# LSaldyt/JAX_llama

Measured on AMD Instinct MI355X. Metric: output_tokens_per_sec, higher is better.
Workload: dtype bf16; 1 GPU; model=llama3-8b, global_batch=2048, seq_len=384, prompt_len=128, gen_len=256, parallelism=dp1, mp=1

## Files before the change

### jax_llama_amd/csrc/bindings.cpp

```cpp
#include <torch/extension.h>
#include <c10/hip/HIPStream.h>

#include "kernels/launchers.h"

namespace {

using torch::Tensor;

hipStream_t stream() { return c10::hip::getCurrentHIPStream().stream(); }

void check(bool cond, const char* msg) { TORCH_CHECK(cond, "jax_llama_amd._C: ", msg); }

void check_gpu(const Tensor& t, const char* name) {
  TORCH_CHECK(t.is_cuda(), "jax_llama_amd._C: ", name, " must be a GPU tensor");
  TORCH_CHECK(t.is_contiguous(), "jax_llama_amd._C: ", name, " must be contiguous");
}

void rc(int r, const char* what) {
  TORCH_CHECK(r == 0, "jax_llama_amd._C: ", what, " failed (code ", r, ")");
}

void gemm_rc(int r, const char* what) {
  const char* why = r == -1   ? "no legal plan for this shape / tile id / epilogue / fused norm / K split"
                    : r == -3 ? "the slab workspace is missing or too small"
// ... 368 lines not shown
                     int64_t splits, c10::optional<Tensor> x_packed, int64_t spl, c10::optional<Tensor> sk_ws,
                     c10::optional<Tensor> sk_tk, c10::optional<Tensor> o_w, int64_t o_n, int64_t o_k,
                     c10::optional<Tensor> o_h, c10::optional<Tensor> o_hb, c10::optional<Tensor> o_hb_pack,
                     int64_t tp_state) {
  check_gpu(x, "x");
  check_packed(w, n, k);
  check(x.dim() == 2 && x.size(1) == k && x.scalar_type() == torch::kBFloat16, "linear_qkv_attn: x bf16 [M, K]");
  const int64_t m = x.size(0);
  check(m <= 32, "linear_qkv_attn: M <= 32");
  jla::QKVArgs qa = qkv_args(m, n, table, positions, kc, vc, slot, 1, h, hkv, dh, q);
  for (auto* t : {&kv_start, &out, &ws, &tickets, &sync}) check_gpu(*t, "linear_qkv_attn arg");
  check(kv_start.scalar_type() == torch::kInt32 && kv_start.numel() == m, "kv_start int32 [B]");
  check(out.scalar_type() == torch::kBFloat16 && out.numel() == m * h * dh, "out bf16 [B, H * Dh]");
  check(ws.scalar_type() == torch::kFloat32 && ws.numel() >= m * hkv * splits * (h / hkv) * (dh + 4), "ws too small");
  check(tickets.scalar_type() == torch::kInt32 && tickets.numel() >= m * hkv, "tickets int32 [pairs]");
  check(sync.scalar_type() == torch::kInt32 && (size_t)sync.numel() >= jla::qkv_attn_sync_ints(),
        "sync int32 [qkv_attn_sync_ints()]");
  check(t_cap <= kc.size(2), "t_cap <= cache length");
  const jla::bf16_t* xp = packed_ptr(x_packed, m, k, "x_packed");
  check(spl == 1 || spl == 2, "linear_qkv_attn: spl 1 or 2");
  if (spl > 1) {
    check(sk_ws.has_value() && sk_tk.has_value(), "linear_qkv_attn spl 2: sk_ws and sk_tk (skinny_workspace)");
    check_gpu(*sk_ws, "sk_ws");
    check_gpu(*sk_tk, "sk_tk");
    check(sk_ws->scalar_type() == torch::kFloat32 && sk_tk->scalar_type() == torch::kInt32 &&
              sk_tk->numel() >= n / 16,
          "linear_qkv_attn: sk_ws fp32, sk_tk int32 [N / 16]");
    qa.sk_ws = ptr<float>(*sk_ws);
    qa.sk_tk = ptr<int32_t>(*sk_tk);
    qa.sk_ws_floats = (int)sk_ws->numel();
  }
  jla::QKVArgs qo{};
  float* oh = nullptr;
  int o_mode = 0;
  if (o_w.has_value()) {
    check_packed(*o_w, o_n, o_k);
    check(o_k == h * dh, "linear_qkv_attn: Wo has H * Dh input columns");
    check(o_h.has_value() && o_hb.has_value(), "linear_qkv_attn: the fused o projection needs h and hb");
    check_gpu(*o_h, "h");
    check_gpu(*o_hb, "hb");
    check(o_h->scalar_type() == torch::kFloat32 && o_h->numel() == m * o_n && o_hb->scalar_type() == torch::kBFloat16 &&
              o_hb->numel() == m * o_n, "linear_qkv_attn: h fp32 / hb bf16 [M, N_o]");
    const int og = jla::qkv_attn_o_groups((int)m, (int)(h / hkv), (int)o_n, (int)o_k);
    check(og > 0, "linear_qkv_attn: the o projection cannot be fused at this shape (qkv_attn_o_groups)");
    oh = ptr<float>(*o_h);
    qo.res_bf16 = bf(*o_hb);
    qo.pack = packed_ptr(o_hb_pack, m, o_n, "o_hb_pack");
    o_mode = MODE_RESIDUAL;
    if (tp_state) {
      void* st = reinterpret_cast<void*>(tp_state);
      check(og <= jla::CAR_WG_COUNTERS && og * jla::TPRES_REGION <= jla::car_max_bytes(st),
            "linear_qkv_attn: too many o workgroups for the TP buffer");
      qo.tp = jla::car_device(st);
      o_mode = MODE_TPRESID;
    }
  }
  rc(jla::linear_qkv_attn(xp ? xp : cbf(x), w.data_ptr(), m, n, k, (float)rms_eps, qa, xp != nullptr, bf(out),
                          packed_ptr(out_pack, m, h * dh, "out_pack"), ptr<int32_t>(kv_start), ptr<float>(ws),
                          ptr<int32_t>(tickets), ptr<int32_t>(sync), (int)t_cap, (int)splits, (int)spl, stream(),
                          o_w.has_value() ? o_w->data_ptr() : nullptr, oh, (int)o_n, (int)o_k, o_mode,
                          o_w.has_value() ? &qo : nullptr),
     "linear_qkv_attn");
}

bool check_gemm_ws(const c10::optional<Tensor>& ws, int64_t k, int64_t ksplit, int64_t m, int64_t n, bool rms,
                   int64_t tile) {
  if (!is_g5(tile) && ksplit <= 1) return false;
  check(ws.has_value(), "gemm: a K split (gemm5: any plan) needs the slab workspace");
  check_gpu(*ws, "gemm ws");
  const int64_t ks = is_g5(tile) ? jla::gemm5_ksplit((int)k, (int)ksplit) : ksplit;
  check(ws->scalar_type() == torch::kFloat32 && ws->numel() >= ks * m * (n + (rms ? 1 : 0)), "gemm ws too small");
  return true;
}

static float* rms_ws_ptr(const c10::optional<Tensor>& rws, int64_t m, size_t* floats) {
  *floats = 0;
  if (!rws.has_value()) return nullptr;
  check_gpu(*rws, "rms_ws");
  check(rws->scalar_type() == torch::kFloat32 && rws->numel() >= m, "rms_ws: fp32, >= M floats");
  *floats = rws->numel();
  return ptr<float>(*rws);
}

void gemm(Tensor x, Tensor w, int64_t n, int64_t k, Tensor out, int64_t mode, bool accumulate,
          c10::optional<Tensor> mirror, int64_t ksplit, c10::optional<Tensor> ws, double rms_eps, int64_t tile,
          c10::optional<Tensor> pack_out, c10::optional<Tensor> rms_ws, int64_t n_body) {
  check_gpu(x, "x");
  check_packed(w, n, k);
  check(n_body >= 0 && (n_body == 0 || jla::gemm_tail_width((int)tile) > 0), "gemm n_body: tail-balanced tiles only");
  check(x.dim() == 2 && x.size(1) == k && x.scalar_type() == torch::kBFloat16, "x must be bf16 [M, K]");
  check(mode >= 0 && mode <= 2, "gemm mode");
  const int64_t m = x.size(0);
  check_linear_out(out, m, n, mode);
  jla::bf16_t* mir = mode == 1 ? mirror_ptr(mirror, out.numel()) : nullptr;
  jla::QKVArgs pqa{};
  if (pack_out.has_value()) {
    check(m <= SKINNY_MAX_M && (mode == 1 || mode == 2) && (mode != 1 || mir), "gemm pack_out: decode M, residual "
          "(with its mirror) or SwiGLU");
    check(ksplit > 1 || is_g5(tile), "gemm pack_out: the split-K reduce-kernel path only");
    pqa.pack = packed_ptr(pack_out, m, mode == 2 ? n / 2 : n, "pack_out");
  }
  const bool slabs = check_gemm_ws(ws, k, ksplit, m, n, rms_eps >= 0, tile);
  size_t rfl = 0;
  float* rws = rms_ws_ptr(rms_ws, m, &rfl);
  gemm_rc(jla::gemm(cbf(x), w.data_ptr(), out.data_ptr(), m, n, k, mode, accumulate,
                    out.scalar_type() == torch::kFloat32, mir, pqa.pack ? &pqa : nullptr,
                    slabs ? ptr<float>(*ws) : nullptr, slabs ? ws->numel() : 0, ksplit, stream(), (float)rms_eps,
                    (int)tile, rws, rfl, (int)n_body),
          "gemm");
}

void gemm_qkv(Tensor x, Tensor w, int64_t n, int64_t k, Tensor table, Tensor positions, Tensor kc, Tensor vc,
              Tensor slot, int64_t seq_len, int64_t h, int64_t hkv, int64_t dh, Tensor q, int64_t ksplit,
              c10::optional<Tensor> ws, double rms_eps, int64_t tile, c10::optional<Tensor> rms_ws) {
  check_gpu(x, "x");
  check_packed(w, n, k);
  check(x.dim() == 2 && x.size(1) == k && x.scalar_type() == torch::kBFloat16, "x must be bf16 [M, K]");
  const int64_t m = x.size(0);
  jla::QKVArgs qa = qkv_args(m, n, table, positions, kc, vc, slot, seq_len, h, hkv, dh, q);
  const bool slabs = check_gemm_ws(ws, k, ksplit, m, n, rms_eps >= 0, tile);
  size_t rfl = 0;
  float* rws = rms_ws_ptr(rms_ws, m, &rfl);
  gemm_rc(jla::gemm(cbf(x), w.data_ptr(), nullptr, m, n, k, MODE_QKV, 0, 0, nullptr, &qa,
                    slabs ? ptr<float>(*ws) : nullptr, slabs ? ws->numel() : 0, ksplit, stream(), (float)rms_eps,
                    (int)tile, rws, rfl),
          "gemm_qkv");
}

void rope_kv_write(Tensor qkv, Tensor table, Tensor positions, Tensor kc, Tensor vc, Tensor slot, int64_t seq_len,
                   int64_t h, int64_t hkv, int64_t dh, Tensor q) {
  for (auto* t : {&qkv, &table, &positions, &kc, &vc, &slot, &q}) check_gpu(*t, "rope_kv_write arg");
  check(qkv.scalar_type() == torch::kBFloat16 && kc.scalar_type() == torch::kBFloat16 &&
            vc.scalar_type() == torch::kBFloat16 && q.scalar_type() == torch::kBFloat16,
        "rope_kv_write bf16 tensors");
  check(table.scalar_type() == torch::kFloat32 && table.dim() == 3 && table.size(1) == dh / 2 && table.size(2) == 2,
        "rope table must be fp32 [L, Dh/2, 2]");
  check(positions.scalar_type() == torch::kInt32 && slot.scalar_type() == torch::kInt32, "int32 positions/slot");
  const int64_t m = qkv.size(0);
  check(qkv.dim() == 2 && qkv.size(1) == (h + 2 * hkv) * dh, "qkv shape");
  check(positions.numel() == m && m % seq_len == 0, "positions shape");
  const int64_t b = m / seq_len;
  check(kc.dim() == 4 && kc.size(0) == b && kc.size(1) == hkv && kc.size(3) == dh && vc.sizes() == kc.sizes(),
        "cache shape [B, Hkv, T, Dh]");
  check(q.numel() == m * h * dh, "q out shape");
  rc(jla::rope_kv_write(cbf(qkv), ptr<float>(table), table.size(0), ptr<int32_t>(positions), bf(kc), bf(vc),
                        ptr<int32_t>(slot), m, seq_len, h, hkv, dh, kc.size(2), bf(q), stream()),
     "rope_kv_write");
}

void check_attn(const Tensor& q, const Tensor& kc, const Tensor& vc, const Tensor& slot, const Tensor& kv_start,
                const c10::optional<Tensor>& key_mask, const Tensor& out) {
  for (auto* t : {&q, &kc, &vc, &slot, &kv_start, &out}) check_gpu(*t, "attention arg");
  check(q.scalar_type() == torch::kBFloat16 && kc.scalar_type() == torch::kBFloat16 &&
            vc.scalar_type() == torch::kBFloat16 && out.scalar_type() == torch::kBFloat16,
        "attention bf16 tensors");
  check(q.dim() == 4 && kc.dim() == 4 && kc.sizes() == vc.sizes(), "attention shapes");
  check(kc.size(0) == q.size(0) && kc.size(3) == q.size(3), "cache/q shape mismatch");
  check(q.size(2) % kc.size(1) == 0, "H must be a multiple of Hkv");
  check(slot.scalar_type() == torch::kInt32 && kv_start.scalar_type() == torch::kInt32 &&
            kv_start.numel() == q.size(0),
        "slot/kv_start");
  check(out.numel() == q.numel(), "attention out shape");
  if (key_mask.has_value()) {
    check_gpu(*key_mask, "key_mask");
    check(key_mask->scalar_type() == torch::kUInt8 && key_mask->dim() == 2 && key_mask->size(0) == q.size(0),
          "key_mask must be uint8 [B, L]");
  }
}

void attn_decode(Tensor q, Tensor kc, Tensor vc, Tensor slot, Tensor kv_start, c10::optional<Tensor> key_mask,
                 Tensor out, Tensor ws, Tensor tickets, int64_t t_cap, int64_t nsplit, c10::optional<Tensor> out_pack) {
  check_attn(q, kc, vc, slot, kv_start, key_mask, out);
  check(q.size(1) == 1, "attn_decode: one query per row");
  const int64_t b = q.size(0), h = q.size(2), dh = q.size(3), hkv = kc.size(1), T = kc.size(2);
  check(t_cap <= T, "t_cap exceeds the cache length");
  check_gpu(ws, "ws");
  check_gpu(tickets, "tickets");
  const jla::AttnPlanResult r = jla::attn_decode_plan(jla::attn_knobs(), b, h, hkv, dh, t_cap, key_mask.has_value());
  TORCH_CHECK(r.rc == 0, "jax_llama_amd._C: attn_decode: no plan (", r.why, "; see attn_plan.h)");
  TORCH_CHECK(nsplit == r.plan.nsplit, "jax_llama_amd._C: attn_decode: nsplit ", nsplit, " is not the plan's ",
              r.plan.nsplit, " (attn_decode_plan_check)");
  check(!out_pack.has_value() || r.plan.packs,
        "attn_decode: this launch does not write the packed copy (attn_decode_plan_check's packs)");
  check(ws.scalar_type() == torch::kFloat32 && (size_t)ws.numel() >= r.plan.ws_floats, "workspace too small");
  check(tickets.scalar_type() == torch::kInt32 && tickets.numel() >= r.plan.tickets, "tickets too small");
  const uint8_t* km = key_mask.has_value() ? ptr<uint8_t>(*key_mask) : nullptr;
  const int ml = key_mask.has_value() ? key_mask->size(1) : 0;
  rc(jla::attn_decode(cbf(q), cbf(kc), cbf(vc), ptr<int32_t>(slot), ptr<int32_t>(kv_start), km, ml, bf(out),
                      ptr<float>(ws), ptr<int32_t>(tickets), b, h, hkv, dh, T, t_cap, nsplit, stream(),
                      packed_ptr(out_pack, b, h * dh, "out_pack")),
     "attn_decode");
}

void attn_prefill(Tensor q, Tensor kc, Tensor vc, Tensor slot, Tensor kv_start, c10::optional<Tensor> key_mask,
                  Tensor out) {
  check_attn(q, kc, vc, slot, kv_start, key_mask, out);
  const uint8_t* km = key_mask.has_value() ? ptr<uint8_t>(*key_mask) : nullptr;
  const int ml = key_mask.has_value() ? key_mask->size(1) : 0;
  rc(jla::attn_prefill(cbf(q), cbf(kc), cbf(vc), ptr<int32_t>(slot), ptr<int32_t>(kv_start), km, ml, bf(out),
                       q.size(0), q.size(1), q.size(2), kc.size(1), q.size(3), kc.size(2), stream()),
     "attn_prefill");
}

static void check_kv8(const Tensor& kq, const Tensor& ks, const Tensor& vq, const Tensor& vs, int64_t b, int64_t hkv,
                      const char* who) {
  for (auto* t : {&kq, &ks, &vq, &vs}) check_gpu(*t, who);
  check(kq.scalar_type() == torch::kUInt8 && vq.scalar_type() == torch::kUInt8 && kq.dim() == 4 && kq.size(0) == b &&
            kq.size(1) == hkv && kq.size(2) > 0 && kq.size(3) == jla::ATTN_DH && vq.sizes() == kq.sizes(),
// ... 24 lines not shown
                           kq.size(2), bf(q), stream()),
     "rope_kv_write_q8");
}

void kv8_dequant(Tensor kq, Tensor ks, Tensor vq, Tensor vs, int64_t n, Tensor kout, Tensor vout) {
  check(kq.dim() == 4, "kv8_dequant: q bytes must be uint8 [B, Hkv, T, 128]");
  const int64_t b = kq.size(0), hkv = kq.size(1);
  check_kv8(kq, ks, vq, vs, b, hkv, "kv8_dequant cache");
  check_gpu(kout, "kout");
  check_gpu(vout, "vout");
  check(kout.scalar_type() == torch::kBFloat16 && vout.scalar_type() == torch::kBFloat16 && kout.dim() == 4 &&
            kout.size(0) == b && kout.size(1) == hkv && kout.size(3) == jla::ATTN_DH && vout.sizes() == kout.sizes(),
        "kv8_dequant: outputs must be bf16 [B, Hkv, n_out, 128]");
  check(n >= 0 && n <= kq.size(2) && n <= kout.size(2), "kv8_dequant: n within the cache and the outputs");
  check(b * hkv <= INT32_MAX && kq.size(2) <= INT32_MAX, "kv8_dequant: sizes");
  rc(jla::kv8_dequant(ptr<uint8_t>(kq), ptr<float>(ks), ptr<uint8_t>(vq), ptr<float>(vs), bf(kout), bf(vout), b * hkv,
                      kq.size(2), n, kout.size(2), stream()),
     "kv8_dequant");
}

void attn_decode_q8(Tensor q, Tensor kq, Tensor ks, Tensor vq, Tensor vs, Tensor slot, Tensor kv_start,
                    c10::optional<Tensor> key_mask, Tensor out, int64_t t_cap, c10::optional<Tensor> ws,
                    c10::optional<Tensor> tickets) {
  for (auto* t : {&q, &slot, &kv_start, &out}) check_gpu(*t, "attn_decode_q8 arg");
  check(q.scalar_type() == torch::kBFloat16 && out.scalar_type() == torch::kBFloat16 && q.dim() == 4 && q.size(1) == 1,
        "attn_decode_q8: q bf16 [B, 1, H, Dh]");
  const int64_t b = q.size(0), h = q.size(2), dh = q.size(3);
  check(kq.dim() == 4, "attn_decode_q8: q bytes must be uint8 [B, Hkv, T, 128]");
  const int64_t hkv = kq.size(1), T = kq.size(2);
  check_kv8(kq, ks, vq, vs, b, hkv, "attn_decode_q8 cache");
  check(slot.scalar_type() == torch::kInt32 && slot.numel() >= 1 && kv_start.scalar_type() == torch::kInt32 &&
            kv_start.numel() == b,
        "slot/kv_start");
  check(out.numel() == q.numel(), "attention out shape");
  check(t_cap >= 0 && t_cap <= T, "t_cap exceeds the cache length");
  check(b <= 65535, "attn_decode_q8: at most 65535 rows");
  if (key_mask.has_value()) {
    check_gpu(*key_mask, "key_mask");
    check(key_mask->scalar_type() == torch::kUInt8 && key_mask->dim() == 2 && key_mask->size(0) == b,
          "key_mask must be uint8 [B, L]");
  }
  const jla::AttnQ8PlanResult r =
      jla::attn_decode_q8_plan(jla::attn_knobs(), b, h, hkv, dh, t_cap, key_mask.has_value());
  TORCH_CHECK(r.rc == 0, "jax_llama_amd._C: attn_decode_q8: no plan (", r.why, "; see attn_plan.h)");
  float* wsp = nullptr;
  int32_t* tkp = nullptr;
  if (r.plan.nsplit > 1) {
    TORCH_CHECK(ws.has_value() && tickets.has_value(), "jax_llama_amd._C: attn_decode_q8: the plan splits the keys (nsplit ",
                r.plan.nsplit, "): ws and tickets are required (attn_decode_q8_split_check)");
    check_gpu(*ws, "ws");
    check_gpu(*tickets, "tickets");
    TORCH_CHECK(ws->scalar_type() == torch::kFloat32 && ws->device() == q.device() &&
                    (size_t)ws->numel() >= r.plan.ws_floats,
                "jax_llama_amd._C: attn_decode_q8: ws must be fp32 on q's device with at least B * H * nsplit * (128 + 4) = ",
                r.plan.ws_floats, " floats (attn_decode_q8_split_check)");
    TORCH_CHECK(tickets->scalar_type() == torch::kInt32 && tickets->device() == q.device() &&
                    tickets->numel() >= r.plan.tickets,
                "jax_llama_amd._C: attn_decode_q8: tickets must be int32 on q's device, one per (row, kv head) pair = ",
                r.plan.tickets, " (attn_decode_q8_split_check)");
    wsp = ptr<float>(*ws);
    tkp = ptr<int32_t>(*tickets);
  }
  const uint8_t* km = key_mask.has_value() ? ptr<uint8_t>(*key_mask) : nullptr;
  const int ml = key_mask.has_value() ? key_mask->size(1) : 0;
  rc(jla::attn_decode_q8(cbf(q), ptr<uint8_t>(kq), ptr<float>(ks), ptr<uint8_t>(vq), ptr<float>(vs),
                         ptr<int32_t>(slot), ptr<int32_t>(kv_start), km, ml, bf(out), b, h, hkv, dh, T, t_cap,
                         stream(), wsp, r.plan.ws_floats, tkp, r.plan.tickets),
     "attn_decode_q8");
}

void argmax(Tensor logits, Tensor idx, Tensor val) {
  check_gpu(logits, "logits");
  check_gpu(idx, "idx");
  check_gpu(val, "val");
  check(logits.scalar_type() == torch::kFloat32 && logits.dim() == 2, "logits must be fp32 [B, V]");
  check(idx.scalar_type() == torch::kInt32 && val.scalar_type() == torch::kFloat32 &&
            idx.numel() == logits.size(0) && val.numel() == logits.size(0),
        "argmax outputs");
  rc(jla::argmax(ptr<float>(logits), logits.size(0), logits.size(1), ptr<int32_t>(idx), ptr<float>(val), stream()),
     "argmax");
}

void gemm_argmax(Tensor x, Tensor w, int64_t n, int64_t k, Tensor ws, double rms_eps, Tensor idx, Tensor val,
                 c10::optional<Tensor> rms_ws) {
  check_gpu(x, "x");
  check_packed(w, n, k);
  check(x.dim() == 2 && x.size(1) == k && x.scalar_type() == torch::kBFloat16, "x must be bf16 [M, K]");
  const int64_t m = x.size(0);
  check_gpu(ws, "ws");
  check(ws.scalar_type() == torch::kFloat32 && (size_t)ws.numel() >= jla::gemm_argmax_workspace_floats(m, n),
        "gemm_argmax ws too small");
  check_gpu(idx, "idx");
  check_gpu(val, "val");
  check(idx.scalar_type() == torch::kInt32 && val.scalar_type() == torch::kFloat32 && idx.numel() == m &&
            val.numel() == m,
        "gemm_argmax outputs");
  size_t rfl = 0;
  float* rws = rms_ws_ptr(rms_ws, m, &rfl);
  rc(jla::gemm_argmax(cbf(x), w.data_ptr(), ptr<float>(ws), ws.numel(), m, n, k, (float)rms_eps, ptr<int32_t>(idx),
                      ptr<float>(val), stream(), rws, rfl),
     "gemm_argmax");
}

static void check_logprob_io(const Tensor& targets, const Tensor& tgt, const Tensor& mx, const Tensor& se, int64_t m,
                             int64_t col_offset) {
  for (auto* t : {&targets, &tgt, &mx, &se}) check_gpu(*t, "logprob arg");
  check(targets.scalar_type() == torch::kInt32 && targets.numel() == m, "targets must be int32 [M]");
  for (auto* t : {&tgt, &mx, &se})
    check(t->scalar_type() == torch::kFloat32 && t->numel() == m, "logprob outputs must be fp32 [M]");
  check(col_offset >= 0 && col_offset <= INT32_MAX, "col_offset");
}

void gemm_logprob(Tensor x, Tensor w, int64_t n, int64_t k, Tensor ws, double rms_eps, Tensor targets,
                  int64_t col_offset, Tensor tgt, Tensor mx, Tensor se, c10::optional<Tensor> rms_ws) {
  check_gpu(x, "x");
  check_packed(w, n, k);
  check(x.dim() == 2 && x.size(1) == k && x.scalar_type() == torch::kBFloat16, "x must be bf16 [M, K]");
  const int64_t m = x.size(0);
  check_gpu(ws, "ws");
  check(ws.scalar_type() == torch::kFloat32 && (size_t)ws.numel() >= jla::gemm_logprob_workspace_floats(m, n),
        "gemm_logprob ws too small");
  check_logprob_io(targets, tgt, mx, se, m, col_offset);
  size_t rfl = 0;
  float* rws = rms_ws_ptr(rms_ws, m, &rfl);
  gemm_rc(jla::gemm_logprob(cbf(x), w.data_ptr(), ptr<float>(ws), ws.numel(), m, n, k, (float)rms_eps,
                            ptr<int32_t>(targets), (int)col_offset, ptr<float>(tgt), ptr<float>(mx), ptr<float>(se),
                            stream(), rws, rfl),
          "gemm_logprob");
}

void logprob_rows(Tensor logits, Tensor targets, int64_t col_offset, Tensor tgt, Tensor mx, Tensor se) {
  check_gpu(logits, "logits");
  check(logits.scalar_type() == torch::kFloat32 && logits.dim() == 2 && logits.size(1) > 0,
        "logits must be fp32 [B, V]");
  check(logits.size(1) <= INT32_MAX, "logprob_rows: V too large");
  check_logprob_io(targets, tgt, mx, se, logits.size(0), col_offset);
  rc(jla::logprob_rows(ptr<float>(logits), logits.size(0), logits.size(1), ptr<int32_t>(targets), (int)col_offset,
                       ptr<float>(tgt), ptr<float>(mx), ptr<float>(se), stream()),
     "logprob_rows");
}

void topk_chunk(Tensor logits, int64_t k, int64_t idx_offset, Tensor cv, Tensor ci) {
  for (auto* t : {&logits, &cv, &ci}) check_gpu(*t, "topk_chunk arg");
  check(logits.scalar_type() == torch::kFloat32 && logits.dim() == 2, "logits must be fp32 [B, V]");
  const int64_t b = logits.size(0), v = logits.size(1);
  check(k >= 1 && k <= 64 && k <= v, "topk_chunk: 1 <= k <= min(64, V)");
  const int64_t c = (int64_t)jla::topk_chunks(v) * k;
  check(cv.scalar_type() == torch::kFloat32 && ci.scalar_type() == torch::kInt32 && cv.numel() == b * c &&
            ci.numel() == b * c,
        "topk_chunk: candidates must be [B, chunks*k] fp32/int32");
  rc(jla::topk_chunk(ptr<float>(logits), b, v, k, idx_offset, ptr<float>(cv), ptr<int32_t>(ci), stream()),
     "topk_chunk");
}

void topk_merge(Tensor cv, Tensor ci, int64_t k, int64_t mode, c10::optional<Tensor> out_v,
                c10::optional<Tensor> out_i, c10::optional<Tensor> nxt, double temperature, double top_p,
                int64_t seed, c10::optional<Tensor> step) {
  check_gpu(cv, "cv");
  check_gpu(ci, "ci");
  check(cv.dim() == 2 && cv.sizes() == ci.sizes() && cv.scalar_type() == torch::kFloat32 &&
            ci.scalar_type() == torch::kInt32,
        "topk_merge: candidates [B, C] fp32/int32");
  const int64_t b = cv.size(0), c = cv.size(1);
  check(k >= 1 && k <= 64 && k <= c && c <= 4096, "topk_merge: 1 <= k <= 64, k <= C <= 4096");
  float* ov = nullptr;
  int32_t* oi = nullptr;
  int32_t* nx = nullptr;
  const int32_t* st = nullptr;
  if (mode == 0) {
    check(out_v.has_value() && out_i.has_value(), "topk_merge mode 0 needs out_v/out_i");
    check_gpu(*out_v, "out_v");
    check_gpu(*out_i, "out_i");
    check(out_v->scalar_type() == torch::kFloat32 && out_i->scalar_type() == torch::kInt32 &&
              out_v->numel() == b * k && out_i->numel() == b * k,
          "topk_merge outputs [B, k]");
    ov = ptr<float>(*out_v);
    oi = ptr<int32_t>(*out_i);
  } else {
    check(mode == 1 && nxt.has_value() && step.has_value(), "topk_merge mode 1 needs nxt and step");
    check_gpu(*nxt, "nxt");
    check_gpu(*step, "step");
    check(nxt->scalar_type() == torch::kInt32 && nxt->numel() == b && step->scalar_type() == torch::kInt32,
          "topk_merge nxt [B] / step [1] int32");
    check(temperature > 0, "topk_merge: temperature > 0");
    nx = ptr<int32_t>(*nxt);
    st = ptr<int32_t>(*step);
  }
  rc(jla::topk_merge(ptr<float>(cv), ptr<int32_t>(ci), b, c, k, mode, ov, oi, nx, (float)temperature, (float)top_p,
                     (uint64_t)seed, st, stream()),
     "topk_merge");
}

void decode_update(Tensor nxt, Tensor finished, Tensor sequences, Tensor cur_len, Tensor tokens, Tensor positions,
                   Tensor slot, int64_t pad, int64_t eos) {
  for (auto* t : {&nxt, &finished, &sequences, &cur_len, &tokens, &positions, &slot}) {
    check_gpu(*t, "decode_update arg");
    check(t->scalar_type() == torch::kInt32, "decode_update: int32 tensors");
  }
  const int64_t b = nxt.numel();
  check(finished.numel() == b && tokens.numel() == b && positions.numel() == b && sequences.dim() == 2 &&
            sequences.size(0) == b,
        "decode_update shapes");
  rc(jla::decode_update(ptr<int32_t>(nxt), ptr<int32_t>(finished), ptr<int32_t>(sequences), ptr<int32_t>(cur_len),
                        ptr<int32_t>(tokens), ptr<int32_t>(positions), ptr<int32_t>(slot), b, sequences.size(1), pad,
                        eos, stream()),
     "decode_update");
}

py::tuple car_alloc(int64_t max_bytes, int64_t world) {
  void* buf = nullptr;
// ... 63 lines not shown
  check(m >= 1 && m <= SKINNY_MAX_M, "linear_tp_residual: 1 <= M <= 64");
  check(h.scalar_type() == torch::kFloat32 && h.numel() == m * n && hb.scalar_type() == torch::kBFloat16 &&
            hb.numel() == m * n, "h fp32 / hb bf16 [M, N]");
  void* st = reinterpret_cast<void*>(state);
  const int64_t groups = n / 16;
  check(groups <= jla::CAR_WG_COUNTERS && groups * jla::TPRES_REGION <= jla::car_max_bytes(st),
        "linear_tp_residual: too many workgroups for the buffer");
  jla::QKVArgs qa{};
  qa.res_bf16 = bf(hb);
  qa.pack = packed_ptr(hb_pack, m, n, "hb_pack");
  qa.tp = jla::car_device(st);
  run_skinny(x, w, n, k, h.data_ptr(), MODE_TPRESID, -1.0, true, true, &qa, variant, ws ? *ws : Tensor(),
             tickets ? *tickets : Tensor(), packed_ptr(x_packed, m, k, "x_packed"));
}

void gemm_tp_residual(int64_t state, Tensor x, Tensor w, int64_t n, int64_t k, Tensor h, Tensor hb, int64_t ksplit,
                      Tensor ws, int64_t tile) {
  check_gpu(x, "x");
  check_gpu(h, "h");
  check_gpu(hb, "hb");
  check_packed(w, n, k);
  check(x.dim() == 2 && x.size(1) == k && x.scalar_type() == torch::kBFloat16, "x must be bf16 [M, K]");
  const int64_t m = x.size(0);
  check(h.scalar_type() == torch::kFloat32 && h.numel() == m * n && hb.scalar_type() == torch::kBFloat16 &&
            hb.numel() == m * n, "h fp32 / hb bf16 [M, N]");
  void* st = reinterpret_cast<void*>(state);
  const int64_t groups = jla::gemm_tp_groups((int)m, (int)n);
  check(groups <= jla::CAR_WG_COUNTERS && groups * jla::TPRES_REGION <= jla::car_max_bytes(st),
        "gemm_tp_residual: the output does not fit the fused exchange buffer");
  check_gemm_ws(ws, k, ksplit, m, n, false, tile);
  jla::QKVArgs qa{};
  qa.tp = jla::car_device(st);
  gemm_rc(jla::gemm(cbf(x), w.data_ptr(), h.data_ptr(), m, n, k, MODE_TPRESID, 1, 1, bf(hb), &qa, ptr<float>(ws),
                    ws.numel(), ksplit, stream(), -1.f, (int)tile, nullptr, 0),
          "gemm_tp_residual");
}

void car_pairs(int64_t state, int64_t mode, Tensor vals, Tensor idx, int64_t idx_offset, int64_t k,
               c10::optional<Tensor> out_v, Tensor out_i) {
  check_gpu(vals, "vals");
  check_gpu(idx, "idx");
  check_gpu(out_i, "out_i");
  check(vals.scalar_type() == torch::kFloat32 && idx.scalar_type() == torch::kInt32 &&
            out_i.scalar_type() == torch::kInt32 && vals.numel() == idx.numel(),
        "car_pairs dtypes");
  const int64_t n = vals.numel();
  auto* st = reinterpret_cast<void*>(state);
  float* ov = nullptr;
  if (out_v.has_value()) {
    check_gpu(*out_v, "out_v");
    check(out_v->scalar_type() == torch::kFloat32 && out_v->numel() == out_i.numel(), "out_v");
    ov = ptr<float>(*out_v);
  }
  if (mode == 0) {
    check(out_i.numel() == n, "car_pairs argmax out shape");
  } else {
    check(mode == 1 && ov && k > 0 && n % k == 0 && out_i.numel() == n * jla::car_world(st), "car_pairs top-k shapes");
  }
  rc(jla::car_pairs(st, (int)mode, ptr<float>(vals), ptr<int32_t>(idx), (int)idx_offset, n, (int)k, ov,
                    ptr<int32_t>(out_i), stream()),
     "car_pairs");
}

}

PYBIND11_MODULE(TORCH_EXTENSION_NAME, m) {
  m.doc() = "jax_llama_amd gfx950 (MI355X) HIP kernels";
  m.attr("SKINNY_MAX_M") = SKINNY_MAX_M;
  m.attr("ARCH") = "gfx950";
  m.def("embedding", &embedding, py::arg("ids"), py::arg("table"), py::arg("out"),
        py::arg("mirror") = py::none());
  m.def("rms_scale", &rms_scale);
  m.def("rmsnorm", &rmsnorm);
  m.def("residual_add", &residual_add);
  m.def("gemm_f32", &gemm_f32);
  m.def("prefetch", &prefetch, py::arg("t"), py::arg("grid") = 128);
  m.def("linear_skinny", &linear_skinny, py::arg("x"), py::arg("w"), py::arg("n"), py::arg("k"), py::arg("out"),
        py::arg("mode"), py::arg("rms_eps"), py::arg("accumulate"), py::arg("variant"), py::arg("ws"),
        py::arg("tickets"), py::arg("mirror") = py::none(), py::arg("x_packed") = py::none(),
        py::arg("pack_out") = py::none());
  m.def("gemm", &gemm, py::arg("x"), py::arg("w"), py::arg("n"), py::arg("k"), py::arg("out"), py::arg("mode"),
        py::arg("accumulate"), py::arg("mirror") = py::none(), py::arg("ksplit") = 1, py::arg("ws") = py::none(),
        py::arg("rms_eps") = -1.0, py::arg("tile") = 0, py::arg("pack_out") = py::none(),
        py::arg("rms_ws") = py::none(), py::arg("n_body") = 0);
  m.def("gemm_tail_split", [](int64_t tiles_m, int64_t n, int64_t width, int64_t cus) {
    const int nb = jla::gemm_tail_split((int)tiles_m, (int)n, (int)width, cus > 0 ? (int)cus : jla::gemm_num_cus());
    return std::make_pair((int64_t)nb, nb > 0 ? (n - nb * width + 127) / 128 : (int64_t)0);
  }, py::arg("tiles_m"), py::arg("n"), py::arg("width"), py::arg("cus") = 0);
  m.def("gemm_plan_check", [](int64_t m, int64_t n, int64_t k, int64_t mode, bool rms, int64_t ksplit, int64_t tile,
                              bool has_rms_ws, int64_t n_body) {
    return jla::gemm_plan_check((int)m, (int)n, (int)k, (int)mode, rms, (int)ksplit, (int)tile, has_rms_ws, (int)n_body);
  }, py::arg("m"), py::arg("n"), py::arg("k"), py::arg("mode"), py::arg("rms"), py::arg("ksplit"), py::arg("tile"),
     py::arg("has_rms_ws"), py::arg("n_body") = 0);
  m.def("gemv_plan_check", [](int64_t m, int64_t n, int64_t k, int64_t mode, bool x_f32, bool x_packed,
                              int64_t variant) {
    const jla::GemvPlanResult r = jla::gemv_plan((int)m, (int)n, (int)k, (int)mode, x_f32, x_packed, (int)variant);
    const jla::GemvPlan& p = r.plan;
    return py::make_tuple(r.rc, p.mt, p.nt, p.nw, p.deep, p.xp, p.ksplit);
  }, py::arg("m"), py::arg("n"), py::arg("k"), py::arg("mode"), py::arg("x_f32"), py::arg("x_packed"),
     py::arg("variant"));
  m.def("gemv_w8_plan_check", [](int64_t m, int64_t n, int64_t k, int64_t mode, bool x_f32) {
    const jla::GemvPlanResult r = jla::gemv_w8_plan((int)m, (int)n, (int)k, (int)mode, x_f32);
    return py::make_tuple(r.rc, r.plan.mt, r.plan.nt, r.plan.nw);
  }, py::arg("m"), py::arg("n"), py::arg("k"), py::arg("mode"), py::arg("x_f32"));
  m.def("dequant_fp8", &dequant_fp8, py::arg("w8"), py::arg("scale"), py::arg("n"), py::arg("k"), py::arg("out"));
  m.def("linear_skinny_w8", &linear_skinny_w8, py::arg("x"), py::arg("w8"), py::arg("scale"), py::arg("n"),
        py::arg("k"), py::arg("out"), py::arg("mode"), py::arg("rms_eps"), py::arg("accumulate"),
        py::arg("mirror") = py::none(), py::arg("pack_out") = py::none());
  m.def("linear_qkv_w8", &linear_qkv_w8, py::arg("x"), py::arg("w8"), py::arg("scale"), py::arg("n"), py::arg("k"),
        py::arg("rms_eps"), py::arg("table"), py::arg("positions"), py::arg("kc"), py::arg("vc"), py::arg("slot"),
        py::arg("seq_len"), py::arg("h"), py::arg("hkv"), py::arg("dh"), py::arg("q"));
  m.def("gemv_w4_plan_check", [](int64_t m, int64_t n, int64_t k, int64_t mode, bool x_f32) {
    const jla::GemvPlanResult r = jla::gemv_w4_plan((int)m, (int)n, (int)k, (int)mode, x_f32);
    return py::make_tuple(r.rc, r.plan.mt, r.plan.nt, r.plan.nw);
  }, py::arg("m"), py::arg("n"), py::arg("k"), py::arg("mode"), py::arg("x_f32"));
  m.def("dequant_fp4", &dequant_fp4, py::arg("w4"), py::arg("s4"), py::arg("n"), py::arg("k"), py::arg("out"));
  m.def("linear_skinny_w4", &linear_skinny_w4, py::arg("x"), py::arg("w4"), py::arg("s4"), py::arg("n"),
        py::arg("k"), py::arg("out"), py::arg("mode"), py::arg("rms_eps"), py::arg("accumulate"),
        py::arg("mirror") = py::none(), py::arg("pack_out") = py::none());
  m.def("linear_qkv_w4", &linear_qkv_w4, py::arg("x"), py::arg("w4"), py::arg("s4"), py::arg("n"), py::arg("k"),
        py::arg("rms_eps"), py::arg("table"), py::arg("positions"), py::arg("kc"), py::arg("vc"), py::arg("slot"),
        py::arg("seq_len"), py::arg("h"), py::arg("hkv"), py::arg("dh"), py::arg("q"));
  m.def("gemv_variant_table", []() {
    py::dict t;
    for (const jla::GemvVariant& v : jla::GEMV_VARIANTS) t[py::int_(v.id)] = py::make_tuple(v.xp, v.split);
    return t;
  });
  m.attr("GEMV_SPLIT_MAX_GROUPS") = jla::GEMV_SPLIT_MAX_GROUPS;
  m.def("gemm_qkv_direct_ok", [](int64_t m, int64_t tile, int64_t k) {
    return jla::gemm_qkv_direct_ok((int)m, (int)tile, (int)k) != 0;
  });
  m.def("gemm_set_g4_default", [](int64_t on) { jla::gemm_set_g4_default((int)on); });
  m.def("gemm_set_g4_group", [](int64_t gm) { jla::gemm_set_g4_group((int)gm); });
  m.def("gemm_qkv", &gemm_qkv, py::arg("x"), py::arg("w"), py::arg("n"), py::arg("k"), py::arg("table"),
        py::arg("positions"), py::arg("kc"), py::arg("vc"), py::arg("slot"), py::arg("seq_len"), py::arg("h"),
        py::arg("hkv"), py::arg("dh"), py::arg("q"), py::arg("ksplit"), py::arg("ws"), py::arg("rms_eps") = -1.0,
        py::arg("tile") = 0, py::arg("rms_ws") = py::none());
  m.def("gemm_argmax", &gemm_argmax, py::arg("x"), py::arg("w"), py::arg("n"), py::arg("k"), py::arg("ws"),
        py::arg("rms_eps"), py::arg("idx"), py::arg("val"), py::arg("rms_ws") = py::none());
  m.def("gemm_argmax_workspace", [](int64_t m, int64_t n) { return (int64_t)jla::gemm_argmax_workspace_floats(m, n); });
  m.def("gemm_logprob", &gemm_logprob, py::arg("x"), py::arg("w"), py::arg("n"), py::arg("k"), py::arg("ws"),
        py::arg("rms_eps"), py::arg("targets"), py::arg("col_offset"), py::arg("tgt"), py::arg("mx"), py::arg("se"),
        py::arg("rms_ws") = py::none());
  m.def("gemm_logprob_workspace",
        [](int64_t m, int64_t n) { return (int64_t)jla::gemm_logprob_workspace_floats(m, n); });
  m.def("logprob_rows", &logprob_rows);
  m.def("gemm_ksplit", [](int64_t m, int64_t n, int64_t k) { return jla::gemm_ksplit(m, n, k); });
  m.def("rope_kv_write", &rope_kv_write);
  m.def("attn_set_impl", [](int64_t impl, int64_t waves_target) { jla::attn_set_impl(impl, waves_target); },
        py::arg("impl"), py::arg("waves_target") = 0);
  m.def("attn_reset_knobs", []() { jla::attn_reset_knobs(); }, "every attn_set_* knob back to its default");
  m.def("attn_decode_plan_check", [](int64_t b, int64_t h, int64_t hkv, int64_t dh, int64_t t_cap, bool masked) {
    const jla::AttnPlanResult r =
        jla::attn_decode_plan(jla::attn_knobs(), (int)b, (int)h, (int)hkv, (int)dh, (int)t_cap, masked);
    const jla::AttnPlan& p = r.plan;
    return py::make_tuple(r.rc, r.why, r.rc ? "" : jla::attn_kernel_name(p.kernel), p.nsplit, p.packs,
                          (int64_t)p.ws_floats, p.tickets, p.rep, p.kpg, p.ring, p.fold, p.wpp, p.split_len);
  }, py::arg("b"), py::arg("h"), py::arg("hkv"), py::arg("dh"), py::arg("t_cap"), py::arg("masked"));
  m.def("attn_decode_splits", [](int64_t b, int64_t hkv, int64_t t, int64_t rep) {
    return jla::attn_decode_plan(jla::attn_knobs(), (int)b, (int)(hkv * rep), (int)hkv, jla::ATTN_DH, (int)t, false)
        .plan.nsplit;
  });
  m.def("attn_decode_packs", [](int64_t b, int64_t hkv, int64_t rep) {
    return (int)jla::attn_decode_plan(jla::attn_knobs(), (int)b, (int)(hkv * rep), (int)hkv, jla::ATTN_DH, 1, false)
        .plan.packs;
  });
  m.def("linear_qkv", &linear_qkv, py::arg("x"), py::arg("w"), py::arg("n"), py::arg("k"), py::arg("rms_eps"),
        py::arg("table"), py::arg("positions"), py::arg("kc"), py::arg("vc"), py::arg("slot"), py::arg("seq_len"),
        py::arg("h"), py::arg("hkv"), py::arg("dh"), py::arg("q"), py::arg("variant"), py::arg("ws"), py::arg("tickets"),
        py::arg("x_packed") = py::none());
  m.def("linear_qkv_attn", &linear_qkv_attn, py::arg("x"), py::arg("w"), py::arg("n"), py::arg("k"),
        py::arg("rms_eps"), py::arg("table"), py::arg("positions"), py::arg("kc"), py::arg("vc"), py::arg("slot"),
        py::arg("h"), py::arg("hkv"), py::arg("dh"), py::arg("q"), py::arg("kv_start"), py::arg("out"),
        py::arg("out_pack"), py::arg("ws"), py::arg("tickets"), py::arg("sync"), py::arg("t_cap"), py::arg("splits"),
        py::arg("x_packed") = py::none(), py::arg("spl") = 1, py::arg("sk_ws") = py::none(),
        py::arg("sk_tk") = py::none(), py::arg("o_w") = py::none(), py::arg("o_n") = 0, py::arg("o_k") = 0,
        py::arg("o_h") = py::none(), py::arg("o_hb") = py::none(), py::arg("o_hb_pack") = py::none(),
        py::arg("tp_state") = 0);
  m.def("qkv_attn_splits", [](int64_t m, int64_t b, int64_t hkv, int64_t rep, int64_t t_cap, int64_t n, int64_t cus,
                              int64_t spl, int64_t o_groups) {
    return jla::qkv_attn_splits((int)m, (int)b, (int)hkv, (int)rep, (int)t_cap, (int)n, (int)cus, (int)spl,
                                (int)o_groups);
  }, py::arg("m"), py::arg("b"), py::arg("hkv"), py::arg("rep"), py::arg("t_cap"), py::arg("n"), py::arg("cus"),
     py::arg("spl") = 1, py::arg("o_groups") = 0);
  m.def("qkv_attn_o_groups", [](int64_t m, int64_t rep, int64_t n, int64_t k) {
    return jla::qkv_attn_o_groups((int)m, (int)rep, (int)n, (int)k);
  });
  m.def("qkv_attn_sync_ints", []() { return (int64_t)jla::qkv_attn_sync_ints(); });
  m.def("qkv_attn_set_o_nt", [](int64_t nt) { jla::qkv_attn_set_o_nt((int)nt); });
  m.def("qkv_attn_set_diag", [](int64_t d) { jla::qkv_attn_set_diag((int)d); });
  m.def("qkv_attn_set_stamps", [](c10::optional<Tensor> t) {
    if (t.has_value()) {
      check_gpu(*t, "stamps");
      check(t->scalar_type() == torch::kInt64, "stamps int64");
    }
    jla::qkv_attn_set_stamps(t.has_value() ? reinterpret_cast<unsigned long long*>(t->data_ptr()) : nullptr);
  });
  m.def("qkv_attn_occupancy", [](int64_t m, int64_t rep, int64_t spl, int64_t o_groups) {
    return jla::qkv_attn_occupancy((int)m, (int)rep, (int)spl, (int)o_groups);
  }, py::arg("m"), py::arg("rep"), py::arg("spl") = 1, py::arg("o_groups") = 0);
  m.def("skinny_workspace", &skinny_workspace);
  m.def("linear_skinny_argmax", &linear_skinny_argmax);
  m.def("gemm_tp_residual", &gemm_tp_residual, py::arg("state"), py::arg("x"), py::arg("w"), py::arg("n"), py::arg("k"),
        py::arg("h"), py::arg("hb"), py::arg("ksplit"), py::arg("ws"), py::arg("tile"));
  m.def("gemm_tp_groups", [](int64_t m, int64_t n) { return (int64_t)jla::gemm_tp_groups((int)m, (int)n); });
  m.def("linear_tp_residual", &linear_tp_residual, py::arg("state"), py::arg("x"), py::arg("w"), py::arg("n"),
        py::arg("k"), py::arg("h"), py::arg("hb"), py::arg("variant"), py::arg("x_packed") = py::none(),
        py::arg("hb_pack") = py::none(), py::arg("ws") = py::none(), py::arg("tickets") = py::none());
  m.def("bounds_error", [](bool reset) {
    const int r = reset ? 1 : 0;
    return (int64_t)(jla::jla_bounds_norm_embed(r) | jla::jla_bounds_rope_kv(r) | jla::jla_bounds_sample(r) |
                     jla::jla_bounds_gemm(r) | jla::jla_bounds_gemv(r) | jla::jla_bounds_kv8(r) |
                     jla::jla_bounds_attn_decode(r) | jla::jla_bounds_attn_prefill(r));
  }, "OR of the bounds-checked debug build's error words (JLA_BOUNDS_* bits); always 0 in a release build",
        py::arg("reset") = false);
#ifdef JLA_DEBUG_BOUNDS
  m.attr("DEBUG_BOUNDS") = true;
#else
  m.attr("DEBUG_BOUNDS") = false;
#endif
  m.def("attn_set_diag", [](int64_t d) { jla::attn_set_diag((int)d); });
  m.def("cu_mask_stream", [](std::vector<int64_t> words) {
    std::vector<uint32_t> mk(words.begin(), words.end());
    hipStream_t s = nullptr;
    rc(jla::cu_mask_stream_create(mk.data(), (int)mk.size(), &s), "cu_mask_stream");
    return reinterpret_cast<int64_t>(s);
// ... 97 lines not shown
```

### jax_llama_amd/csrc/kernels/gemm.hip

```cpp
#include <type_traits>

#include "car.h"
#include "common.h"
#include "gemm4w.h"
#include "gemm5ws.h"
#include "gemm_plan.h"
#include "launchers.h"
#include "ring.h"

namespace jla {

constexpr int G2_BN = 256, G2_NBUF = 4, G2_GROUP_M = 8;
#ifdef JLA_GEMM_STAMPS
__device__ unsigned long long g_gemm_stamps[8192 * 8 * 6];
#endif

JLA_DEV void g2_tile_coords(int pid, int tiles_m, int tiles_n, int& tm, int& tn) {
  const int in_group = G2_GROUP_M * tiles_n;
  const int first_m = (pid / in_group) * G2_GROUP_M;
  const int gsz = min(tiles_m - first_m, G2_GROUP_M);
  tm = first_m + (pid % in_group) % gsz;
  tn = (pid % in_group) / gsz;
}

// ... 966 lines not shown
  }
  const size_t idx = e4 * 4;
  const int m = (int)(idx / N), col = (int)(idx - (size_t)m * N);
  float4 v = sum_splits(ws, ksplit, slab4, e4);
  float rs = 1.f;
  if (ssq) {
    float t = 0.f;
    for (int s = 0; s < ksplit; ++s) t += ssq[(size_t)s * M + m];
    rs = 1.f / sqrtf(t / (float)K + rms_eps);
    v.x *= rs;
    v.y *= rs;
    v.z *= rs;
    v.w *= rs;
  }
  float vv[4] = {v.x, v.y, v.z, v.w};
  if constexpr (MODE == MODE_SWIGLU) {
    const int tile = col >> 4, c0 = col & 15;
    float4 u = sum_splits(ws, ksplit, slab4, e4 + 4);
    u.x *= rs;
    u.y *= rs;
    u.z *= rs;
    u.w *= rs;
    const float uu[4] = {u.x, u.y, u.z, u.w};
    bf16_t* o = static_cast<bf16_t*>(out) + (size_t)m * (N >> 1) + (tile >> 1) * 16 + c0;
    const uint2 pk = make_uint2(pack2bf(silu(vv[0]) * uu[0], silu(vv[1]) * uu[1]),
                                pack2bf(silu(vv[2]) * uu[2], silu(vv[3]) * uu[3]));
    *reinterpret_cast<uint2*>(o) = pk;
    if (qa.pack) *reinterpret_cast<uint2*>(qa.pack + pack_off(m, (tile >> 1) * 16 + c0, N >> 1)) = pk;
  } else if constexpr (MODE == MODE_RESIDUAL) {
    float4* o = reinterpret_cast<float4*>(static_cast<float*>(out) + idx);
    float4 r = *o;
    if (accumulate) {
      r.x += vv[0];
      r.y += vv[1];
      r.z += vv[2];
      r.w += vv[3];
    } else {
      r = make_float4(vv[0], vv[1], vv[2], vv[3]);
    }
    *o = r;
    if (mirror) {
      const uint2 pk = make_uint2(pack2bf(r.x, r.y), pack2bf(r.z, r.w));
      *reinterpret_cast<uint2*>(mirror + idx) = pk;
      if (qa.pack) *reinterpret_cast<uint2*>(qa.pack + pack_off(m, col, N)) = pk;
    }
  } else if constexpr (MODE == MODE_QKV) {
    const int head = col / qa.Dh, d0 = col - head * qa.Dh;
    const int b = m / qa.S, sq = m - b * qa.S;
    if (head < qa.H + qa.Hkv) {
      int pos = qa.positions[m];
      if (pos < 0 || pos >= qa.table_len) JLA_FLAG(JLA_BOUNDS_ROPE_POS);
      pos = pos < 0 ? 0 : (pos >= qa.table_len ? qa.table_len - 1 : pos);
#pragma unroll
      for (int p = 0; p < 2; ++p) {
        const float2 cs = qa.table[(size_t)pos * (qa.Dh >> 1) + (d0 >> 1) + p];
        const float xr = vv[2 * p], xi = vv[2 * p + 1];
        vv[2 * p] = xr * cs.x - xi * cs.y;
        vv[2 * p + 1] = xr * cs.y + xi * cs.x;
      }
    }
    const uint2 packed = make_uint2(pack2bf(vv[0], vv[1]), pack2bf(vv[2], vv[3]));
    if (head < qa.H) {
      *reinterpret_cast<uint2*>(qa.q + ((size_t)m * qa.H + head) * qa.Dh + d0) = packed;
    } else {
      const int slot = qa.slot[0] + sq;
      if (slot < qa.T) {
        const bool is_k = head < qa.H + qa.Hkv;
        const int kh = is_k ? head - qa.H : head - qa.H - qa.Hkv;
        bf16_t* cache = is_k ? qa.kc : qa.vc;
        *reinterpret_cast<uint2*>(cache + (((size_t)b * qa.Hkv + kh) * qa.T + slot) * qa.Dh + d0) = packed;
      } else {
        JLA_FLAG(JLA_BOUNDS_KV_SLOT);
      }
    }
  } else {
    if (out_f32)
      *reinterpret_cast<float4*>(static_cast<float*>(out) + idx) = make_float4(vv[0], vv[1], vv[2], vv[3]);
    else
      *reinterpret_cast<uint2*>(static_cast<bf16_t*>(out) + idx) =
          make_uint2(pack2bf(vv[0], vv[1]), pack2bf(vv[2], vv[3]));
  }
}

constexpr int TPR_ELEMS = 4096;
static_assert(TPR_ELEMS / 2 * 8 == TPRES_REGION, "one fused-exchange region per workgroup");
__global__ void __launch_bounds__(256)
    gemm_reduce_tp_kernel(const float* __restrict__ ws, int ksplit, float* __restrict__ h, bf16_t* __restrict__ hb,
                          int M, int N, const CarDevice* __restrict__ dev) {
  const CarDevice& d = *dev;
  const int w = blockIdx.x;
  const size_t slab4 = (size_t)M * N / 4;
  __shared__ int s_calls;
  if (threadIdx.x == 0) s_calls = __hip_atomic_load(d.wg_ctr + w, __ATOMIC_RELAXED, __HIP_MEMORY_SCOPE_AGENT) + 1;
  u32x2 gq[4];
  f32x4 hv[4];
#pragma unroll
  for (int j = 0; j < 4; ++j) {
    const size_t e4 = (size_t)w * (TPR_ELEMS / 4) + j * 256 + threadIdx.x;
    gq[j] = u32x2{0u, 0u};
    hv[j] = f32x4{0.f, 0.f, 0.f, 0.f};
    if (e4 < slab4) {
      const float4 v = sum_splits(ws, ksplit, slab4, e4);
      gq[j] = u32x2{pack2bf(v.x, v.y), pack2bf(v.z, v.w)};
      hv[j] = *reinterpret_cast<const f32x4*>(h + e4 * 4);
    }
  }
  __syncthreads();
  const int calls = s_calls;
  const unsigned tag = gran_tag_fused(calls);
  const long long wg_base = (long long)w * TPRES_REGION;
  const long long par_base = (long long)(calls & 1) * d.world * d.max_bytes;
#pragma unroll
  for (int j = 0; j < 4; ++j) {
    const size_t e4 = (size_t)w * (TPR_ELEMS / 4) + j * 256 + threadIdx.x;
    if (e4 >= slab4) continue;
    const long long g = wg_base + (long long)(j * 256 + threadIdx.x) * 16;
    for (int p = 0; p < d.world; ++p) {
      const __amdgpu_buffer_rsrc_t rp = rsrc(d.buf[p]);
      const long long o = par_base + (long long)d.rank * d.max_bytes + g;
      st_sys8(rp, o, u32x2{gq[j][0], tag});
      st_sys8(rp, o + 8, u32x2{gq[j][1], tag});
    }
  }
  const bool give_up = __hip_atomic_load(d.error, __ATOMIC_RELAXED, __HIP_MEMORY_SCOPE_SYSTEM) != 0;
  const __amdgpu_buffer_rsrc_t mine = rsrc(d.buf[d.rank]);
#pragma unroll
  for (int j = 0; j < 4; ++j) {
    const size_t e4 = (size_t)w * (TPR_ELEMS / 4) + j * 256 + threadIdx.x;
    if (e4 >= slab4) continue;
    const long long g = wg_base + (long long)(j * 256 + threadIdx.x) * 16;
    float sm[4] = {0.f, 0.f, 0.f, 0.f};
    u32x4 r[CAR_MAX_WORLD];
    car_gather16(d, mine, par_base + g, d.max_bytes, tag, give_up, r);
#pragma unroll
    for (int p = 0; p < CAR_MAX_WORLD; ++p) {
      if (p < d.world) {
        sm[0] += __uint_as_float(r[p][0] << 16);
        sm[1] += __uint_as_float(r[p][0] & 0xffff0000u);
        sm[2] += __uint_as_float(r[p][2] << 16);
        sm[3] += __uint_as_float(r[p][2] & 0xffff0000u);
      }
    }
    f32x4 n;
#pragma unroll
    for (int i = 0; i < 4; ++i) n[i] = hv[j][i] + sm[i];
    *reinterpret_cast<f32x4*>(h + e4 * 4) = n;
    *reinterpret_cast<u32x2*>(hb + e4 * 4) = u32x2{pack2bf(n[0], n[1]), pack2bf(n[2], n[3])};
  }
  if (threadIdx.x == 0) __hip_atomic_store(d.wg_ctr + w, calls, __ATOMIC_RELAXED, __HIP_MEMORY_SCOPE_AGENT);
}
int gemm_tp_groups(int M, int N) { return (int)(((size_t)M * N + TPR_ELEMS - 1) / TPR_ELEMS); }


static int g2_wm(int M) { return M <= 128 ? 1 : 2; }

int gemm_ksplit(int M, int N, int K) {
  const int KS = K >> 5;
  const int bm = 128 * g2_wm(M);
  const int tiles = ((N + G2_BN - 1) / G2_BN) * ((M + bm - 1) / bm);
  int ks = min(256 / tiles, max(1, K / (2 * M)));
  ks = ks < 1 ? 1 : (ks > 16 ? 16 : ks);
  while (ks > 1 && KS / ks < 4) --ks;
  const int kc = (KS + ks - 1) / ks;
  return (KS + kc - 1) / kc;
}

size_t gemm_workspace_floats(int M, int N, int K) {
  const int ks = gemm_ksplit(M, N, K);
  return ks > 1 ? (size_t)ks * M * (N + 1) : 0;
}

static int num_cus() {
  static int cus = 0;
  if (cus == 0) {
    int dev = 0;
    hipDeviceProp_t prop;
    if (hipGetDevice(&dev) == hipSuccess && hipGetDeviceProperties(&prop, dev) == hipSuccess)
      cus = prop.multiProcessorCount;
    if (cus <= 0) cus = 256;
  }
  return cus;
}
int gemm_num_cus() { return num_cus(); }

static bool g_g4_default = true;
void gemm_set_g4_default(int on) { g_g4_default = on != 0; }
int gemm_qkv_direct_ok(int M, int tile, int K) {
  const GemmPlanResult r = gemm_plan(M, 16, K, MODE_QKV, true, 1, tile, true, 0, 0, g_g4_default);
  return r.rc == 0 && !r.plan.reduce;
}
int gemm_plan_check(int M, int N, int K, int mode, int rms, int ksplit, int tile, int has_rms_ws, int n_body) {
  return gemm_plan(M, N, K, mode, rms != 0, ksplit, tile, has_rms_ws != 0, n_body, num_cus(), g_g4_default).rc;
}

struct GemmArgs {
  const bf16_t* x;
  const u32x4* w;
  void* out;
  int M, N, K, accumulate, out_f32;
  bf16_t* mirror;
  float rms_eps;
  float* ssq;
  float* rms_ws;
  QKVArgs qa;
  hipStream_t s;
};

static bool g4_row_stat(const GemmArgs& a, const GemmPlan& p, const float*& inv) {
  inv = p.norm == NORM_PRECOMPUTED ? a.rms_ws : nullptr;
  return inv == nullptr || rms_rowinv(a.x, a.rms_ws, a.M, a.K, a.rms_eps, a.s) == 0;
}

static int g_g4_group = 0;
void gemm_set_g4_group(int gm) { g_g4_group = gm; }
static int g4_group_m(int tiles_m) {
  const int gm = g_g4_group > 0 ? g_g4_group : 4;
  return gm < tiles_m ? gm : tiles_m;
}
static int g_g5_diag = 0;
void gemm5_set_diag(int d) { g_g5_diag = d; }

template <int MODE, int NJ>
static void launch_g4(const GemmArgs& a, const GemmPlan& p) {
  const int tm = (a.M + G4_BM - 1) / G4_BM, tn = (a.N + 32 * NJ - 1) / (32 * NJ);
  const int grid = tm * tn * p.ksplit, gm = g4_group_m(tm);
  const float* inv;
  if (!g4_row_stat(a, p, inv)) return;
#define JLA_G4(R, DIAG, DEEP)                                                                                       \
  gemm4_kernel<MODE, R, NJ, DIAG, DEEP><<<grid, 256, 0, a.s>>>(a.x, a.w, a.out, a.M, a.N, a.K, a.accumulate, a.out_f32, \
                                                               a.mirror, p.kc, tm, tn, a.rms_eps, a.ssq, a.qa, inv, gm)
  if constexpr (NJ != 8) {
    if (inv)
      JLA_G4(2, 0, true);
    else
      JLA_G4(0, 0, true);
  } else {
    if constexpr (MODE == MODE_STORE) {
      if (p.norm == NORM_NONE && (g_g5_diag & 192)) {
        if ((g_g5_diag & 192) == 64)
          JLA_G4(0, 1, false);
        else if ((g_g5_diag & 192) == 128)
          JLA_G4(0, 2, false);
        else
          JLA_G4(0, 3, false);
        return;
      }
    }
    if (p.norm == NORM_PRECOMPUTED) {
      if (p.deep) JLA_G4(2, 0, true); else JLA_G4(2, 0, false);
    } else if (p.norm == NORM_INLOOP) {
      if (p.deep) JLA_G4(1, 0, true); else JLA_G4(1, 0, false);
    } else {
      if (p.deep) JLA_G4(0, 0, true); else JLA_G4(0, 0, false);
    }
  }
#undef JLA_G4
}

template <int MODE>
static void launch_g4p(const GemmArgs& a, const GemmPlan& p) {
  const int tm = (a.M + G4_BM - 1) / G4_BM, tn = (a.N + G4_BN - 1) / G4_BN;
  const int grid = min(tm * tn, num_cus()), gm = g4_group_m(tm);
  const float* inv;
  if (!g4_row_stat(a, p, inv)) return;
#define JLA_G4P(R)                                                                                                  \
  gemm4p_kernel<MODE, R><<<grid, 256, 0, a.s>>>(a.x, a.w, a.out, a.M, a.N, a.K, a.accumulate, a.out_f32, a.mirror, tm, \
                                                tn, a.rms_eps, a.qa, inv, gm)
  if (p.norm == NORM_PRECOMPUTED)
    JLA_G4P(2);
  else if (p.norm == NORM_INLOOP)
    JLA_G4P(1);
  else
    JLA_G4P(0);
#undef JLA_G4P
}

template <int MODE, int NJB>
static void launch_g4t(const GemmArgs& a, const GemmPlan& p) {
  const int tm = (a.M + G4_BM - 1) / G4_BM, nt = (a.N - p.n_body * 32 * NJB + 127) / 128;
  const int grid = tm * (p.n_body + nt), gm = g4_group_m(tm);
  const float* inv;
  if (!g4_row_stat(a, p, inv)) return;
  if (inv)
    gemm4t_kernel<MODE, 2, NJB><<<grid, 256, 0, a.s>>>(a.x, a.w, a.out, a.M, a.N, a.K, a.accumulate, a.out_f32,
                                                       a.mirror, tm, p.n_body, nt, a.rms_eps, inv, gm);
  else
    gemm4t_kernel<MODE, 0, NJB><<<grid, 256, 0, a.s>>>(a.x, a.w, a.out, a.M, a.N, a.K, a.accumulate, a.out_f32,
                                                       a.mirror, tm, p.n_body, nt, a.rms_eps, nullptr, gm);
}

template <int MODE>
static void launch_g2(const GemmArgs& a, const GemmPlan& p) {
  const int cfg = p.family;
// ... 5 lines not shown
      a.x, a.w, a.out, a.M, a.N, a.K, a.accumulate, a.out_f32, a.mirror, p.kc, tm, tn, a.rms_eps, a.ssq, a.qa)
#define JLA_G2_CFG(R)                        \
  if (cfg == 2)                              \
    JLA_G2(1, false, R, 8, 4, false, 0);     \
  else if (cfg == 3)                         \
    JLA_G2(2, true, R, 4, 2, false, 0);      \
  else                                       \
    JLA_G2(2, true, R, 8, 4, true, 2)
  [[maybe_unused]] const bool rms = p.norm != NORM_NONE;
  if constexpr (MODE == MODE_QKV) {
    JLA_G2(2, true, true, 8, 4, true, 2);
  } else if constexpr (MODE == MODE_ARGMAX) {
    if (rms)
      JLA_G2(2, true, true, 8, 4, true, 2);
    else
      JLA_G2(2, true, false, 8, 4, true, 2);
  } else if constexpr (MODE == MODE_RESIDUAL) {
    JLA_G2_CFG(false);
  } else {
    if (rms) {
      JLA_G2_CFG(true);
    } else {
      JLA_G2_CFG(false);
    }
  }
#undef JLA_G2_CFG
#undef JLA_G2
}

static void launch_g5(const GemmArgs& a, const GemmPlan& p) {
  const int mt = a.M <= 128 ? 8 : 16, rows = 16 * mt, ntw = p.nj;
  const int tiles_m = (a.M + rows - 1) / rows, tiles_n = (a.N + 64 * ntw - 1) / (64 * ntw);
  const int grid = tiles_m * tiles_n * p.ksplit;
#define JLA_G5(MTV, NTV)                                                                                            \
  gemm5_partial_kernel<MTV, NTV><<<grid, 256, 0, a.s>>>(a.x, a.w, static_cast<float*>(a.out), a.M, a.N, a.K, p.kc, \
                                                        tiles_m, tiles_n, a.ssq, g_g5_diag)
  if (mt == 8 && ntw == 4)
    JLA_G5(8, 4);
  else if (mt == 8)
    JLA_G5(8, 2);
  else if (ntw == 4)
    JLA_G5(16, 4);
  else
    JLA_G5(16, 2);
#undef JLA_G5
}

template <int MODE>
static void launch_plan(const GemmArgs& a, const GemmPlan& p) {
  constexpr bool PLAIN = MODE == MODE_STORE || MODE == MODE_RESIDUAL || MODE == MODE_SWIGLU;
  switch (p.family) {
    case GEMM2_256x256:
    case GEMM2_128x256:
    case GEMM2_128x128:
      if constexpr (MODE != MODE_LOGPROB) launch_g2<MODE>(a, p);
      break;
    case GEMM4:
      if (p.nj == 8) launch_g4<MODE, 8>(a, p);
      if constexpr (MODE != MODE_ARGMAX && MODE != MODE_LOGPROB) {
        if (p.nj == 6) launch_g4<MODE, 6>(a, p);
      }
      if constexpr (PLAIN || MODE == MODE_PARTIAL) {
        if (p.nj == 4) launch_g4<MODE, 4>(a, p);
      }
      break;
    case GEMM4_PERSISTENT:
      if constexpr (PLAIN || MODE == MODE_QKV) launch_g4p<MODE>(a, p);
      break;
    case GEMM4_TAIL:
      if constexpr (PLAIN) {
        if (p.nj == 6)
          launch_g4t<MODE, 6>(a, p);
        else
          launch_g4t<MODE, 8>(a, p);
      }
      break;
    case GEMM5:
      if constexpr (MODE == MODE_PARTIAL) launch_g5(a, p);
      break;
    case GEMM_NONE: break;
  }
}

static int launch_reduce(const float* ws, int ksplit, void* out, int M, int N, int K, int mode, int accumulate,
                         int out_f32, bf16_t* mirror, const QKVArgs* qkv, const float* ssq, float rms_eps,
                         hipStream_t s) {
  const size_t total4 = (size_t)M * N / (mode == MODE_SWIGLU ? 8 : 4);
  const int rgrid = (int)((total4 + 255) / 256);
  QKVArgs qa{};
  if (qkv) qa = *qkv;
  const float eps = ssq ? rms_eps : 0.f;
  switch (mode) {
    case MODE_STORE:
      gemm_reduce_kernel<MODE_STORE><<<rgrid, 256, 0, s>>>(ws, ksplit, out, M, N, accumulate, out_f32, nullptr, qa,
                                                           ssq, K, eps);
      break;
    case MODE_RESIDUAL:
      gemm_reduce_kernel<MODE_RESIDUAL><<<rgrid, 256, 0, s>>>(ws, ksplit, out, M, N, accumulate, 1, mirror, qa,
                                                              nullptr, K, eps);
      break;
    case MODE_SWIGLU:
      gemm_reduce_kernel<MODE_SWIGLU><<<rgrid, 256, 0, s>>>(ws, ksplit, out, M, N, accumulate, 0, nullptr, qa, ssq,
                                                            K, eps);
      break;
    case MODE_QKV:
      gemm_reduce_kernel<MODE_QKV><<<rgrid, 256, 0, s>>>(ws, ksplit, out, M, N, accumulate, 0, nullptr, qa, ssq, K,
                                                         eps);
      break;
    case MODE_TPRESID:
      if (!qkv || !qa.tp || !mirror || ssq || (N & 3)) return -1;
      gemm_reduce_tp_kernel<<<gemm_tp_groups(M, N), 256, 0, s>>>(ws, ksplit, static_cast<float*>(out), mirror, M, N,
                                                                 static_cast<const CarDevice*>(qa.tp));
      break;
    default: return -1;
  }
  JLA_CHECK_LAUNCH();
  return 0;
}

int gemm(const bf16_t* x, const void* W, void* out, int M, int N, int K, int mode, int accumulate, int out_f32,
         bf16_t* mirror, const QKVArgs* qkv, float* ws, size_t ws_floats, int ksplit, hipStream_t s,
         float rms_eps, int tile, float* rms_ws, size_t rms_ws_floats, int n_body) {
  const bool has_rms_ws = rms_ws != nullptr && rms_ws_floats >= (size_t)M;
  const GemmPlanResult r =
      gemm_plan(M, N, K, mode, rms_eps >= 0.f, ksplit, tile, has_rms_ws, n_body, num_cus(), g_g4_default);
  const GemmPlan& p = r.plan;
  if (r.rc != 0 || p.family == GEMM_NONE) return r.rc;
  if (mode == MODE_ARGMAX || mode == MODE_LOGPROB || (mode == MODE_QKV && !qkv)) return -1;
  const u32x4* w = static_cast<const u32x4*>(W);
  if (!p.reduce) {
    GemmArgs a{x, w, out, M, N, K, accumulate, out_f32, nullptr, rms_eps, nullptr, rms_ws, QKVArgs{}, s};
    switch (mode) {
      case MODE_QKV:
        a.out = nullptr, a.accumulate = a.out_f32 = 0, a.qa = *qkv;
        launch_plan<MODE_QKV>(a, p);
        break;
      case MODE_STORE: launch_plan<MODE_STORE>(a, p); break;
      case MODE_RESIDUAL:
        a.out_f32 = 1, a.mirror = mirror, a.rms_eps = -1.f;
        launch_plan<MODE_RESIDUAL>(a, p);
        break;
      case MODE_SWIGLU:
        a.out_f32 = 0;
        launch_plan<MODE_SWIGLU>(a, p);
        break;
      default: return -1;
    }
    JLA_CHECK_LAUNCH();
    return 0;
  }
  const size_t slabs = (size_t)p.ksplit * M * N;
  if (ws == nullptr || ws_floats < slabs + (p.norm != NORM_NONE ? (size_t)p.ksplit * M : 0)) return -3;
  float* ssq = p.norm != NORM_NONE ? ws + slabs : nullptr;
  launch_plan<MODE_PARTIAL>(GemmArgs{x, w, ws, M, N, K, 0, 1, nullptr, rms_eps, ssq, nullptr, QKVArgs{}, s}, p);
  JLA_CHECK_LAUNCH();
  return launch_reduce(ws, p.ksplit, out, M, N, K, mode, accumulate, out_f32, mirror, qkv, ssq, rms_eps, s);
}

JLA_DEV void amax_merge(float& bv, int& bi, float ov, int oi) {
  if (ov > bv || (ov == bv && oi < bi)) {
    bv = ov;
    bi = oi;
  }
}

template <int TPR>
__global__ void __launch_bounds__(TPR == 64 ? 256 : TPR)
    argmax_partials_kernel(const float2* __restrict__ part, int P, int M, int32_t* __restrict__ idx,
                           float* __restrict__ val) {
  __shared__ float s_v[16];
  __shared__ int s_i[16];
  const int row = TPR == 64 ? blockIdx.x * 4 + (threadIdx.x >> 6) : blockIdx.x;
  const int t = TPR == 64 ? (threadIdx.x & 63) : threadIdx.x;
  if (row >= M) return;
  const float2* pr = part + (size_t)row * P;
  float bv[4] = {-INFINITY, -INFINITY, -INFINITY, -INFINITY};
  int bi[4] = {0x7fffffff, 0x7fffffff, 0x7fffffff, 0x7fffffff};
  for (int k0 = t; k0 < P; k0 += 4 * TPR) {
    float2 e[4];
#pragma unroll
    for (int u = 0; u < 4; ++u) {
      const int k = k0 + u * TPR;
      e[u] = k < P ? pr[k] : make_float2(-INFINITY, __int_as_float(0x7fffffff));
    }
#pragma unroll
    for (int u = 0; u < 4; ++u) amax_merge(bv[u], bi[u], e[u].x, __float_as_int(e[u].y));
  }
#pragma unroll
  for (int u = 1; u < 4; ++u) amax_merge(bv[0], bi[0], bv[u], bi[u]);
#pragma unroll
  for (int o = 32; o > 0; o >>= 1) amax_merge(bv[0], bi[0], __shfl_xor(bv[0], o, 64), __shfl_xor(bi[0], o, 64));
  if constexpr (TPR > 64) {
    const int w = threadIdx.x >> 6;
    if ((threadIdx.x & 63) == 0) {
      s_v[w] = bv[0];
      s_i[w] = bi[0];
    }
    __syncthreads();
    if (threadIdx.x == 0) {
      for (int ww = 1; ww < TPR / 64; ++ww) amax_merge(bv[0], bi[0], s_v[ww], s_i[ww]);
      idx[row] = bi[0] == 0x7fffffff ? 0 : bi[0];
      val[row] = bv[0];
    }
  } else if (t == 0) {
    idx[row] = bi[0] == 0x7fffffff ? 0 : bi[0];
    val[row] = bv[0];
  }
}

static void launch_argmax_partials(const float2* part, int P, int M, int32_t* idx, float* val, hipStream_t s) {
  if (M <= 512)
    argmax_partials_kernel<1024><<<M, 1024, 0, s>>>(part, P, M, idx, val);
  else
    argmax_partials_kernel<64><<<(M + 3) / 4, 256, 0, s>>>(part, P, M, idx, val);
}

int argmax_partials(const float* part, int P, int M, int32_t* idx, float* val, hipStream_t s) {
  if (M <= 0) return 0;
  launch_argmax_partials(reinterpret_cast<const float2*>(part), P, M, idx, val, s);
  JLA_CHECK_LAUNCH();
  return 0;
}

size_t gemm_argmax_workspace_floats(int M, int N) { return (size_t)M * ((N + G2_BN - 1) / G2_BN) * 4 * 2; }

int gemm_argmax(const bf16_t* x, const void* W, float* ws, size_t ws_floats, int M, int N, int K, float rms_eps,
                int32_t* idx, float* val, hipStream_t s, float* rms_ws, size_t rms_ws_floats) {
  const bool has_rms_ws = rms_ws != nullptr && rms_ws_floats >= (size_t)M;
  const GemmPlanResult r = gemm_plan(M, N, K, MODE_ARGMAX, rms_eps >= 0.f, 1, 0, has_rms_ws, 0, 0, g_g4_default);
  if (r.rc != 0 || r.plan.family == GEMM_NONE) return r.rc;
  if (ws == nullptr || ws_floats < gemm_argmax_workspace_floats(M, N)) return -3;
  launch_plan<MODE_ARGMAX>(
      GemmArgs{x, static_cast<const u32x4*>(W), ws, M, N, K, 0, 1, nullptr, rms_eps, nullptr, rms_ws, QKVArgs{}, s},
      r.plan);
  JLA_CHECK_LAUNCH();
  const int P = (N + G2_BN - 1) / G2_BN * (r.plan.family == GEMM4 ? 2 : 4);
  launch_argmax_partials(reinterpret_cast<const float2*>(ws), P, M, idx, val, s);
  JLA_CHECK_LAUNCH();
  return 0;
}

JLA_DEV void lse_merge(float& m, float& s, float om, float os) {
  constexpr float LOG2E = 1.4426950408889634f;
  if (om == -INFINITY) return;
  if (m == -INFINITY) {
    m = om;
    s = os;
    return;
  }
  const float nm = fmaxf(m, om);
  s = s * __builtin_amdgcn_exp2f((m - nm) * LOG2E) + os * __builtin_amdgcn_exp2f((om - nm) * LOG2E);
  m = nm;
}

template <int TPR>
__global__ void __launch_bounds__(TPR == 64 ? 256 : TPR)
    lse_partials_kernel(const float2* __restrict__ part, int P, int M, float* __restrict__ mx,
                        float* __restrict__ se) {
  __shared__ float s_m[16];
  __shared__ float s_s[16];
  const int row = TPR == 64 ? blockIdx.x * 4 + (threadIdx.x >> 6) : blockIdx.x;
  const int t = TPR == 64 ? (threadIdx.x & 63) : threadIdx.x;
  if (row >= M) return;
  const float2* pr = part + (size_t)row * P;
  float bm[4] = {-INFINITY, -INFINITY, -INFINITY, -INFINITY};
  float bs[4] = {0.f, 0.f, 0.f, 0.f};
  for (int k0 = t; k0 < P; k0 += 4 * TPR) {
    float2 e[4];
#pragma unroll
    for (int u = 0; u < 4; ++u) {
      const int k = k0 + u * TPR;
      e[u] = k < P ? pr[k] : make_float2(-INFINITY, 0.f);
    }
#pragma unroll
    for (int u = 0; u < 4; ++u) lse_merge(bm[u], bs[u], e[u].x, e[u].y);
  }
#pragma unroll
  for (int u = 1; u < 4; ++u) lse_merge(bm[0], bs[0], bm[u], bs[u]);
#pragma unroll
  for (int o = 32; o > 0; o >>= 1)
    lse_merge(bm[0], bs[0], __shfl_xor(bm[0], o, 64), __shfl_xor(bs[0], o, 64));
  if constexpr (TPR > 64) {
    const int w = threadIdx.x >> 6;
    if ((threadIdx.x & 63) == 0) {
      s_m[w] = bm[0];
      s_s[w] = bs[0];
    }
    __syncthreads();
    if (threadIdx.x == 0) {
      for (int ww = 1; ww < TPR / 64; ++ww) lse_merge(bm[0], bs[0], s_m[ww], s_s[ww]);
      mx[row] = bm[0];
      se[row] = bs[0];
    }
  } else if (t == 0) {
    mx[row] = bm[0];
    se[row] = bs[0];
  }
}

static void launch_lse_partials(const float2* part, int P, int M, float* mx, float* se, hipStream_t s) {
  if (M <= 512)
    lse_partials_kernel<1024><<<M, 1024, 0, s>>>(part, P, M, mx, se);
  else
    lse_partials_kernel<64><<<(M + 3) / 4, 256, 0, s>>>(part, P, M, mx, se);
}

size_t gemm_logprob_workspace_floats(int M, int N) { return (size_t)M * ((N + G4_BN - 1) / G4_BN) * 2 * 2; }

int gemm_logprob(const bf16_t* x, const void* W, float* ws, size_t ws_floats, int M, int N, int K, float rms_eps,
                 const int32_t* targets, int col_offset, float* tgt, float* mx, float* se, hipStream_t s,
                 float* rms_ws, size_t rms_ws_floats) {
  const bool has_rms_ws = rms_ws != nullptr && rms_ws_floats >= (size_t)M;
  const GemmPlanResult r = gemm_plan(M, N, K, MODE_LOGPROB, rms_eps >= 0.f, 1, 0, has_rms_ws, 0, 0, g_g4_default);
  if (r.rc != 0 || r.plan.family == GEMM_NONE) return r.rc;
  if (ws == nullptr || ws_floats < gemm_logprob_workspace_floats(M, N)) return -3;
  if (targets == nullptr || tgt == nullptr || mx == nullptr || se == nullptr) return -1;
  const hipError_t zeroed = hipMemsetAsync(tgt, 0, (size_t)M * sizeof(float), s);
  if (zeroed != hipSuccess) return (int)zeroed;
  GemmArgs a{x, static_cast<const u32x4*>(W), ws, M, N, K, 0, 1, nullptr, rms_eps, nullptr, rms_ws, QKVArgs{}, s};
  a.qa.lp_targets = targets, a.qa.lp_tgt = tgt, a.qa.lp_col_offset = col_offset;
  launch_plan<MODE_LOGPROB>(a, r.plan);
  JLA_CHECK_LAUNCH();
  launch_lse_partials(reinterpret_cast<const float2*>(ws), (N + G4_BN - 1) / G4_BN * 2, M, mx, se, s);
  JLA_CHECK_LAUNCH();
  return 0;
}

JLA_BOUNDS_ACCESSOR(gemm)

}
```

### jax_llama_amd/csrc/kernels/launchers.h

```cpp
#pragma once
#include <hip/hip_runtime.h>
#include <stdint.h>

#include "attn_plan.h"
#include "gemm_plan.h"
#include "gemv_plan.h"

namespace jla {
typedef uint16_t bf16_t;

int embedding(const int32_t* ids, const bf16_t* table, float* out, bf16_t* mirror, int M, int D, int V,
              hipStream_t s);
int rms_scale(const float* x, bf16_t* out, int M, int D, float eps, hipStream_t s);
int rms_scale_bf16(const bf16_t* x, bf16_t* out, int M, int D, float eps, hipStream_t s);
int rms_rowinv(const bf16_t* x, float* inv, int M, int D, float eps, hipStream_t s);
int residual_add(float* h, const void* p, int p_bf16, bf16_t* hb, long long n, hipStream_t s);
int prefetch(const void* p, long long nbytes, int grid, unsigned* sink, hipStream_t s);
int stream_probe(const void* p, long long nbytes, int grid, unsigned* sink, hipStream_t s);
int gemm_f32(const float* x, const float* w, float* y, int M, int N, int K, hipStream_t s);
int rmsnorm(const float* x, const float* w, float* out, int M, int D, float eps, hipStream_t s);

struct QKVArgs {
  const float2* table;
  int table_len;
  union {
    const int32_t* positions;
    const int32_t* lp_targets;
  };
  bf16_t* kc;
  bf16_t* vc;
  const int32_t* slot;
  int S, H, Hkv, Dh, T;
  bf16_t* q;
  bf16_t* res_bf16;
  bf16_t* pack;
  const void* tp;
  union {
    float* sk_ws;
    float* lp_tgt;
  };
  int32_t* sk_tk;
  union {
    int sk_ws_floats;
    int lp_col_offset;
  };
};

constexpr int CAR_WG_COUNTERS = 4096;
constexpr long long TPRES_REGION = 64 * 64 * 4;

int qkv_attn_o_groups(int M, int rep, int N, int K);
size_t qkv_attn_sync_ints();
void qkv_attn_set_o_nt(int nt);
int qkv_attn_splits(int M, int B, int Hkv, int rep, int t_cap, int N, int cus, int spl = 1, int o_groups = 0);
int qkv_attn_occupancy(int M, int rep, int spl = 1, int o_groups = 0);
void qkv_attn_set_stamps(unsigned long long* p);
void qkv_attn_set_diag(int d);
int linear_qkv_attn(const bf16_t* x, const void* W, int M, int N, int K, float rms_eps, const QKVArgs& qa, bool xp,
                    bf16_t* out, bf16_t* out_pack, const int32_t* kv_start, float* ws, int32_t* tickets, int32_t* sync,
                    int t_cap, int splits, int spl, hipStream_t s,
                    const void* o_w = nullptr, float* o_h = nullptr, int o_n = 0, int o_k = 0, int o_mode = 0,
                    const QKVArgs* qo = nullptr);
int linear_skinny(const void* x, int x_is_f32, const void* W, void* out, int M, int N, int K, int mode,
                  float rms_eps, int accumulate, int out_f32, const QKVArgs* qkv, int variant, hipStream_t s);
int dequant_fp8(const void* W8, const float* scale, void* out, int N, int K, hipStream_t s);
int linear_skinny_w8(const void* x, int x_is_f32, const void* W8, const float* scale, void* out, int M, int N, int K,
                     int mode, float rms_eps, int accumulate, int out_f32, const QKVArgs* qkv, hipStream_t s);
int dequant_fp4(const void* W4, const void* S4, void* out, int N, int K, hipStream_t s);
int linear_skinny_w4(const void* x, int x_is_f32, const void* W4, const void* S4, void* out, int M, int N, int K,
                     int mode, float rms_eps, int accumulate, int out_f32, const QKVArgs* qkv, hipStream_t s);
int clock_probe(int iters, int grid, unsigned long long* out, hipStream_t s);
int gemm(const bf16_t* x, const void* W, void* out, int M, int N, int K, int mode, int accumulate, int out_f32,
         bf16_t* mirror, const QKVArgs* qkv, float* ws, size_t ws_floats, int ksplit, hipStream_t s,
         float rms_eps = -1.f, int tile = 0, float* rms_ws = nullptr, size_t rms_ws_floats = 0, int n_body = 0);
int gemm_plan_check(int M, int N, int K, int mode, int rms, int ksplit, int tile, int has_rms_ws, int n_body);
int gemm_ksplit(int M, int N, int K);
size_t gemm_workspace_floats(int M, int N, int K);
int gemm_tp_groups(int M, int N);
int gemm_qkv_direct_ok(int M, int tile, int K);
int gemm_num_cus();
void gemm_set_g4_default(int on);
void gemm_set_g4_group(int gm);
void gemm5_set_diag(int d);
int gemm_argmax(const bf16_t* x, const void* W, float* ws, size_t ws_floats, int M, int N, int K, float rms_eps,
                int32_t* idx, float* val, hipStream_t s, float* rms_ws = nullptr, size_t rms_ws_floats = 0);
size_t gemm_argmax_workspace_floats(int M, int N);
int argmax_partials(const float* part, int P, int M, int32_t* idx, float* val, hipStream_t s);
int gemm_logprob(const bf16_t* x, const void* W, float* ws, size_t ws_floats, int M, int N, int K, float rms_eps,
                 const int32_t* targets, int col_offset, float* tgt, float* mx, float* se, hipStream_t s,
                 float* rms_ws = nullptr, size_t rms_ws_floats = 0);
size_t gemm_logprob_workspace_floats(int M, int N);

int rope_kv_write(const bf16_t* qkv, const float* table, int table_len, const int32_t* positions, bf16_t* kc,
                  bf16_t* vc, const int32_t* slot, int M, int S, int H, int Hkv, int Dh, int T, bf16_t* q_out,
                  hipStream_t s);

const AttnKnobs& attn_knobs();
void attn_reset_knobs();
void attn_set_impl(int impl, int waves_target);
void attn_set_v3_max_pairs(int n);
void attn_set_v3_kpg(int mult);
void attn_set_v5_max_pairs(int n);
void attn_set_v5_fold(int n);
void attn_set_v6(int mode);
void attn_set_v6_wpp(int wpp);
void attn_set_q8_waves(int waves);
void attn_set_q8_splits(int n);
void attn_set_diag(int d);
void attn_set_v6_diag(int d);
unsigned jla_bounds_norm_embed(int reset);
unsigned jla_bounds_rope_kv(int reset);
unsigned jla_bounds_sample(int reset);
unsigned jla_bounds_gemm(int reset);
unsigned jla_bounds_gemv(int reset);
unsigned jla_bounds_attn_decode(int reset);
unsigned jla_bounds_attn_prefill(int reset);
int attn_decode(const bf16_t* q, const bf16_t* kc, const bf16_t* vc, const int32_t* slot, const int32_t* kv_start,
                const uint8_t* key_mask, int mask_len, bf16_t* out, float* ws, int32_t* tickets, int B, int H,
                int Hkv, int Dh, int T, int t_cap, int nsplit, hipStream_t s, bf16_t* out_pack = nullptr);
int attn_decode_v6(const bf16_t* q, const bf16_t* kc, const bf16_t* vc, const int32_t* slot, const int32_t* kv_start,
                   const uint8_t* key_mask, int mask_len, bf16_t* out, int B, int H, int Hkv, int T, int t_cap,
                   int wpp, hipStream_t s, bf16_t* out_pack);
unsigned jla_bounds_kv8(int reset);
int rope_kv_write_q8(const bf16_t* qkv, const float* table, int table_len, const int32_t* positions, uint8_t* kq,
                     float* ks, uint8_t* vq, float* vs, const int32_t* slot, int M, int S, int H, int Hkv, int Dh,
                     int T, bf16_t* q_out, hipStream_t s);
int kv8_dequant(const uint8_t* kq, const float* ks, const uint8_t* vq, const float* vs, bf16_t* kout, bf16_t* vout,
                int pairs, int T, int n, int n_out, hipStream_t s);
int attn_decode_q8(const bf16_t* q, const uint8_t* kq, const float* ks, const uint8_t* vq, const float* vs,
                   const int32_t* slot, const int32_t* kv_start, const uint8_t* key_mask, int mask_len, bf16_t* out,
                   int B, int H, int Hkv, int Dh, int T, int t_cap, hipStream_t s, float* ws = nullptr,
                   size_t ws_floats = 0, int32_t* tickets = nullptr, int n_tickets = 0);
void attn_prefill_set_impl(int impl);
int attn_prefill(const bf16_t* q, const bf16_t* kc, const bf16_t* vc, const int32_t* slot, const int32_t* kv_start,
                 const uint8_t* key_mask, int mask_len, bf16_t* out, int B, int S, int H, int Hkv, int Dh, int T,
                 hipStream_t s);

int argmax(const float* logits, int B, int V, int32_t* idx, float* val, hipStream_t s);
int logprob_rows(const float* logits, int B, int V, const int32_t* targets, int col_offset, float* tgt, float* mx,
                 float* se, hipStream_t s);
int topk_chunks(int V);
int topk_chunk(const float* logits, int B, int V, int K, int idx_offset, float* cv, int32_t* ci, hipStream_t s);
int topk_merge(const float* cv, const int32_t* ci, int B, int C, int K, int mode, float* out_v, int32_t* out_i,
               int32_t* nxt, float temperature, float top_p, uint64_t seed, const int32_t* step, hipStream_t s);
size_t car_buffer_bytes(long long max_bytes, int world);
int car_alloc(long long max_bytes, int world, void** buf, void** sig, hipIpcMemHandle_t* hbuf, hipIpcMemHandle_t* hsig);
void car_free(void* buf, void* sig);
int car_init(int rank, int world, long long max_bytes, void* own_buf, void* own_sig, const hipIpcMemHandle_t* hbufs,
             const hipIpcMemHandle_t* hsigs, double timeout_s, void** state);
int car_reduce(void* state, int op, const void* in, void* out, float* h, bf16_t* hb, long long nbytes, int is_bf16,
               int two_shot, hipStream_t s,
               bf16_t* hb_pack = nullptr, int pack_cols = 0);
int car_pairs(void* state, int mode, const float* a, const int32_t* b, int idx_offset, long long n, int k,
              float* out_a, int32_t* out_b, hipStream_t s);
void car_set_gran_max(long long n);
int car_error(void* state);
const void* car_device(void* state);
long long car_max_bytes(void* state);
int car_world(void* state);
int car_set_grid(void* state, int grid);
void car_destroy(void* state);
int decode_update(const int32_t* nxt, int32_t* finished, int32_t* sequences, int32_t* cur_len, int32_t* tokens,
                  int32_t* positions, int32_t* slot, int B, int L, int pad, int eos, hipStream_t s);
int cu_census(uint32_t* out, int blocks, hipStream_t s);
int cu_mask_stream_create(const uint32_t* mask, int words, hipStream_t* out);
int cu_mask_stream_get(hipStream_t s, uint32_t* mask, int words);
int stream_destroy(hipStream_t s);
int graph_kernel_nodes(hipGraph_t g);

}
```

### jax_llama_amd/models/llama.py

```python
from __future__ import annotations

from dataclasses import dataclass
from typing import Any, Dict, List, Optional, Tuple

import numpy as np
import torch

from .. import ops
from ..config import LLaMAConfig
from ..ops import reference as ref
from ..parallel.comm import NO_COMM, TPComm
from ..parallel.partition import shard_tree
from .kv_cache import KV_FORMATS, KVCache
from .modules import LLaMABlockCollection
from .weights import Fp8Linear, Mxfp4Linear, PackedLinear

BF16 = torch.bfloat16


def _t(x) -> torch.Tensor:
    if torch.is_tensor(x):
        return x
    return torch.as_tensor(np.asarray(x))

# ... 231 lines not shown

    def save_pretrained(self, save_directory: str) -> str:
        from ..utils.native_ckpt import save_pretrained
        return save_pretrained(self, save_directory)

    @classmethod
    def from_pretrained(cls, directory: str, device="cpu", comm: Optional[TPComm] = None):
        from ..utils.native_ckpt import from_pretrained
        return from_pretrained(directory, device=device, comm=comm)

    WEIGHT_FORMATS = ("fp8_e4m3", "mxfp4")

    def quantize_weights_(self, fmt: str = "fp8_e4m3") -> "LLaMAForCausalLM":
        if fmt not in self.WEIGHT_FORMATS:
            raise ValueError(f"quantize_weights_: unknown format {fmt!r} (one of {self.WEIGHT_FORMATS})")
        if self.weight_format != "bf16":
            raise RuntimeError(f"quantize_weights_: the weights are already {self.weight_format}")
        if any(lw.qkv is None for lw in self.layers):
            raise RuntimeError("quantize_weights_: the model has no weights yet")
        names = ("qkv", "o", "gu", "down")
        if fmt == "mxfp4":
            for lw in self.layers:
                for name in names:
                    lin = getattr(lw, name)
                    if lin.n % 16 or lin.k % 128:
                        raise ValueError(f"quantize_weights_('mxfp4'): {name} is {lin.n}x{lin.k}; MXFP4 linear weights "
                                         "need N % 16 == 0 and K % 128 == 0")
        cls = Mxfp4Linear if fmt == "mxfp4" else Fp8Linear
        for lw in self.layers:
            for name in names:
                setattr(lw, name, cls.from_linear(getattr(lw, name)))
        from ..runtime.engine import drop_engines
        drop_engines(self)
        if self.device.type == "cuda":
            torch.cuda.empty_cache()
        return self

    @property
    def weight_format(self) -> str:
        if any(getattr(lw.qkv, "mxfp4", False) for lw in self.layers):
            return "mxfp4"
        return "fp8_e4m3" if any(getattr(lw.qkv, "fp8", False) for lw in self.layers) else "bf16"

    def weight_bytes(self) -> int:
        n = self.wte.numel() * 2 + self.lm_head.nbytes()
        for lw in self.layers:
            n += lw.qkv.nbytes() + lw.o.nbytes() + lw.gu.nbytes() + lw.down.nbytes()
        return n

    def streamed_weight_bytes_per_token(self) -> int:
        return self.weight_bytes() - self.wte.numel() * 2

    KV_CACHE_FORMATS = KV_FORMATS

    def _check_kv_format(self, fmt: str) -> str:
        if fmt not in self.KV_CACHE_FORMATS:
            raise ValueError(f"unknown KV-cache format {fmt!r} (one of {self.KV_CACHE_FORMATS})")
        if fmt == "fp8_e4m3":
            if self.head_dim != 128:
                raise ValueError(f"the fp8_e4m3 KV cache needs head_dim == 128, got {self.head_dim}")
            rep = self.n_heads // self.n_kv_heads
            if self.n_heads % self.n_kv_heads or rep not in (1, 2, 4, 8):
                raise ValueError("the fp8_e4m3 KV cache needs 1, 2, 4 or 8 query heads per kv head, got "
                                 f"{self.n_heads} / {self.n_kv_heads}")
        return fmt

    def set_kv_cache_format(self, fmt: str) -> "LLaMAForCausalLM":
        self._kv_cache_format = self._check_kv_format(fmt)
        return self

    @property
    def kv_cache_format(self) -> str:
        return getattr(self, "_kv_cache_format", "bf16")

    def init_cache(self, batch_size: int, max_length: int, kv_format: Optional[str] = None) -> KVCache:
        if max_length > self.rope_length:
            raise ValueError(f"max_length {max_length} exceeds the RoPE table ({self.rope_length}); "
                             "raise config.max_sequence_length")
        fmt = self.kv_cache_format if kv_format is None else self._check_kv_format(kv_format)
        return KVCache(self.config.num_hidden_layers, batch_size, self.n_kv_heads, max_length,
                       self.head_dim, self.device, kv_format=fmt)

    def _row_parallel(self, x: torch.Tensor, w: PackedLinear, h: torch.Tensor, hb: torch.Tensor,
                      x_packed: Optional[torch.Tensor] = None, mirror_packed: Optional[torch.Tensor] = None) -> None:
        if self.comm.size == 1:
            ops.linear_residual(x, w, h, mirror=hb, x_packed=x_packed, mirror_packed=mirror_packed)
        elif self.comm.linear_residual_(x, w, h, hb, x_packed=x_packed, hb_pack=mirror_packed):
            pass
        else:
            dt = self.comm.partial_dtype(x.numel() // x.shape[-1] * w.n, x.is_cuda)
            part = ops.linear(x, w, out_dtype=dt, x_packed=x_packed)
            self.comm.all_reduce_residual_(part, h, hb, hb_pack=mirror_packed, owned=True)

    def forward_tokens(self, ids: torch.Tensor, positions: torch.Tensor, cache: KVCache, slot0,
                       kv_start: torch.Tensor, key_mask: Optional[torch.Tensor] = None,
                       logits_mode: str = "last", collect_hidden: bool = False,
                       collect_attn: bool = False, targets: Optional[torch.Tensor] = None):
        if (logits_mode == "logprob") != (targets is not None):
            raise ValueError("logits_mode='logprob' takes `targets` (and no other mode does)")
        with ops.autotune.tp_scope(self.comm):
            return self._forward_tokens(ids, positions, cache, slot0, kv_start, key_mask, logits_mode,
                                        collect_hidden, collect_attn, targets)

    def _forward_tokens(self, ids, positions, cache, slot0, kv_start, key_mask, logits_mode, collect_hidden,
                        collect_attn, targets=None):
        b, s = ids.shape
        d = self.config.hidden_size
        hb = torch.empty(b * s, d, dtype=BF16, device=self.device)
        h = ops.embedding(ids.reshape(-1), self.wte, mirror=hb)
        hidden, attns = self.blocks(h, hb, positions, cache, slot0, kv_start, key_mask, s,
                                    output_hidden_states=collect_hidden, output_attentions=collect_attn)
        if logits_mode == "none":
            logits = None
        elif logits_mode == "logprob":
            off = self.tp_rank * self.vocab_local
            if self.precision == "highest":
                logits = ops.linear_f32_logprob(self.final_norm(h), self.lm_head_f32, targets, col_offset=off)
            else:
                logits = ops.linear_logprob(hb, self.lm_head, targets, rms_eps=self.eps, col_offset=off)
        elif self.precision == "highest":
            hl = h if logits_mode == "all" else h.reshape(b, s, d)[:, -1].contiguous()
            logits = ops.linear_f32(self.final_norm(hl), self.lm_head_f32)
            if logits_mode == "argmax":
                logits = ops.argmax(logits.contiguous())
        elif logits_mode == "argmax":
            logits = ops.linear_argmax(hb.reshape(b, s, d)[:, -1].contiguous(), self.lm_head, rms_eps=self.eps)
        else:
            hl = hb if logits_mode == "all" else hb.reshape(b, s, d)[:, -1].contiguous()
            logits = ops.linear(hl, self.lm_head, rms_eps=self.eps, out_dtype=torch.float32)
        return logits, h, hidden, attns

    def gather_logits(self, logits_local: torch.Tensor) -> torch.Tensor:
        if self.comm.size == 1:
            return logits_local
        g = self.comm.all_gather(logits_local)
        return g.permute(1, 0, 2).reshape(logits_local.shape[0], -1)

    def final_norm(self, h: torch.Tensor) -> torch.Tensor:
        return ops.rmsnorm(h, self.ln_f, self.eps)

    def _prepare_call(self, input_ids, attention_mask, position_ids, past_key_values):
        ids = _t(input_ids).to(self.device, torch.int32)
        b, s = ids.shape
        if position_ids is None:
            if past_key_values is not None:
                raise ValueError("Make sure to provide `position_ids` when passing `past_key_values`.")
            position_ids = torch.arange(s, dtype=torch.int32).expand(b, s)
        pos = _t(position_ids).to(self.device, torch.int32).reshape(b, s).contiguous()
        if past_key_values is None:
            cache = KVCache(self.config.num_hidden_layers, b, self.n_kv_heads, s, self.head_dim, self.device,
                            kv_format=self.kv_cache_format)
            slot0 = 0
        else:
            cache = past_key_values
            slot0 = cache.index
            if slot0 + s > cache.max_length:
                raise ValueError(f"cache overflow: {slot0}+{s} > {cache.max_length}")
        t_valid = slot0 + s
        if attention_mask is None:
            mask = torch.ones(b, t_valid, dtype=torch.int32)
        else:
            mask = _t(attention_mask).to("cpu").to(torch.int32)
            if mask.shape[1] >= t_valid:
                mask = mask[:, :t_valid]
            elif mask.shape[1] == s:
                mask = torch.cat([torch.ones(b, slot0, dtype=torch.int32), mask], 1)
            else:
                raise ValueError(f"attention_mask of shape {tuple(mask.shape)} does not cover {t_valid} slots")
        kv_start, key_mask = mask_to_kv_start(mask, self.device)
        return ids, pos, cache, slot0, kv_start, key_mask

    def __call__(self, input_ids, attention_mask=None, position_ids=None, params=None,
                 past_key_values: Optional[KVCache] = None, dropout_rng=None, train: bool = False,
                 output_attentions: Optional[bool] = None, output_hidden_states: Optional[bool] = None,
                 return_dict: Optional[bool] = None):
        if train:
            raise NotImplementedError("inference-only framework (reference dropout/remat paths are training-only)")
        if params is not None and id(params) != self._params_id:
            self.load_params(params)
        oa = self.config.output_attentions if output_attentions is None else output_attentions
        oh = self.config.output_hidden_states if output_hidden_states is None else output_hidden_states
        rd = self.config.return_dict if return_dict is None else return_dict
        ids, pos, cache, slot0, kv_start, key_mask = self._prepare_call(
            input_ids, attention_mask, position_ids, past_key_values)
        b, s = ids.shape
        logits, h, hidden, attns = self.forward_tokens(ids, pos, cache, slot0, kv_start, key_mask,
                                                       logits_mode="all", collect_hidden=oh,
                                                       collect_attn=oa)
        if past_key_values is not None:
            cache.advance(s)
        logits = self.gather_logits(logits).reshape(b, s, -1).to(self.dtype)
        hs = None
        if oh:
            hs = tuple(x.to(self.dtype) for x in hidden) + (self.final_norm(h).reshape(b, s, -1).to(self.dtype),)
        out = CausalLMOutput(logits=logits, past_key_values=past_key_values, hidden_states=hs,
                             attentions=tuple(attns) if oa else None)
        return out if rd else out.to_tuple()

    def score(self, input_ids, attention_mask=None, labels=None, ignore_index: int = -100) -> ScoreOutput:
        from ..runtime import engine as _engine
        ids = _t(input_ids).to("cpu", torch.int64)
        if ids.dim() != 2 or ids.shape[1] < 2:
            raise ValueError(f"score: input_ids must be (B, S) with S >= 2, got {tuple(ids.shape)}")
        b, s = ids.shape
        if s > self.rope_length:
            raise ValueError(f"score: {s} positions exceed the RoPE table ({self.rope_length}); "
                             "raise config.max_sequence_length")
        lab = ids if labels is None else _t(labels).to("cpu", torch.int64)
        if lab.shape != ids.shape:
            raise ValueError(f"score: labels {tuple(lab.shape)} must have input_ids' shape {tuple(ids.shape)}")
        if attention_mask is None:
# ... 86 lines not shown
```

### jax_llama_amd/models/modules.py

```python
from __future__ import annotations

from typing import List, Optional

import torch

from .. import ops
from ..ops import reference as ref


class LLaMAAttention:
    def __init__(self, model, layer_idx: int):
        self.model = model
        self.layer_idx = layer_idx

    @property
    def weights(self):
        return self.model.layers[self.layer_idx]

    def __call__(self, h, hb, positions, cache, slot0, kv_start, key_mask, seq_len: int,
                 output_attentions: bool = False, pk: Optional["PackedActs"] = None) -> Optional[torch.Tensor]:
        m, lw = self.model, self.weights
        kc, vc = cache.layer(self.layer_idx)
        splits = og = 0
        o_state = None
        if not output_attentions:
            og = ops.qkv_attention_o_groups(hb, lw.o, m.n_heads, m.n_kv_heads, kc) if seq_len == 1 else 0
            o_state = m.comm.fused_o_state(hb, lw.o) if og else None
            og = og if o_state is not None else 0
            splits = ops.qkv_attention_splits(hb, lw.qkv, kc, seq_len, m.n_heads, m.n_kv_heads, key_mask, og)
            if og and not splits:
                og = 0
                splits = ops.qkv_attention_splits(hb, lw.qkv, kc, seq_len, m.n_heads, m.n_kv_heads, key_mask)
        if splits:
            hb_p = pk.hb if pk else None
            o = (lw.o, h, hb, hb_p, o_state) if og else None
            att_p = pk.att if pk is not None and not og else None
            a = ops.linear_qkv_attention(hb, lw.qkv, m.eps, m.rope, positions, kc, vc, slot0, kv_start, m.n_heads,
                                         m.n_kv_heads, m.head_dim, splits, x_packed=pk.hb_in() if pk else None,
                                         out_packed=att_p, o=o)
            if not og:
                m._row_parallel(a, lw.o, h, hb, x_packed=att_p, mirror_packed=hb_p)
            if pk is not None and pk.hb is not None:
                pk.hb_ok = True
            return None
        q = ops.linear_qkv_rope(hb, lw.qkv, m.eps, m.rope, positions, kc, vc, slot0, seq_len,
                                m.n_heads, m.n_kv_heads, m.head_dim, x_packed=pk.hb_in() if pk else None)
        b = hb.shape[0] // seq_len
        q4 = q.reshape(b, seq_len, m.n_heads, m.head_dim)
        weights = None
        att_p = None
        if output_attentions:
            s0 = int(slot0) if not torch.is_tensor(slot0) else int(slot0.item())
            kw, vw = (ops.kv8_dequant(kc, vc, s0 + seq_len) if ops.is_fp8_kv(kc) else (kc, vc))
            _, weights = ref.attention(q4, kw, vw, s0, kv_start, key_mask, return_weights=True)
            a = ops.attention(q4, kc, vc, slot0, kv_start, key_mask)
        else:
            att_p = pk.att if pk is not None and ops.attention_packs(q4, kc, key_mask) else None
            a = ops.attention(q4, kc, vc, slot0, kv_start, key_mask, out_packed=att_p)
        m._row_parallel(a, lw.o, h, hb, x_packed=att_p, mirror_packed=pk.hb if pk else None)
        if pk is not None and pk.hb is not None:
            pk.hb_ok = True
        return weights


class LLaMAMLP:
    def __init__(self, model, layer_idx: int):
        self.model = model
        self.layer_idx = layer_idx

    def __call__(self, h, hb, pk: Optional["PackedActs"] = None) -> None:
        m, lw = self.model, self.model.layers[self.layer_idx]
        g = ops.linear_swiglu(hb, lw.gu, rms_eps=m.eps, x_packed=pk.hb_in() if pk else None,
                              out_packed=pk.act if pk else None)

        m._row_parallel(g, lw.down, h, hb, x_packed=pk.act if pk else None, mirror_packed=pk.hb if pk else None)


class LLaMABlock:

    def __init__(self, model, layer_idx: int):
        self.attention = LLaMAAttention(model, layer_idx)
        self.feed_forward = LLaMAMLP(model, layer_idx)

    def __call__(self, h, hb, positions, cache, slot0, kv_start, key_mask, seq_len: int,
                 output_attentions: bool = False, pk: Optional["PackedActs"] = None):
        w = self.attention(h, hb, positions, cache, slot0, kv_start, key_mask, seq_len, output_attentions, pk)
        self.feed_forward(h, hb, pk)
        return w


class PackedActs:

    def __init__(self, rows: int, model, device, full: bool = True):
        self.hb = ops.packed_empty(rows, model.config.hidden_size, device) if full else None
        self.att = ops.packed_empty(rows, model.n_heads * model.head_dim, device)
        self.act = ops.packed_empty(rows, model.ffn, device) if full else None
        self.hb_ok = False

    def hb_in(self) -> Optional[torch.Tensor]:
        return self.hb if self.hb_ok else None


class LLaMABlockCollection:

    def __init__(self, model):
        self.blocks: List[LLaMABlock] = [LLaMABlock(model, i) for i in range(len(model.layers))]
        self.model = model

    def __len__(self):
        return len(self.blocks)

    def __call__(self, h, hb, positions, cache, slot0, kv_start, key_mask, seq_len: int,
                 output_hidden_states: bool = False, output_attentions: bool = False):
        hidden, attns = [], []
        b = hb.shape[0] // seq_len
        rows = hb.shape[0]
        pk = None
        if (ops.PACKED_X and hb.is_cuda and ops.PACKED_X_MIN_M <= rows <= min(ops.PACKED_ATT_MAX_M, ops.SKINNY_M)
                and self.model.comm.packs_residual(rows * self.model.config.hidden_size * 4)):
            pk = PackedActs(rows, self.model, hb.device, full=rows <= ops.PACKED_X_MAX_M)
        for blk in self.blocks:
            if output_hidden_states:
                hidden.append(h.reshape(b, seq_len, -1).clone())
            w = blk(h, hb, positions, cache, slot0, kv_start, key_mask, seq_len, output_attentions, pk)
            if output_attentions:
                attns.append(w)
        return hidden, attns
```

### jax_llama_amd/ops/__init__.py

```python
from __future__ import annotations

import contextlib
import os
from typing import Optional

import torch

from . import autotune
from . import reference as ref
from ._ext import available as ext_available
from ._ext import ext

BF16 = torch.bfloat16

Fp8KV = ref.Fp8KV
is_fp8_kv = ref.is_fp8_kv

MODE_STORE = 0
MODE_RESIDUAL = 1
MODE_SWIGLU = 2
MODE_QKV = 3

GEMV_VARIANT = int(os.environ.get("JLA_GEMV_VARIANT", "0"))


def _is_gpu(t: torch.Tensor) -> bool:
    return t.device.type == "cuda"


class _Workspace:

    def __init__(self):
        self._bufs = {}
        self.generation = 0
        self._scope = ""

    @contextlib.contextmanager
    def scope(self, tag: str):
        prev, self._scope = self._scope, tag + "/"
        try:
            yield
        finally:
            self._scope = prev

    def get(self, name: str, numel: int, dtype: torch.dtype, device: torch.device) -> torch.Tensor:
        key = (self._scope + name, device, dtype)
        buf = self._bufs.get(key)
        if buf is None or buf.numel() < numel:
            buf = torch.empty(max(numel, 1), dtype=dtype, device=device)
            self._bufs[key] = buf
            self.generation += 1
        return buf[:numel]

    def get_zeroed(self, name: str, numel: int, dtype: torch.dtype, device: torch.device) -> torch.Tensor:
        key = ("zeroed:" + self._scope + name, device, dtype)
        buf = self._bufs.get(key)
        if buf is None or buf.numel() < numel:
            buf = torch.zeros(max(numel, 1), dtype=dtype, device=device)
            self._bufs[key] = buf
            self.generation += 1
        return buf[:numel]

    def clear(self):
        self._bufs.clear()
        self.generation += 1


workspace = _Workspace()


def embedding(ids: torch.Tensor, table: torch.Tensor, mirror: Optional[torch.Tensor] = None) -> torch.Tensor:
    if not _is_gpu(table):
        out = ref.embedding(ids, table)
        if mirror is not None:
            mirror.copy_(out.to(BF16))
        return out
    out = torch.empty(ids.numel(), table.shape[1], dtype=torch.float32, device=table.device)
    ext().embedding(ids.reshape(-1).to(torch.int32), table, out, mirror)
    return out


def rms_scale(x: torch.Tensor, eps: float) -> torch.Tensor:
    if not _is_gpu(x):
        return ref.rms_scale(x, eps)
    out = torch.empty(x.shape, dtype=BF16, device=x.device)
    ext().rms_scale(x, out, float(eps))
    return out


def residual_add_(h: torch.Tensor, p: torch.Tensor, mirror: Optional[torch.Tensor] = None) -> torch.Tensor:
    if not _is_gpu(h):
        h.add_(p.float().view_as(h))
        if mirror is not None:
            mirror.copy_(h.to(BF16))
        return h
    assert h.is_contiguous() and h.dtype == torch.float32
    if mirror is None or h.numel() % 8:
        h.add_(p.view_as(h))
        if mirror is not None:
            mirror.copy_(h)
        return h
    ext().residual_add(h, p.contiguous(), mirror)
    return h


PREFETCH_GRID = int(os.environ.get("JLA_PREFETCH_GRID", "128"))


def prefetch(t: torch.Tensor) -> None:
    if _is_gpu(t):
        ext().prefetch(t, PREFETCH_GRID)


def linear_f32(x: torch.Tensor, w: torch.Tensor) -> torch.Tensor:
    if not _is_gpu(x):
        return x.float() @ w.float().t()
    y = torch.empty(x.shape[0], w.shape[0], dtype=torch.float32, device=x.device)
    ext().gemm_f32(x.float().contiguous(), w.float().contiguous(), y)
    return y


def rmsnorm(x: torch.Tensor, weight: torch.Tensor, eps: float) -> torch.Tensor:
    if not _is_gpu(x):
        return ref.rmsnorm(x, weight, eps)
    out = torch.empty(x.shape, dtype=torch.float32, device=x.device)
    ext().rmsnorm(x.float().contiguous(), weight.float().contiguous(), out, float(eps))
    return out


BOUNDS_CODES = {0: "token id outside the vocabulary", 1: "KV-cache write past the cache (slot >= T)",
                2: "decode step past the sequence buffer", 3: "attention asked for keys past the cache",
                4: "position outside the RoPE table"}


class BoundsError(RuntimeError):
    pass


def bounds_error(reset: bool = False) -> int:
    if not ext_available():
        return 0
    return int(ext().bounds_error(bool(reset)))


def check_bounds(reset: bool = True):
    if not ext_available() or not getattr(ext(), "DEBUG_BOUNDS", False):
        return
    err = bounds_error(reset)
    if err:
        raise BoundsError("device-side index out of range: " +
                          "; ".join(v for k, v in BOUNDS_CODES.items() if err >> k & 1))


def linear(x: torch.Tensor, w, rms_eps: Optional[float] = None, out_dtype=BF16,
           out: Optional[torch.Tensor] = None, x_packed: Optional[torch.Tensor] = None) -> torch.Tensor:
    if not _is_gpu(x):
        r = ref.linear(x, w.dense(), rms_eps, out_dtype)
        if out is not None:
            out.copy_(r)
            return out
        return r
    m = x.shape[0]
    if out is None:
        out = torch.empty(m, w.n, dtype=out_dtype, device=x.device)
    _gpu_linear(x, w, out, MODE_STORE, rms_eps, True, None, x_packed)
    return out


def linear_residual(x: torch.Tensor, w, residual: torch.Tensor, rms_eps: Optional[float] = None,
                    accumulate: bool = True, mirror: Optional[torch.Tensor] = None,
                    x_packed: Optional[torch.Tensor] = None, mirror_packed: Optional[torch.Tensor] = None) -> torch.Tensor:
    if not _is_gpu(x):
        ref.linear_residual(x, w.dense(), residual, rms_eps, accumulate)
        if mirror is not None:
            mirror.copy_(residual.to(BF16))
        return residual
    _gpu_linear(x, w, residual, MODE_RESIDUAL, rms_eps, accumulate, mirror, x_packed, mirror_packed)
    return residual


def linear_swiglu(x: torch.Tensor, w, rms_eps: Optional[float] = None, x_packed: Optional[torch.Tensor] = None,
                  out_packed: Optional[torch.Tensor] = None) -> torch.Tensor:
    if not _is_gpu(x):
        return ref.linear_swiglu(x, w.dense(), rms_eps)
    out = torch.empty(x.shape[0], w.n // 2, dtype=BF16, device=x.device)
    _gpu_linear(x, w, out, MODE_SWIGLU, rms_eps, True, None, x_packed, out_packed)
    return out


PACKED_X = os.environ.get("JLA_PACKED_X", "1") != "0"
PACKED_X_MIN_M = int(os.environ.get("JLA_PACKED_X_MIN_M", "9"))
PACKED_X_MAX_M = int(os.environ.get("JLA_PACKED_X_MAX_M", "64"))
PACKED_ATT_MAX_M = int(os.environ.get("JLA_PACKED_ATT_MAX_M", "64"))
SKINNY_M = 64
XP_VARIANTS, SPLIT_VARIANTS = autotune.XP_VARIANTS, autotune.SPLIT_VARIANTS


def packed_rows(m: int) -> int:
    return 16 if m <= 16 else (32 if m <= 32 else 64)


def packed_empty(m: int, cols: int, device) -> torch.Tensor:
    return torch.empty(packed_rows(m), cols, dtype=BF16, device=device)


class _Dequantized:

    def __init__(self, weight, n, k):
        self.weight, self.n, self.k = weight, n, k


def is_fp8(w) -> bool:
    return bool(getattr(w, "fp8", False))


def is_mxfp4(w) -> bool:
    return bool(getattr(w, "mxfp4", False))


def is_quantized(w) -> bool:
    return is_fp8(w) or is_mxfp4(w)


def bf16_weight(w):
    if is_mxfp4(w):
        buf = workspace.get(f"w4_deq_{w.n}x{w.k}", w.n * w.k, BF16, w.device).view(w.n // 16, w.k // 32, 64, 8)
        ext().dequant_fp4(w.qweight, w.scale, w.n, w.k, buf)
        return _Dequantized(buf, w.n, w.k)
    if not is_fp8(w):
        return w
    buf = workspace.get(f"w8_deq_{w.n}x{w.k}", w.n * w.k, BF16, w.device).view(w.n // 16, w.k // 32, 64, 8)
    ext().dequant_fp8(w.qweight, w.scale, w.n, w.k, buf)
    return _Dequantized(buf, w.n, w.k)


def _w8_fast(e, x, w, mode) -> bool:
    return x.shape[0] > 0 and e.gemv_w8_plan_check(x.shape[0], w.n, w.k, mode, x.dtype != BF16)[0] == 0


def _w4_fast(e, x, w, mode) -> bool:
    return x.shape[0] > 0 and e.gemv_w4_plan_check(x.shape[0], w.n, w.k, mode, x.dtype != BF16)[0] == 0


def _gpu_linear(x, w, out, mode, rms_eps, accumulate, mirror=None, x_packed=None, pack_out=None):
    assert x.is_contiguous() and out.is_contiguous()
    assert x.shape[1] == w.k, (x.shape, w.k)
    m = x.shape[0]
    e = ext()
    if is_mxfp4(w):
        if _w4_fast(e, x, w, mode):
            e.linear_skinny_w4(x, w.qweight, w.scale, w.n, w.k, out, mode, -1.0 if rms_eps is None else float(rms_eps),
                               bool(accumulate), mirror, pack_out if mode != MODE_STORE else None)
            return
        w = bf16_weight(w)
    if is_fp8(w):
        if _w8_fast(e, x, w, mode):
            e.linear_skinny_w8(x, w.qweight, w.scale, w.n, w.k, out, mode, -1.0 if rms_eps is None else float(rms_eps),
                               bool(accumulate), mirror, pack_out if mode != MODE_STORE else None)
            return
        w = bf16_weight(w)
    if m > e.SKINNY_MAX_M:
        x_packed = pack_out = None
    v = TILED if m > e.SKINNY_MAX_M else _variant(e, x, w, mode, x_packed, pack_out)
    if v == TILED and pack_out is not None and not _tiled_packs(e, m, w.n, w.k, x.device, mode, rms_eps):
        v = 1
    if v == TILED:
        _tiled(e, x, w.weight, w.n, w.k, out, mode, rms_eps, accumulate, mirror, pack_out)
    else:
        ws, tk = _skinny_ws(e, m, w.n, w.k, mode, x.device)
        e.linear_skinny(x, w.weight, w.n, w.k, out, mode, -1.0 if rms_eps is None else float(rms_eps),
                        bool(accumulate), v, ws, tk, mirror, x_packed if v in XP_VARIANTS else None, pack_out)


def linear_tp_residual(x: torch.Tensor, w, h: torch.Tensor, hb: torch.Tensor, state: int,
                       x_packed: Optional[torch.Tensor] = None, hb_pack: Optional[torch.Tensor] = None) -> torch.Tensor:
    e = ext()
    m = x.shape[0]
    assert x.dtype == BF16 and x.is_contiguous() and m <= e.SKINNY_MAX_M, (x.dtype, x.shape)
    v = _variant(e, x, w, MODE_RESIDUAL, x_packed, pack_out=True)
    if v not in autotune.GEMV_VARIANTS:
        v = 1
    ws = tk = None
    if v in SPLIT_VARIANTS:
        ws, tk = _skinny_ws(e, m, w.n, w.k, MODE_RESIDUAL, x.device)
    e.linear_tp_residual(state, x, w.weight, w.n, w.k, h, hb, v, x_packed if v in XP_VARIANTS else None, hb_pack,
                         ws, tk)
    return h


def tiled_tp_residual(x: torch.Tensor, w, h: torch.Tensor, hb: torch.Tensor, state: int) -> bool:
    e = ext()
    m = x.shape[0]
    assert x.dtype == BF16 and x.is_contiguous(), (x.dtype, x.shape)
    ks, tm = autotune.choose_gemm_plan(e, m, w.n, w.k, x.device, MODE_STORE, False)
    if tm not in autotune.G5_TILES and ks <= 1:
        return False
    ks, tm, ws = _gemm_ws(e, m, w.n, w.k, x.device, MODE_STORE, False)
    e.gemm_tp_residual(state, x, w.weight, w.n, w.k, h, hb, ks, ws, tm)
    return True


TILED = autotune.TILED_VARIANT
QKV_DIRECT = os.environ.get("JLA_QKV_DIRECT", "1") != "0"


def _fused_rms(e, mode, rms_eps) -> bool:
    return rms_eps is not None and mode != MODE_RESIDUAL


def _tiled_input(x, rms_eps, fused=False):
    if rms_eps is not None and not fused:
        return rms_scale(x, rms_eps)
    return x if x.dtype == BF16 else x.to(BF16)


def _gemm_ws(e, m, n, k, device, mode=MODE_STORE, rms=False):
    ks, tm = autotune.choose_gemm_plan(e, m, n, k, device, mode, rms)
    if tm in autotune.G5_TILES:
        eks = e.gemm5_ksplit(k, ks)
        return ks, tm, workspace.get("gemm_ws", eks * m * (n + 1), torch.float32, device)
    ws = workspace.get("gemm_ws", ks * m * (n + 1), torch.float32, device) if ks > 1 else None
    return ks, tm, ws


def _rms_ws(x, fused: bool, ks: int):
    if not fused or ks > 1:
        return None
    return workspace.get("gemm_rms", x.shape[0], torch.float32, x.device)


def _tiled(e, x, weight, n, k, out, mode, rms_eps, accumulate, mirror=None, pack_out=None):
    fused = _fused_rms(e, mode, rms_eps)
    xb = _tiled_input(x, rms_eps, fused)
    ks, tm, ws = _gemm_ws(e, x.shape[0], n, k, x.device, mode, fused)
    e.gemm(xb, weight, n, k, out, mode, bool(accumulate), mirror, ks, ws, float(rms_eps) if fused else -1.0, tm,
           pack_out, _rms_ws(x, fused, ks))


def _tiled_packs(e, m, n, k, device, mode, rms_eps) -> bool:
    if e is None or m > SKINNY_M or mode not in (MODE_RESIDUAL, MODE_SWIGLU):
        return False
    ks, tm = autotune.choose_gemm_plan(e, m, n, k, device, mode, _fused_rms(e, mode, rms_eps))
    if tm in autotune.G5_TILES:
        return True
    return ks > 1


def _variant(e, x, w, mode, x_packed=None, pack_out=None, no_split=False) -> int:
    xp_in, p_out = x_packed is not None, pack_out is not None
    if GEMV_VARIANT:
        v = GEMV_VARIANT
        xp, split = autotune.GEMV_VARIANTS.get(v, (False, False))
        if (xp and not xp_in) or (p_out and v == TILED and not _tiled_packs(
                e, x.shape[0], w.n, w.k, x.device, mode, None if mode == MODE_RESIDUAL else 1e-5)) or (
                split and (no_split or x.dtype != BF16 or w.n // 16 > autotune.SPLIT_MAX_GROUPS)):
            v = 1
        if v == 12 and mode == MODE_SWIGLU:
            v = 15
        return v
    m = x.shape[0]
    pmode = MODE_STORE if mode == MODE_QKV else mode
    ws, tk = _skinny_ws(e, m, w.n, w.k, pmode, x.device)
    ncols = w.n // 2 if pmode == MODE_SWIGLU else w.n
    odt = torch.float32 if pmode == MODE_RESIDUAL else BF16
    scratch = workspace.get("tune_out", m * ncols, odt, x.device).view(m, ncols)
    mirror = workspace.get("tune_mirror", m * ncols, BF16, x.device).view(m, ncols) if (
        p_out and pmode == MODE_RESIDUAL) else None
    pscratch = workspace.get("tune_pack", packed_rows(m) * ncols, BF16, x.device).view(-1, ncols) if p_out else None

    tiled_packs = p_out and _tiled_packs(e, m, w.n, w.k, x.device, pmode, None if pmode == MODE_RESIDUAL else 1e-5)

    def run(v, xx, wt):
        if v == TILED:
            _tiled(e, xx, wt, w.n, w.k, scratch, pmode, None if pmode == MODE_RESIDUAL else 1e-5, True, mirror,
                   pscratch if tiled_packs else None)
        else:
            e.linear_skinny(xx, wt, w.n, w.k, scratch, pmode, 1e-5, True, v, ws, tk, mirror,
                            x_packed if v in XP_VARIANTS else None, pscratch)

    return autotune.choose(e, x, w, pmode, run, xp_in=xp_in, pack_out=p_out, no_split=no_split,
                           tiled_packs=tiled_packs)


_SK_SIZES = {}


def _skinny_ws(e, m, n, k, mode, device):
    key = (m, n, k, mode)
    sz = _SK_SIZES.get(key)
    if sz is None:
        sz = _SK_SIZES[key] = tuple(e.skinny_workspace(m, n))
    floats, tickets = sz
    return (workspace.get("skinny", max(1, floats), torch.float32, device),
            workspace.get_zeroed("skinny_tickets", max(1, tickets), torch.int32, device))


def rope_kv_write(qkv: torch.Tensor, table: torch.Tensor, positions: torch.Tensor,
                  k_cache: torch.Tensor, v_cache: torch.Tensor, slot0, seq_len: int,
                  n_heads: int, n_kv_heads: int, head_dim: int) -> torch.Tensor:
    if not _is_gpu(qkv):
        s0 = int(slot0) if not torch.is_tensor(slot0) else int(slot0.item())
        return ref.rope_kv_write(qkv, table, positions, k_cache, v_cache, s0, seq_len,
                                 n_heads, n_kv_heads, head_dim)
    m = qkv.shape[0]
    q = torch.empty(m, n_heads, head_dim, dtype=BF16, device=qkv.device)
    slot_t = _slot_tensor(slot0, qkv.device)
    if is_fp8_kv(k_cache) or is_fp8_kv(v_cache):
        _check_kv8_pair(k_cache, v_cache)
        ext().rope_kv_write_q8(qkv, table, positions.reshape(-1).to(torch.int32), k_cache.q, k_cache.scale, v_cache.q,
                               v_cache.scale, slot_t, int(seq_len), int(n_heads), int(n_kv_heads), int(head_dim), q)
        return q
    ext().rope_kv_write(qkv, table, positions.reshape(-1).to(torch.int32), k_cache, v_cache,
                        slot_t, int(seq_len), int(n_heads), int(n_kv_heads), int(head_dim), q)
    return q


def linear_qkv_rope(x: torch.Tensor, w, rms_eps: Optional[float], table: torch.Tensor, positions: torch.Tensor,
                    k_cache: torch.Tensor, v_cache: torch.Tensor, slot0, seq_len: int, n_heads: int,
                    n_kv_heads: int, head_dim: int, x_packed: Optional[torch.Tensor] = None) -> torch.Tensor:
    if not _is_gpu(x):
        s0 = int(slot0) if not torch.is_tensor(slot0) else int(slot0.item())
        return ref.linear_qkv_rope(x, w.dense(), rms_eps, table, positions, k_cache, v_cache, s0, seq_len,
                                   n_heads, n_kv_heads, head_dim)
    m = x.shape[0]
    e = ext()
    if is_fp8_kv(k_cache) or is_fp8_kv(v_cache):
        qkv = linear(x, w, rms_eps=rms_eps, x_packed=x_packed if m <= e.SKINNY_MAX_M else None)
        return rope_kv_write(qkv, table, positions, k_cache, v_cache, slot0, seq_len, n_heads, n_kv_heads, head_dim)
    if is_mxfp4(w):
        if _w4_fast(e, x, w, MODE_QKV):
            q = torch.empty(m, n_heads, head_dim, dtype=BF16, device=x.device)
            e.linear_qkv_w4(x, w.qweight, w.scale, w.n, w.k, -1.0 if rms_eps is None else float(rms_eps), table,
                            positions.reshape(-1).to(torch.int32), k_cache, v_cache, _slot_tensor(slot0, x.device),
                            int(seq_len), int(n_heads), int(n_kv_heads), int(head_dim), q)
            return q
        w = bf16_weight(w)
    if is_fp8(w):
        if _w8_fast(e, x, w, MODE_QKV):
            q = torch.empty(m, n_heads, head_dim, dtype=BF16, device=x.device)
            e.linear_qkv_w8(x, w.qweight, w.scale, w.n, w.k, -1.0 if rms_eps is None else float(rms_eps), table,
                            positions.reshape(-1).to(torch.int32), k_cache, v_cache, _slot_tensor(slot0, x.device),
                            int(seq_len), int(n_heads), int(n_kv_heads), int(head_dim), q)
            return q
        w = bf16_weight(w)
    if m > e.SKINNY_MAX_M:
        x_packed = None
    v = TILED if m > e.SKINNY_MAX_M else _variant(e, x, w, MODE_QKV, x_packed)
    if v == TILED:
        ks, tm, ws = _gemm_ws(e, m, w.n, w.k, x.device, MODE_STORE, _fused_rms(e, MODE_QKV, rms_eps))
        fused = _fused_rms(e, MODE_QKV, rms_eps)
        if ks == 1 and fused and QKV_DIRECT and e.gemm_qkv_direct_ok(m, tm, w.k):
            q = torch.empty(m, n_heads, head_dim, dtype=BF16, device=x.device)
            e.gemm_qkv(_tiled_input(x, rms_eps, fused), w.weight, w.n, w.k, table, positions.reshape(-1).to(torch.int32),
                       k_cache, v_cache, _slot_tensor(slot0, x.device), int(seq_len), int(n_heads), int(n_kv_heads),
                       int(head_dim), q, 1, None, float(rms_eps), tm, _rms_ws(x, fused, 1))
            return q
        if ks == 1:
            qkv = linear(x, w, rms_eps=rms_eps)
            return rope_kv_write(qkv, table, positions, k_cache, v_cache, slot0, seq_len, n_heads, n_kv_heads,
                                 head_dim)
        q = torch.empty(m, n_heads, head_dim, dtype=BF16, device=x.device)
        e.gemm_qkv(_tiled_input(x, rms_eps, fused), w.weight, w.n, w.k, table, positions.reshape(-1).to(torch.int32),
                   k_cache, v_cache, _slot_tensor(slot0, x.device), int(seq_len), int(n_heads), int(n_kv_heads),
                   int(head_dim), q, ks, ws, float(rms_eps) if fused else -1.0, tm)
        return q
    q = torch.empty(m, n_heads, head_dim, dtype=BF16, device=x.device)
    ws, tk = _skinny_ws(e, m, w.n, w.k, MODE_QKV, x.device)
    e.linear_qkv(x, w.weight, w.n, w.k, -1.0 if rms_eps is None else float(rms_eps), table,
                 positions.reshape(-1).to(torch.int32), k_cache, v_cache, _slot_tensor(slot0, x.device),
                 int(seq_len), int(n_heads), int(n_kv_heads), int(head_dim), q, v, ws, tk,
                 x_packed if v in XP_VARIANTS else None)
    return q


QKV_ATTN = int(os.environ.get("JLA_QKV_ATTN", "1"))
QKV_ATTN_SPL = int(os.environ.get("JLA_QKV_ATTN_SPL", "2"))
QKV_ATTN_O = int(os.environ.get("JLA_QKV_ATTN_O", "0"))
_CUS = {}


class InLaunchTimeout(RuntimeError):
    """An in-launch wait gave up (the fused qkv + attention launch: a qkv workgroup never published)."""


def check_inlaunch() -> None:
    global QKV_ATTN
    for (name, _dev, _dt), buf in list(workspace._bufs.items()):
        if name.startswith("zeroed:") and name.endswith("qa_sync") and buf.is_cuda and int(buf[2].item()):
            QKV_ATTN = 0
            buf.zero_()
            workspace.generation += 1
            raise InLaunchTimeout("fused qkv + attention launch: a wait timed out (the attention workgroups on the qkv "
                                  "workgroups, or the o workgroups on the attention ones; error word qa_sync[2]); the "
                                  "fused path is now off for this process")


def _num_cus(device) -> int:
    key = str(device)
    if key not in _CUS:
        _CUS[key] = torch.cuda.get_device_properties(device).multi_processor_count
    return _CUS[key]


def qkv_attention_o_groups(x: torch.Tensor, w_o, n_heads: int, n_kv_heads: int, k_cache=None) -> int:
    if not QKV_ATTN_O or not _is_gpu(x) or is_quantized(w_o) or is_fp8_kv(k_cache):
        return 0
    return int(ext().qkv_attn_o_groups(x.shape[0], n_heads // n_kv_heads, w_o.n, w_o.k))


def qkv_attention_splits(x: torch.Tensor, w, k_cache: torch.Tensor, seq_len: int, n_heads: int, n_kv_heads: int,
                         key_mask: Optional[torch.Tensor] = None, o_groups: int = 0) -> int:
    if not QKV_ATTN or seq_len != 1 or key_mask is not None or not _is_gpu(x) or x.dtype != BF16 or is_quantized(w):
        return 0
    if is_fp8_kv(k_cache):
        return 0
    m = x.shape[0]
    if QKV_ATTN == 1 and (m > 4 or n_heads < 8 * n_kv_heads):
        return 0
    return int(ext().qkv_attn_splits(m, m, n_kv_heads, n_heads // n_kv_heads, k_cache.shape[2], w.n,
                                     _num_cus(x.device), 1, int(o_groups)))


def _qkv_attention_spl(e, m, w, k_cache, n_heads, n_kv_heads, device, o_groups=0) -> int:
    if QKV_ATTN_SPL > 1 and e.qkv_attn_splits(m, m, n_kv_heads, n_heads // n_kv_heads, k_cache.shape[2], w.n,
                                               _num_cus(device), 2, int(o_groups)) > 0:
        return 2
    return 1


def linear_qkv_attention(x: torch.Tensor, w, rms_eps: Optional[float], table: torch.Tensor, positions: torch.Tensor,
                         k_cache: torch.Tensor, v_cache: torch.Tensor, slot0, kv_start: torch.Tensor, n_heads: int,
                         n_kv_heads: int, head_dim: int, splits: int, x_packed: Optional[torch.Tensor] = None,
                         out_packed: Optional[torch.Tensor] = None, spl: Optional[int] = None,
                         o: Optional[tuple] = None) -> torch.Tensor:
    e = ext()
    m = x.shape[0]
    dev = x.device
    rep = n_heads // n_kv_heads
    q = workspace.get("qa_q", m * n_heads * head_dim, BF16, dev).view(m, n_heads, head_dim)
    out = torch.empty(m, n_heads * head_dim, dtype=BF16, device=dev)
    ws = workspace.get("qa_ws", m * n_kv_heads * splits * rep * (head_dim + 4), torch.float32, dev)
    tickets = workspace.get_zeroed("qa_tickets", max(m * n_kv_heads, 64), torch.int32, dev)
    sync = workspace.get_zeroed("qa_sync", int(e.qkv_attn_sync_ints()), torch.int32, dev)
    og = 0 if o is None else int(e.qkv_attn_o_groups(m, rep, o[0].n, o[0].k))
    spl = _qkv_attention_spl(e, m, w, k_cache, n_heads, n_kv_heads, dev, og) if spl is None else int(spl)
    sk_ws = sk_tk = None
    if spl > 1:
        sk_ws, sk_tk = _skinny_ws(e, m, w.n, w.k, MODE_QKV, dev)
    ow = oh = ohb = ohp = None
    on = ok = 0
    tp_state = 0
    if o is not None:
        wo, oh, ohb, ohp, tp_state = o
        ow, on, ok = wo.weight, wo.n, wo.k
    e.linear_qkv_attn(x, w.weight, w.n, w.k, -1.0 if rms_eps is None else float(rms_eps), table,
                      positions.reshape(-1).to(torch.int32), k_cache, v_cache, _slot_tensor(slot0, dev), n_heads,
                      n_kv_heads, head_dim, q, kv_start, out, out_packed, ws, tickets, sync, k_cache.shape[2], splits,
                      x_packed, spl, sk_ws, sk_tk, ow, on, ok, oh, ohb, ohp, int(tp_state or 0))
    return out


def attention_packs(q: torch.Tensor, k_cache: torch.Tensor, key_mask: Optional[torch.Tensor] = None) -> bool:
    bsz, s, h, dh = q.shape
    if s != 1 or is_fp8_kv(k_cache):
        return False
    rc, _why, _kernel, _nsplit, packs, *_ = ext().attn_decode_plan_check(
        bsz, h, k_cache.shape[1], dh, k_cache.shape[2], key_mask is not None)
    return rc == 0 and bool(packs)


def attention(q: torch.Tensor, k_cache: torch.Tensor, v_cache: torch.Tensor, slot0, kv_start: torch.Tensor,
              key_mask: Optional[torch.Tensor] = None, max_kv: Optional[int] = None,
              out_packed: Optional[torch.Tensor] = None) -> torch.Tensor:
    bsz, s, h, dh = q.shape
    if not _is_gpu(q):
        s0 = int(slot0) if not torch.is_tensor(slot0) else int(slot0.item())
        return ref.attention(q, k_cache, v_cache, s0, kv_start, key_mask).reshape(bsz * s, h * dh)
    out = torch.empty(bsz * s, h * dh, dtype=BF16, device=q.device)
    slot_t = _slot_tensor(slot0, q.device)
    t_cap = int(max_kv) if max_kv is not None else k_cache.shape[2]
    e = ext()
    if is_fp8_kv(k_cache) or is_fp8_kv(v_cache):
        _check_kv8_pair(k_cache, v_cache)
        if out_packed is not None:
            raise ValueError("attention: no packed output copy with an Fp8KV cache (attention_packs)")
        if s == 1:
            _rc, _why, nsplit, ws_floats, n_tickets = e.attn_decode_q8_split_check(
                bsz, h, k_cache.shape[1], dh, t_cap, key_mask is not None)
            ws = tickets = None
            if nsplit > 1:
                ws = workspace.get("attn_q8", ws_floats, torch.float32, q.device)
                tickets = workspace.get_zeroed("attn_q8_tickets", n_tickets, torch.int32, q.device)
            e.attn_decode_q8(q, k_cache.q, k_cache.scale, v_cache.q, v_cache.scale, slot_t, kv_start, key_mask, out,
                             t_cap, ws, tickets)
        else:
            n = k_cache.shape[2] if torch.is_tensor(slot0) else min(int(slot0) + s, k_cache.shape[2])
            kd, vd = kv8_dequant(k_cache, v_cache, n, scratch=True)
            e.attn_prefill(q, kd, vd, slot_t, kv_start, key_mask, out)
        return out
    if s == 1:
        hkv = k_cache.shape[1]
        _rc, _why, _kernel, nsplit, _packs, ws_floats, n_tickets, *_ = e.attn_decode_plan_check(
            bsz, h, hkv, dh, t_cap, key_mask is not None)
        ws = workspace.get("attn_decode", ws_floats, torch.float32, q.device)
        tickets = workspace.get_zeroed("attn_tickets", n_tickets, torch.int32, q.device)
        e.attn_decode(q, k_cache, v_cache, slot_t, kv_start, key_mask, out, ws, tickets, t_cap, nsplit, out_packed)
    else:
        e.attn_prefill(q, k_cache, v_cache, slot_t, kv_start, key_mask, out)
    return out


def _check_kv8_pair(k_cache, v_cache) -> None:
    if not (is_fp8_kv(k_cache) and is_fp8_kv(v_cache)):
        raise TypeError("FP8 KV cache: K and V must both be Fp8KV")


def kv8_dequant(k_cache: "Fp8KV", v_cache: "Fp8KV", n: Optional[int] = None, scratch: bool = False):
    _check_kv8_pair(k_cache, v_cache)
    b, hkv, t, dh = k_cache.shape
    n = t if n is None else int(n)
    if not _is_gpu(k_cache.q):
        return k_cache.dequant(n), v_cache.dequant(n)
    numel = b * hkv * n * dh
    if scratch:
        kd = workspace.get("kv8_k", numel, BF16, k_cache.device).view(b, hkv, n, dh)
        vd = workspace.get("kv8_v", numel, BF16, k_cache.device).view(b, hkv, n, dh)
    else:
        kd = torch.empty(b, hkv, n, dh, dtype=BF16, device=k_cache.device)
        vd = torch.empty_like(kd)
    ext().kv8_dequant(k_cache.q, k_cache.scale, v_cache.q, v_cache.scale, n, kd, vd)
    return kd, vd


def _slot_tensor(slot0, device):
    if torch.is_tensor(slot0):
        return slot0
    t = torch.tensor([int(slot0)], dtype=torch.int32, device=device)
    return t


def argmax(logits: torch.Tensor):
    if not _is_gpu(logits):
        v, i = logits.float().max(-1)
        return ref.argmax(logits), v
    b = logits.shape[0]
    idx = torch.empty(b, dtype=torch.int32, device=logits.device)
    val = torch.empty(b, dtype=torch.float32, device=logits.device)
    ext().argmax(logits, idx, val)
    return idx, val


ARGMAX_FUSED_MIN_M = 256
SKINNY_ARGMAX = os.environ.get("JLA_SKINNY_ARGMAX", "1") != "0"


def linear_argmax(x: torch.Tensor, w, rms_eps: Optional[float] = None):
    m = x.shape[0]
    if not _is_gpu(x):
        return argmax(linear(x, w, rms_eps, out_dtype=torch.float32))
    w = bf16_weight(w)
    if m <= ext().SKINNY_MAX_M and SKINNY_ARGMAX:
        e = ext()
        v = _variant(e, x, w, MODE_STORE, no_split=True)
        if v in autotune.ROW_MAJOR_VARIANTS and v != 10:
            part = workspace.get("skinny_argmax", m * (w.n // 16) * 2, torch.float32, x.device)
            idx = torch.empty(m, dtype=torch.int32, device=x.device)
            val = torch.empty(m, dtype=torch.float32, device=x.device)
            e.linear_skinny_argmax(x, w.weight, w.n, w.k, -1.0 if rms_eps is None else float(rms_eps), v, part, idx,
                                   val)
            return idx, val
    if m < ARGMAX_FUSED_MIN_M:
        return argmax(linear(x, w, rms_eps, out_dtype=torch.float32))
    e = ext()
    assert x.is_contiguous() and x.shape[1] == w.k, (x.shape, w.k)
    xb = x if x.dtype == BF16 else x.to(BF16)
    ws = workspace.get("gemm_argmax", e.gemm_argmax_workspace(m, w.n), torch.float32, x.device)
    idx = torch.empty(m, dtype=torch.int32, device=x.device)
    val = torch.empty(m, dtype=torch.float32, device=x.device)
    e.gemm_argmax(xb, w.weight, w.n, w.k, ws, -1.0 if rms_eps is None else float(rms_eps), idx, val,
                  _rms_ws(x, rms_eps is not None, 1))
    return idx, val


MODE_LOGPROB = 10
LOGPROB_CHUNK_BYTES = 256 << 20


def logprob(logits: torch.Tensor, targets: torch.Tensor, col_offset: int = 0):
    if not _is_gpu(logits):
        return ref.logprob(logits, targets, col_offset)
    assert logits.dim() == 2 and logits.dtype == torch.float32 and logits.is_contiguous(), (logits.shape, logits.dtype)
    m = logits.shape[0]
    out = torch.empty(3, m, dtype=torch.float32, device=logits.device)
    ext().logprob_rows(logits, targets.reshape(-1).to(torch.int32), int(col_offset), out[0], out[1], out[2])
    return out[0], out[1], out[2]


def logprob_fused(x: torch.Tensor, w, rms_eps: Optional[float] = None) -> bool:
    if not _is_gpu(x) or x.shape[0] < ARGMAX_FUSED_MIN_M:
        return False
    rms = rms_eps is not None
    return ext().gemm_plan_check(x.shape[0], w.n, w.k, MODE_LOGPROB, rms, 1, 0, rms) == 0


def _logprob_chunks(m: int, n: int):
    rows = max(1, LOGPROB_CHUNK_BYTES // (4 * n))
    return [(r0, min(m, r0 + rows)) for r0 in range(0, m, rows)]


def linear_logprob(x: torch.Tensor, w, targets: torch.Tensor, rms_eps: Optional[float] = None, col_offset: int = 0):
    if not _is_gpu(x):
        return ref.linear_logprob(x, w.dense(), targets, rms_eps, col_offset)
    w = bf16_weight(w)
    m = x.shape[0]
    assert x.is_contiguous() and x.shape[1] == w.k, (x.shape, w.k)
    tg = targets.reshape(-1).to(torch.int32)
    assert tg.numel() == m, (tg.shape, m)
    out = torch.empty(3, m, dtype=torch.float32, device=x.device)
    if logprob_fused(x, w, rms_eps):
        e = ext()
        xb = x if x.dtype == BF16 else x.to(BF16)
        ws = workspace.get("gemm_logprob", e.gemm_logprob_workspace(m, w.n), torch.float32, x.device)
        e.gemm_logprob(xb, w.weight, w.n, w.k, ws, -1.0 if rms_eps is None else float(rms_eps), tg, int(col_offset),
                       out[0], out[1], out[2], _rms_ws(x, rms_eps is not None, 1))
    else:
        for r0, r1 in _logprob_chunks(m, w.n):
            logits = linear(x[r0:r1], w, rms_eps, out_dtype=torch.float32)
            ext().logprob_rows(logits, tg[r0:r1], int(col_offset), out[0, r0:r1], out[1, r0:r1], out[2, r0:r1])
    return out[0], out[1], out[2]


def linear_f32_logprob(x: torch.Tensor, w: torch.Tensor, targets: torch.Tensor, col_offset: int = 0):
    m = x.shape[0]
    tg = targets.reshape(-1).to(torch.int32)
    parts = [logprob(linear_f32(x[r0:r1], w), tg[r0:r1], col_offset) for r0, r1 in _logprob_chunks(m, w.shape[0])]
    return tuple(torch.cat([p[i] for p in parts]) for i in range(3))


def logprob_combine(tgt: torch.Tensor, mx: torch.Tensor, se: torch.Tensor):
    if tgt.dim() == 1:
        tgt, mx, se = tgt[None], mx[None], se[None]
    tgt, mx, se = tgt.float(), mx.float(), se.float()
    big = mx.max(0).values
    safe = torch.where(torch.isinf(big), torch.zeros_like(big), big)
    total = torch.zeros_like(big)
    t = torch.zeros_like(big)
    for r in range(mx.shape[0]):
        total = total + se[r] * torch.exp(mx[r] - safe)
        t = t + tgt[r]
    lse = big + torch.log(total)
    return t - lse, lse, t == big


SAMPLER_MAX_K = 64


def topk_candidates(logits: torch.Tensor, k: int, idx_offset: int = 0):
    if not _is_gpu(logits):
        v, i = ref.topk_sorted(logits, k)
        return v, i + idx_offset
    e = ext()
    b, v = logits.shape
    c = e.topk_chunks(v) * k
    cv = workspace.get("topk_cv", b * c, torch.float32, logits.device).view(b, c)
    ci = workspace.get("topk_ci", b * c, torch.int32, logits.device).view(b, c)
    e.topk_chunk(logits, k, int(idx_offset), cv, ci)
    out_v = torch.empty(b, k, dtype=torch.float32, device=logits.device)
    out_i = torch.empty(b, k, dtype=torch.int32, device=logits.device)
    e.topk_merge(cv, ci, k, 0, out_v=out_v, out_i=out_i)
    return out_v, out_i


def topk_sample(logits: torch.Tensor, k: int, temperature: float, top_p: float, seed: int,
                step: torch.Tensor, comm=None) -> torch.Tensor:
    b, v = logits.shape
    tp = comm.size if comm is not None else 1
    if not _is_gpu(logits):
        if tp > 1:
            full = comm.all_gather(logits.float().contiguous()).permute(1, 0, 2).reshape(b, -1)
        else:
            full = logits
        return ref.topk_sample(full, k, temperature, 1.0 if top_p is None else top_p, seed, int(step.reshape(-1)[0]))
    e = ext()
    kl = min(k, v)
    c = e.topk_chunks(v) * kl
    cv = workspace.get("topk_cv", b * c, torch.float32, logits.device).view(b, c)
    ci = workspace.get("topk_ci", b * c, torch.int32, logits.device).view(b, c)
    e.topk_chunk(logits, kl, int(comm.rank * v) if tp > 1 else 0, cv, ci)
    if tp > 1:
        lv = torch.empty(b, kl, dtype=torch.float32, device=logits.device)
        li = torch.empty(b, kl, dtype=torch.int32, device=logits.device)
        e.topk_merge(cv, ci, kl, 0, out_v=lv, out_i=li)
        cv, ci = comm.gather_topk(lv, li)
    nxt = torch.empty(b, dtype=torch.int32, device=logits.device)
    e.topk_merge(cv, ci, k, 1, nxt=nxt, temperature=float(temperature),
                 top_p=1.0 if top_p is None else float(top_p), seed=int(seed) & ((1 << 63) - 1), step=step)
    return nxt
```

### jax_llama_amd/runtime/engine.py

```python
from __future__ import annotations

import dataclasses
import os
from collections import OrderedDict
from dataclasses import dataclass
from typing import Optional

import torch

from .. import ops
from ..models.kv_cache import kv_row_bytes
from ..ops import reference as ref

_NEG_INF = float("-inf")


@dataclass
class GenerationConfig:

    max_length: Optional[int] = None
    max_new_tokens: Optional[int] = None
    do_sample: bool = False
    temperature: float = 1.0
    top_k: int = 50
# ... 82 lines not shown
        self.finished = torch.zeros(batch_size, **i32)
        self.cur_len = torch.zeros(1, **i32)
        self.sequences = torch.zeros(batch_size, max_length, **i32)
        self.key_mask: Optional[torch.Tensor] = None
        self._key_mask_buf: Optional[torch.Tensor] = None
        self._graph = None
        self._graph_key = None
        self.keep_graph = False
        self._gen: Optional[torch.Generator] = None
        self.gc: Optional[GenerationConfig] = None

    def _next_token(self, logits_local):
        if self.gc.do_sample:
            return _sample(self.model, logits_local, self.gc, self._gen, self.cur_len)
        return _greedy(self.model, logits_local)

    def _update(self, nxt: torch.Tensor):
        if self.device.type == "cuda":
            ops.ext().decode_update(nxt, self.finished, self.sequences, self.cur_len, self.tokens,
                                    self.positions, self.cache.index_t, int(self.gc.pad_token_id),
                                    int(self.gc.eos_token_id))
            return
        fin = self.finished.bool()
        nxt = torch.where(fin, torch.full_like(nxt, self.gc.pad_token_id), nxt)
        self.finished.copy_((fin | (nxt == self.gc.eos_token_id)).to(torch.int32))
        cl = int(self.cur_len.item())
        if cl < self.max_length:
            self.sequences[:, cl] = nxt
        self.tokens[:, 0] = nxt
        self.positions.add_(1)
        self.cache.index_t.add_(1)
        self.cur_len.add_(1)

    def _logits_mode(self) -> str:
        return "argmax" if _fused_greedy() and not self.gc.do_sample else "last"

    def _decode_step(self):
        logits, *_ = self.model.forward_tokens(self.tokens, self.positions, self.cache, self.cache.index_t,
                                               self.kv_start, self.key_mask, logits_mode=self._logits_mode())
        self._update(self._next_token(logits))

    def prefill(self, input_ids: torch.Tensor, attention_mask: Optional[torch.Tensor]):
        model, dev = self.model, self.device
        ids = input_ids.to(dev, torch.int32)
        b, s = ids.shape
        assert b == self.b and s < self.max_length
        if attention_mask is None:
            mask = torch.ones(b, s, dtype=torch.int32)
        else:
            mask = attention_mask.to("cpu", torch.int32)
        positions = (mask.cumsum(-1) - 1).to(torch.int32)
        ext_mask = torch.ones(b, self.max_length, dtype=torch.int32)
        ext_mask[:, :s] = mask
        from ..models.llama import mask_to_kv_start
        kv_start, key_mask = mask_to_kv_start(ext_mask, dev)
        self.kv_start.copy_(kv_start)
        if key_mask is not None:
            if self._key_mask_buf is None:
                self._key_mask_buf = torch.empty_like(key_mask)
            self._key_mask_buf.copy_(key_mask)
            key_mask = self._key_mask_buf
        self.key_mask = key_mask
        self.cache.reset()
        self.sequences.fill_(self.gc.pad_token_id)
        self.sequences[:, :s] = ids
        self.finished.zero_()
        pos_dev = positions.to(dev)
        logits = self._prefill_rows(ids, pos_dev)
        self.cache.advance(s)
        self.cur_len.fill_(s)
        nxt = self._next_token(logits)
        self.positions.copy_(pos_dev[:, -1:])
        self.cache.index_t.sub_(1)
        self._update(nxt)
        self.cache.index = s
        return s + 1

    def _prefill_rows(self, ids: torch.Tensor, pos_dev: torch.Tensor):
        b, s = ids.shape
        rows = max(1, PREFILL_TOKENS // max(1, s))
        mode = self._logits_mode()
        if b <= rows:
            logits, *_ = self.model.forward_tokens(ids, pos_dev, self.cache, 0, self.kv_start, self.key_mask,
                                                   logits_mode=mode)
            return logits
        parts = []
        for b0 in range(0, b, rows):
            b1 = min(b, b0 + rows)
            km = self.key_mask[b0:b1] if self.key_mask is not None else None
            lg, *_ = self.model.forward_tokens(ids[b0:b1], pos_dev[b0:b1], self.cache.rows(b0, b1), 0,
                                               self.kv_start[b0:b1], km, logits_mode=mode)
            parts.append(lg)
        if isinstance(parts[0], tuple):
            return tuple(torch.cat([p[i] for p in parts]) for i in range(len(parts[0])))
        return torch.cat(parts)

    def prefill_only(self, input_ids, attention_mask, gc: GenerationConfig) -> int:
        self.gc = gc
        return self.prefill(input_ids, attention_mask)

    def _graph_state(self):
        gc = self.gc
        sampler = (gc.top_k, gc.temperature, gc.top_p, int(gc.seed)) if gc.do_sample else None
        return (gc.do_sample, self.key_mask is not None, ops.workspace.generation, _fused_greedy(),
                ops.ARGMAX_FUSED_MIN_M, ops.SKINNY_ARGMAX, ops.QKV_ATTN, self.model.comm.reduce_dtype,
                int(gc.pad_token_id), int(gc.eos_token_id), sampler)

    def _ensure_graph(self):
        if self._graph is not None and self._graph_key == self._graph_state():
            return
        for _ in range(3):
            key = self._graph_state()
            torch.cuda.synchronize(self.device)
            g = torch.cuda.CUDAGraph(keep_graph=self.keep_graph)
            with torch.cuda.graph(g):
                self._decode_step()
            self._graph, self._graph_key = g, key
            if self._graph_state() == key:
                return
        raise RuntimeError("decode graph capture keeps reallocating workspaces")

    def _poll(self) -> bool:
        done = bool(self.finished.all().item())
        self._check()
        return done

    def _check(self):
        self.model.comm.check()
        if self.device.type == "cuda":
            ops.check_inlaunch()
        ops.check_bounds()

    def run(self, input_ids, attention_mask, gc: GenerationConfig) -> torch.Tensor:
        self.gc = gc
        rng_saved = None
        if gc.do_sample:
            self._gen = torch.Generator(device=self.device)
            self._gen.manual_seed(int(gc.seed))
            if self.use_graph:
                self._gen = None
                if self.device.type == "cuda":
                    rng_saved = torch.cuda.get_rng_state(self.device)
                    torch.cuda.manual_seed(int(gc.seed))
        try:
            return self._run(input_ids, attention_mask)
        except Exception:
            self.cache.zero_()
            raise
        finally:
            if rng_saved is not None:
                torch.cuda.set_rng_state(rng_saved, self.device)

    def _run(self, input_ids, attention_mask) -> torch.Tensor:
        cur = self.prefill(input_ids, attention_mask)
        steps_left = self.max_length - cur
        done = steps_left <= 0
        first = True
        step = 0
        while not done:
            if self.use_graph and not first:
                self._ensure_graph()
                self._graph.replay()
            else:
                self._decode_step()
                first = False
            step += 1
            steps_left -= 1
            if steps_left <= 0:
                break
            if step % self.check_every == 0 and self._poll():
                break
        self._check()
        return self.sequences


_ENGINES: "OrderedDict" = OrderedDict()


def _engine_budget(model) -> int:
    env = os.environ.get("JLA_ENGINE_CACHE_GB")
    if env:
        return int(float(env) * (1 << 30))
    if model.device.type == "cuda":
        return int(0.4 * torch.cuda.get_device_properties(model.device).total_memory)
    return 8 << 30


def drop_engines(model) -> int:
# ... 51 lines not shown
```

Before: 41400 tokens/s.

## Fuse RMS row statistics into split-K residual reduce and reuse in next GEMM

Adds a split-K residual reduce kernel that also computes each row's RMS inverse norm from the bf16 mirror while writing the residual. Python-side bookkeeping records which mirror tensor has a valid precomputed stat, so the following norm-fused GEMM (QKV, MLP, argmax, logprob) can skip its separate rms_rowinv launch. Prefill also passes last_rows_only so logits are computed only for the final rows. The change adds state tracking keyed on data_ptr and version, which could go stale and yield wrong norms, and the reduce kernel now does one row per wave, which may lower parallelism for small M.

```diff
diff --git a/jax_llama_amd/csrc/bindings.cpp b/jax_llama_amd/csrc/bindings.cpp
--- a/jax_llama_amd/csrc/bindings.cpp
+++ b/jax_llama_amd/csrc/bindings.cpp
@@ -474,9 +474,10 @@
   return ptr<float>(*rws);
 }
 
-void gemm(Tensor x, Tensor w, int64_t n, int64_t k, Tensor out, int64_t mode, bool accumulate,
+bool gemm(Tensor x, Tensor w, int64_t n, int64_t k, Tensor out, int64_t mode, bool accumulate,
           c10::optional<Tensor> mirror, int64_t ksplit, c10::optional<Tensor> ws, double rms_eps, int64_t tile,
-          c10::optional<Tensor> pack_out, c10::optional<Tensor> rms_ws, int64_t n_body) {
+          c10::optional<Tensor> pack_out, c10::optional<Tensor> rms_ws, int64_t n_body, bool rms_ready,
+          c10::optional<Tensor> rowstat, double rowstat_eps) {
   check_gpu(x, "x");
   check_packed(w, n, k);
   check(n_body >= 0 && (n_body == 0 || jla::gemm_tail_width((int)tile) > 0), "gemm n_body: tail-balanced tiles only");
@@ -495,16 +496,48 @@
   const bool slabs = check_gemm_ws(ws, k, ksplit, m, n, rms_eps >= 0, tile);
   size_t rfl = 0;
   float* rws = rms_ws_ptr(rms_ws, m, &rfl);
+  check(!rms_ready || rws, "gemm rms_ready: needs rms_ws");
+  size_t sfl = 0;
+  float* stat = rms_ws_ptr(rowstat, m, &sfl);
+  const bool writes = stat && jla::gemm_writes_rowstat(m, n, k, mode, ksplit, tile, mir != nullptr);
   gemm_rc(jla::gemm(cbf(x), w.data_ptr(), out.data_ptr(), m, n, k, mode, accumulate,
                     out.scalar_type() == torch::kFloat32, mir, pqa.pack ? &pqa : nullptr,
                     slabs ? ptr<float>(*ws) : nullptr, slabs ? ws->numel() : 0, ksplit, stream(), (float)rms_eps,
-                    (int)tile, rws, rfl, (int)n_body),
+                    (int)tile, rws, rfl, (int)n_body, rms_ready, writes ? stat : nullptr, (float)rowstat_eps),
           "gemm");
+  return writes;
+}
+
+void reduce_residual(Tensor ws, int64_t ksplit, Tensor h, Tensor mirror, bool accumulate,
+                     c10::optional<Tensor> pack_out, c10::optional<Tensor> rowstat, double rowstat_eps) {
+  check_gpu(ws, "ws");
+  check_gpu(h, "h");
+  check(h.dim() == 2 && h.scalar_type() == torch::kFloat32 && ws.scalar_type() == torch::kFloat32, "reduce_residual: "
+        "fp32 h [M, N] and slabs");
+  const int64_t m = h.size(0), n = h.size(1);
+  check(ksplit >= 1 && ws.numel() >= ksplit * m * n && n % 4 == 0, "reduce_residual: ksplit * M * N slab floats, N % 4");
+  jla::bf16_t* mir = mirror_ptr(mirror, h.numel());
+  check(mir != nullptr, "reduce_residual: the bf16 mirror");
+  check(!pack_out.has_value() || m <= SKINNY_MAX_M, "reduce_residual pack_out: decode M");
+  size_t sfl = 0;
+  float* stat = rms_ws_ptr(rowstat, m, &sfl);
+  check(!stat || n % 8 == 0, "reduce_residual rowstat: N % 8 == 0");
+  rc(jla::gemm_reduce_residual(ptr<float>(ws), (int)ksplit, ptr<float>(h), mir, packed_ptr(pack_out, m, n, "pack_out"),
+                               (int)m, (int)n, accumulate, stat, (float)rowstat_eps, stream()),
+     "reduce_residual");
+}
+
+void rms_rowinv(Tensor x, Tensor inv, double eps) {
+  check_gpu(x, "x");
+  check(x.dim() == 2 && x.scalar_type() == torch::kBFloat16 && x.size(1) % 8 == 0, "rms_rowinv: bf16 [M, D], D % 8");
+  size_t fl = 0;
+  float* p = rms_ws_ptr(inv, x.size(0), &fl);
+  rc(jla::rms_rowinv(cbf(x), p, (int)x.size(0), (int)x.size(1), (float)eps, stream()), "rms_rowinv");
 }
 
 void gemm_qkv(Tensor x, Tensor w, int64_t n, int64_t k, Tensor table, Tensor positions, Tensor kc, Tensor vc,
               Tensor slot, int64_t seq_len, int64_t h, int64_t hkv, int64_t dh, Tensor q, int64_t ksplit,
-              c10::optional<Tensor> ws, double rms_eps, int64_t tile, c10::optional<Tensor> rms_ws) {
+              c10::optional<Tensor> ws, double rms_eps, int64_t tile, c10::optional<Tensor> rms_ws, bool rms_ready) {
   check_gpu(x, "x");
   check_packed(w, n, k);
   check(x.dim() == 2 && x.size(1) == k && x.scalar_type() == torch::kBFloat16, "x must be bf16 [M, K]");
@@ -515,7 +548,7 @@
   float* rws = rms_ws_ptr(rms_ws, m, &rfl);
   gemm_rc(jla::gemm(cbf(x), w.data_ptr(), nullptr, m, n, k, MODE_QKV, 0, 0, nullptr, &qa,
                     slabs ? ptr<float>(*ws) : nullptr, slabs ? ws->numel() : 0, ksplit, stream(), (float)rms_eps,
-                    (int)tile, rws, rfl),
+                    (int)tile, rws, rfl, 0, rms_ready && rws),
           "gemm_qkv");
 }
 
@@ -706,7 +739,7 @@
 }
 
 void gemm_argmax(Tensor x, Tensor w, int64_t n, int64_t k, Tensor ws, double rms_eps, Tensor idx, Tensor val,
-                 c10::optional<Tensor> rms_ws) {
+                 c10::optional<Tensor> rms_ws, bool rms_ready) {
   check_gpu(x, "x");
   check_packed(w, n, k);
   check(x.dim() == 2 && x.size(1) == k && x.scalar_type() == torch::kBFloat16, "x must be bf16 [M, K]");
@@ -722,7 +755,7 @@
   size_t rfl = 0;
   float* rws = rms_ws_ptr(rms_ws, m, &rfl);
   rc(jla::gemm_argmax(cbf(x), w.data_ptr(), ptr<float>(ws), ws.numel(), m, n, k, (float)rms_eps, ptr<int32_t>(idx),
-                      ptr<float>(val), stream(), rws, rfl),
+                      ptr<float>(val), stream(), rws, rfl, rms_ready && rws),
      "gemm_argmax");
 }
 
@@ -736,7 +769,8 @@
 }
 
 void gemm_logprob(Tensor x, Tensor w, int64_t n, int64_t k, Tensor ws, double rms_eps, Tensor targets,
-                  int64_t col_offset, Tensor tgt, Tensor mx, Tensor se, c10::optional<Tensor> rms_ws) {
+                  int64_t col_offset, Tensor tgt, Tensor mx, Tensor se, c10::optional<Tensor> rms_ws,
+                  bool rms_ready) {
   check_gpu(x, "x");
   check_packed(w, n, k);
   check(x.dim() == 2 && x.size(1) == k && x.scalar_type() == torch::kBFloat16, "x must be bf16 [M, K]");
@@ -749,7 +783,7 @@
   float* rws = rms_ws_ptr(rms_ws, m, &rfl);
   gemm_rc(jla::gemm_logprob(cbf(x), w.data_ptr(), ptr<float>(ws), ws.numel(), m, n, k, (float)rms_eps,
                             ptr<int32_t>(targets), (int)col_offset, ptr<float>(tgt), ptr<float>(mx), ptr<float>(se),
-                            stream(), rws, rfl),
+                            stream(), rws, rfl, rms_ready && rws),
           "gemm_logprob");
 }
 
@@ -979,7 +1013,12 @@
   m.def("gemm", &gemm, py::arg("x"), py::arg("w"), py::arg("n"), py::arg("k"), py::arg("out"), py::arg("mode"),
         py::arg("accumulate"), py::arg("mirror") = py::none(), py::arg("ksplit") = 1, py::arg("ws") = py::none(),
         py::arg("rms_eps") = -1.0, py::arg("tile") = 0, py::arg("pack_out") = py::none(),
-        py::arg("rms_ws") = py::none(), py::arg("n_body") = 0);
+        py::arg("rms_ws") = py::none(), py::arg("n_body") = 0, py::arg("rms_ready") = false,
+        py::arg("rowstat") = py::none(), py::arg("rowstat_eps") = 0.0);
+  m.def("reduce_residual", &reduce_residual, py::arg("ws"), py::arg("ksplit"), py::arg("h"), py::arg("mirror"),
+        py::arg("accumulate"), py::arg("pack_out") = py::none(), py::arg("rowstat") = py::none(),
+        py::arg("rowstat_eps") = 0.0);
+  m.def("rms_rowinv", &rms_rowinv, py::arg("x"), py::arg("inv"), py::arg("eps"));
   m.def("gemm_tail_split", [](int64_t tiles_m, int64_t n, int64_t width, int64_t cus) {
     const int nb = jla::gemm_tail_split((int)tiles_m, (int)n, (int)width, cus > 0 ? (int)cus : jla::gemm_num_cus());
     return std::make_pair((int64_t)nb, nb > 0 ? (n - nb * width + 127) / 128 : (int64_t)0);
@@ -989,6 +1028,11 @@
     return jla::gemm_plan_check((int)m, (int)n, (int)k, (int)mode, rms, (int)ksplit, (int)tile, has_rms_ws, (int)n_body);
   }, py::arg("m"), py::arg("n"), py::arg("k"), py::arg("mode"), py::arg("rms"), py::arg("ksplit"), py::arg("tile"),
      py::arg("has_rms_ws"), py::arg("n_body") = 0);
+  m.def("gemm_plan_g4_unsplit", [](int64_t m, int64_t n, int64_t k, int64_t mode, bool rms, int64_t ksplit,
+                                   int64_t tile, bool has_rms_ws) {
+    return jla::gemm_plan_g4_unsplit((int)m, (int)n, (int)k, (int)mode, rms, (int)ksplit, (int)tile, has_rms_ws) != 0;
+  }, py::arg("m"), py::arg("n"), py::arg("k"), py::arg("mode"), py::arg("rms"), py::arg("ksplit"), py::arg("tile"),
+     py::arg("has_rms_ws"));
   m.def("gemv_plan_check", [](int64_t m, int64_t n, int64_t k, int64_t mode, bool x_f32, bool x_packed,
                               int64_t variant) {
     const jla::GemvPlanResult r = jla::gemv_plan((int)m, (int)n, (int)k, (int)mode, x_f32, x_packed, (int)variant);
@@ -1032,13 +1076,14 @@
   m.def("gemm_qkv", &gemm_qkv, py::arg("x"), py::arg("w"), py::arg("n"), py::arg("k"), py::arg("table"),
         py::arg("positions"), py::arg("kc"), py::arg("vc"), py::arg("slot"), py::arg("seq_len"), py::arg("h"),
         py::arg("hkv"), py::arg("dh"), py::arg("q"), py::arg("ksplit"), py::arg("ws"), py::arg("rms_eps") = -1.0,
-        py::arg("tile") = 0, py::arg("rms_ws") = py::none());
+        py::arg("tile") = 0, py::arg("rms_ws") = py::none(), py::arg("rms_ready") = false);
   m.def("gemm_argmax", &gemm_argmax, py::arg("x"), py::arg("w"), py::arg("n"), py::arg("k"), py::arg("ws"),
-        py::arg("rms_eps"), py::arg("idx"), py::arg("val"), py::arg("rms_ws") = py::none());
+        py::arg("rms_eps"), py::arg("idx"), py::arg("val"), py::arg("rms_ws") = py::none(),
+        py::arg("rms_ready") = false);
   m.def("gemm_argmax_workspace", [](int64_t m, int64_t n) { return (int64_t)jla::gemm_argmax_workspace_floats(m, n); });
   m.def("gemm_logprob", &gemm_logprob, py::arg("x"), py::arg("w"), py::arg("n"), py::arg("k"), py::arg("ws"),
         py::arg("rms_eps"), py::arg("targets"), py::arg("col_offset"), py::arg("tgt"), py::arg("mx"), py::arg("se"),
-        py::arg("rms_ws") = py::none());
+        py::arg("rms_ws") = py::none(), py::arg("rms_ready") = false);
   m.def("gemm_logprob_workspace",
         [](int64_t m, int64_t n) { return (int64_t)jla::gemm_logprob_workspace_floats(m, n); });
   m.def("logprob_rows", &logprob_rows);
diff --git a/jax_llama_amd/csrc/kernels/gemm.hip b/jax_llama_amd/csrc/kernels/gemm.hip
--- a/jax_llama_amd/csrc/kernels/gemm.hip
+++ b/jax_llama_amd/csrc/kernels/gemm.hip
@@ -1072,6 +1072,103 @@
   }
 }
 
+JLA_DEV void rowstat_piece(const float4 (&v)[2], int row, int i, int N, float* __restrict__ out,
+                           bf16_t* __restrict__ mirror, bf16_t* __restrict__ pack, float& s0, float& s1) {
+  const size_t idx = (size_t)row * N + (size_t)i * 8;
+  float4* o = reinterpret_cast<float4*>(out + idx);
+  o[0] = v[0];
+  o[1] = v[1];
+  const u32x4 pk = {pack2bf(v[0].x, v[0].y), pack2bf(v[0].z, v[0].w), pack2bf(v[1].x, v[1].y),
+                    pack2bf(v[1].z, v[1].w)};
+  *reinterpret_cast<u32x4*>(mirror + idx) = pk;
+  if (pack) *reinterpret_cast<u32x4*>(pack + pack_off(row, i * 8, N)) = pk;
+#pragma unroll
+  for (int e = 0; e < 4; ++e) {
+    const float lo = __uint_as_float(pk[e] << 16), hi = __uint_as_float(pk[e] & 0xffff0000u);
+    s0 = fmaf(lo, lo, s0);
+    s1 = fmaf(hi, hi, s1);
+  }
+}
+
+template <int KS>
+__global__ void __launch_bounds__(256)
+    gemm_reduce_rowstat_kernel(const float* __restrict__ ws, int ksplit, float* __restrict__ out, int M, int N,
+                               int accumulate, bf16_t* __restrict__ mirror, bf16_t* __restrict__ pack,
+                               float* __restrict__ inv, float eps) {
+  const int row = blockIdx.x * 4 + (threadIdx.x >> 6), lane = threadIdx.x & 63;
+  if (row >= M) return;
+  const size_t slab4 = (size_t)M * N / 4;
+  const int pieces = N >> 3;
+  float s0 = 0.f, s1 = 0.f;
+  if constexpr (KS == 0) {
+    for (int i = lane; i < pieces; i += 64) {
+      const size_t e4 = ((size_t)row * N + (size_t)i * 8) >> 2;
+      float4 v[2] = {sum_splits(ws, ksplit, slab4, e4), sum_splits(ws, ksplit, slab4, e4 + 1)};
+      if (accumulate) {
+        const float4* o = reinterpret_cast<const float4*>(out) + e4;
+#pragma unroll
+        for (int j = 0; j < 2; ++j) {
+          float4 r = o[j];
+          r.x += v[j].x;
+          r.y += v[j].y;
+          r.z += v[j].z;
+          r.w += v[j].w;
+          v[j] = r;
+        }
+      }
+      rowstat_piece(v, row, i, N, out, mirror, pack, s0, s1);
+    }
+  } else {
+    constexpr int U = 4;
+    for (int i0 = lane; i0 < pieces; i0 += 64 * U) {
+      float4 q[U][KS][2], r[U][2];
+#pragma unroll
+      for (int u = 0; u < U; ++u) {
+        const int i = min(i0 + 64 * u, pieces - 1);
+        const size_t e4 = ((size_t)row * N + (size_t)i * 8) >> 2;
+        const float4* p = reinterpret_cast<const float4*>(ws) + e4;
+#pragma unroll
+        for (int k = 0; k < KS; ++k) {
+          q[u][k][0] = p[(size_t)k * slab4];
+          q[u][k][1] = p[(size_t)k * slab4 + 1];
+        }
+        if (accumulate) {
+          r[u][0] = reinterpret_cast<const float4*>(out)[e4];
+          r[u][1] = reinterpret_cast<const float4*>(out)[e4 + 1];
+        }
+      }
+#pragma unroll
+      for (int u = 0; u < U; ++u) {
+        const int i = i0 + 64 * u;
+        if (i >= pieces) break;
+        float4 v[2];
+#pragma unroll
+        for (int j = 0; j < 2; ++j) {
+          v[j] = q[u][0][j];
+#pragma unroll
+          for (int k = 1; k < KS; ++k) {
+            v[j].x += q[u][k][j].x;
+            v[j].y += q[u][k][j].y;
+            v[j].z += q[u][k][j].z;
+            v[j].w += q[u][k][j].w;
+          }
+          if (accumulate) {
+            float4 t = r[u][j];
+            t.x += v[j].x;
+            t.y += v[j].y;
+            t.z += v[j].z;
+            t.w += v[j].w;
+            v[j] = t;
+          }
+        }
+        rowstat_piece(v, row, i, N, out, mirror, pack, s0, s1);
+      }
+    }
+  }
+  const float t = wave_sum(s0 + s1);
+  if (lane == 0) inv[row] = 1.f / sqrtf(t / (float)N + eps);
+}
+
 constexpr int TPR_ELEMS = 4096;
 static_assert(TPR_ELEMS / 2 * 8 == TPRES_REGION, "one fused-exchange region per workgroup");
 __global__ void __launch_bounds__(256)
@@ -1183,6 +1280,14 @@
   return gemm_plan(M, N, K, mode, rms != 0, ksplit, tile, has_rms_ws != 0, n_body, num_cus(), g_g4_default).rc;
 }
 
+int gemm_plan_g4_unsplit(int M, int N, int K, int mode, int rms, int ksplit, int tile, int has_rms_ws) {
+  const GemmPlanResult r =
+      gemm_plan(M, N, K, mode, rms != 0, ksplit, tile, has_rms_ws != 0, 0, num_cus(), g_g4_default);
+  const GemmPlan& p = r.plan;
+  return r.rc == 0 && !p.reduce && p.norm != NORM_INLOOP &&
+         (p.family == GEMM4 || p.family == GEMM4_PERSISTENT || p.family == GEMM4_TAIL);
+}
+
 struct GemmArgs {
   const bf16_t* x;
   const u32x4* w;
@@ -1194,11 +1299,13 @@
   float* rms_ws;
   QKVArgs qa;
   hipStream_t s;
+  bool rms_ready = false;
 };
 
 static bool g4_row_stat(const GemmArgs& a, const GemmPlan& p, const float*& inv) {
   inv = p.norm == NORM_PRECOMPUTED ? a.rms_ws : nullptr;
-  return inv == nullptr || rms_rowinv(a.x, a.rms_ws, a.M, a.K, a.rms_eps, a.s) == 0;
+  if (inv == nullptr || a.rms_ready) return true;
+  return rms_rowinv(a.x, a.rms_ws, a.M, a.K, a.rms_eps, a.s) == 0;
 }
 
 static int g_g4_group = 0;
@@ -1370,9 +1477,27 @@
   }
 }
 
+int gemm_reduce_rowstat_ok(int mode, int N, bool mirror) { return mode == MODE_RESIDUAL && mirror && N % 8 == 0; }
+
 static int launch_reduce(const float* ws, int ksplit, void* out, int M, int N, int K, int mode, int accumulate,
                          int out_f32, bf16_t* mirror, const QKVArgs* qkv, const float* ssq, float rms_eps,
-                         hipStream_t s) {
+                         hipStream_t s, float* rowstat = nullptr, float rowstat_eps = 0.f) {
+  if (gemm_reduce_rowstat_ok(mode, N, mirror != nullptr) && rowstat) {
+#define JLA_ROWSTAT(KS)                                                                                         \
+  gemm_reduce_rowstat_kernel<KS><<<(M + 3) / 4, 256, 0, s>>>(ws, ksplit, static_cast<float*>(out), M, N, accumulate, \
+                                                             mirror, qkv ? qkv->pack : nullptr, rowstat, rowstat_eps)
+    if (ksplit == 2)
+      JLA_ROWSTAT(2);
+    else if (ksplit == 3)
+      JLA_ROWSTAT(3);
+    else if (ksplit == 4)
+      JLA_ROWSTAT(4);
+    else
+      JLA_ROWSTAT(0);
+#undef JLA_ROWSTAT
+    JLA_CHECK_LAUNCH();
+    return 0;
+  }
   const size_t total4 = (size_t)M * N / (mode == MODE_SWIGLU ? 8 : 4);
   const int rgrid = (int)((total4 + 255) / 256);
   QKVArgs qa{};
@@ -1408,7 +1533,8 @@
 
 int gemm(const bf16_t* x, const void* W, void* out, int M, int N, int K, int mode, int accumulate, int out_f32,
          bf16_t* mirror, const QKVArgs* qkv, float* ws, size_t ws_floats, int ksplit, hipStream_t s,
-         float rms_eps, int tile, float* rms_ws, size_t rms_ws_floats, int n_body) {
+         float rms_eps, int tile, float* rms_ws, size_t rms_ws_floats, int n_body, int rms_ready, float* rowstat,
+         float rowstat_eps) {
   const bool has_rms_ws = rms_ws != nullptr && rms_ws_floats >= (size_t)M;
   const GemmPlanResult r =
       gemm_plan(M, N, K, mode, rms_eps >= 0.f, ksplit, tile, has_rms_ws, n_body, num_cus(), g_g4_default);
@@ -1418,6 +1544,7 @@
   const u32x4* w = static_cast<const u32x4*>(W);
   if (!p.reduce) {
     GemmArgs a{x, w, out, M, N, K, accumulate, out_f32, nullptr, rms_eps, nullptr, rms_ws, QKVArgs{}, s};
+    a.rms_ready = rms_ready != 0;
     switch (mode) {
       case MODE_QKV:
         a.out = nullptr, a.accumulate = a.out_f32 = 0, a.qa = *qkv;
@@ -1442,7 +1569,23 @@
   float* ssq = p.norm != NORM_NONE ? ws + slabs : nullptr;
   launch_plan<MODE_PARTIAL>(GemmArgs{x, w, ws, M, N, K, 0, 1, nullptr, rms_eps, ssq, nullptr, QKVArgs{}, s}, p);
   JLA_CHECK_LAUNCH();
-  return launch_reduce(ws, p.ksplit, out, M, N, K, mode, accumulate, out_f32, mirror, qkv, ssq, rms_eps, s);
+  return launch_reduce(ws, p.ksplit, out, M, N, K, mode, accumulate, out_f32, mirror, qkv, ssq, rms_eps, s, rowstat,
+                       rowstat_eps);
+}
+
+int gemm_writes_rowstat(int M, int N, int K, int mode, int ksplit, int tile, int mirror) {
+  const GemmPlanResult r = gemm_plan(M, N, K, mode, false, ksplit, tile, false, 0, num_cus(), g_g4_default);
+  return r.rc == 0 && r.plan.family != GEMM_NONE && r.plan.reduce && gemm_reduce_rowstat_ok(mode, N, mirror != 0);
+}
+
+int gemm_reduce_residual(const float* ws, int ksplit, float* h, bf16_t* mirror, bf16_t* pack, int M, int N,
+                         int accumulate, float* rowstat, float rowstat_eps, hipStream_t s) {
+  if (M <= 0) return 0;
+  if (ksplit < 1 || (N & 3) || (rowstat && !gemm_reduce_rowstat_ok(MODE_RESIDUAL, N, mirror != nullptr))) return -1;
+  QKVArgs qa{};
+  qa.pack = pack;
+  return launch_reduce(ws, ksplit, h, M, N, 0, MODE_RESIDUAL, accumulate, 1, mirror, &qa, nullptr, -1.f, s, rowstat,
+                       rowstat_eps);
 }
 
 JLA_DEV void amax_merge(float& bv, int& bi, float ov, int oi) {
@@ -1513,14 +1656,14 @@
 size_t gemm_argmax_workspace_floats(int M, int N) { return (size_t)M * ((N + G2_BN - 1) / G2_BN) * 4 * 2; }
 
 int gemm_argmax(const bf16_t* x, const void* W, float* ws, size_t ws_floats, int M, int N, int K, float rms_eps,
-                int32_t* idx, float* val, hipStream_t s, float* rms_ws, size_t rms_ws_floats) {
+                int32_t* idx, float* val, hipStream_t s, float* rms_ws, size_t rms_ws_floats, int rms_ready) {
   const bool has_rms_ws = rms_ws != nullptr && rms_ws_floats >= (size_t)M;
   const GemmPlanResult r = gemm_plan(M, N, K, MODE_ARGMAX, rms_eps >= 0.f, 1, 0, has_rms_ws, 0, 0, g_g4_default);
   if (r.rc != 0 || r.plan.family == GEMM_NONE) return r.rc;
   if (ws == nullptr || ws_floats < gemm_argmax_workspace_floats(M, N)) return -3;
-  launch_plan<MODE_ARGMAX>(
-      GemmArgs{x, static_cast<const u32x4*>(W), ws, M, N, K, 0, 1, nullptr, rms_eps, nullptr, rms_ws, QKVArgs{}, s},
-      r.plan);
+  launch_plan<MODE_ARGMAX>(GemmArgs{x, static_cast<const u32x4*>(W), ws, M, N, K, 0, 1, nullptr, rms_eps, nullptr,
+                                    rms_ws, QKVArgs{}, s, rms_ready != 0},
+                           r.plan);
   JLA_CHECK_LAUNCH();
   const int P = (N + G2_BN - 1) / G2_BN * (r.plan.family == GEMM4 ? 2 : 4);
   launch_argmax_partials(reinterpret_cast<const float2*>(ws), P, M, idx, val, s);
@@ -1597,7 +1740,7 @@
 
 int gemm_logprob(const bf16_t* x, const void* W, float* ws, size_t ws_floats, int M, int N, int K, float rms_eps,
                  const int32_t* targets, int col_offset, float* tgt, float* mx, float* se, hipStream_t s,
-                 float* rms_ws, size_t rms_ws_floats) {
+                 float* rms_ws, size_t rms_ws_floats, int rms_ready) {
   const bool has_rms_ws = rms_ws != nullptr && rms_ws_floats >= (size_t)M;
   const GemmPlanResult r = gemm_plan(M, N, K, MODE_LOGPROB, rms_eps >= 0.f, 1, 0, has_rms_ws, 0, 0, g_g4_default);
   if (r.rc != 0 || r.plan.family == GEMM_NONE) return r.rc;
@@ -1607,6 +1750,7 @@
   if (zeroed != hipSuccess) return (int)zeroed;
   GemmArgs a{x, static_cast<const u32x4*>(W), ws, M, N, K, 0, 1, nullptr, rms_eps, nullptr, rms_ws, QKVArgs{}, s};
   a.qa.lp_targets = targets, a.qa.lp_tgt = tgt, a.qa.lp_col_offset = col_offset;
+  a.rms_ready = rms_ready != 0;
   launch_plan<MODE_LOGPROB>(a, r.plan);
   JLA_CHECK_LAUNCH();
   launch_lse_partials(reinterpret_cast<const float2*>(ws), (N + G4_BN - 1) / G4_BN * 2, M, mx, se, s);
diff --git a/jax_llama_amd/csrc/kernels/launchers.h b/jax_llama_amd/csrc/kernels/launchers.h
--- a/jax_llama_amd/csrc/kernels/launchers.h
+++ b/jax_llama_amd/csrc/kernels/launchers.h
@@ -72,8 +72,13 @@
 int clock_probe(int iters, int grid, unsigned long long* out, hipStream_t s);
 int gemm(const bf16_t* x, const void* W, void* out, int M, int N, int K, int mode, int accumulate, int out_f32,
          bf16_t* mirror, const QKVArgs* qkv, float* ws, size_t ws_floats, int ksplit, hipStream_t s,
-         float rms_eps = -1.f, int tile = 0, float* rms_ws = nullptr, size_t rms_ws_floats = 0, int n_body = 0);
+         float rms_eps = -1.f, int tile = 0, float* rms_ws = nullptr, size_t rms_ws_floats = 0, int n_body = 0,
+         int rms_ready = 0, float* rowstat = nullptr, float rowstat_eps = 0.f);
+int gemm_writes_rowstat(int M, int N, int K, int mode, int ksplit, int tile, int mirror);
+int gemm_reduce_residual(const float* ws, int ksplit, float* h, bf16_t* mirror, bf16_t* pack, int M, int N,
+                         int accumulate, float* rowstat, float rowstat_eps, hipStream_t s);
 int gemm_plan_check(int M, int N, int K, int mode, int rms, int ksplit, int tile, int has_rms_ws, int n_body);
+int gemm_plan_g4_unsplit(int M, int N, int K, int mode, int rms, int ksplit, int tile, int has_rms_ws);
 int gemm_ksplit(int M, int N, int K);
 size_t gemm_workspace_floats(int M, int N, int K);
 int gemm_tp_groups(int M, int N);
@@ -83,12 +88,13 @@
 void gemm_set_g4_group(int gm);
 void gemm5_set_diag(int d);
 int gemm_argmax(const bf16_t* x, const void* W, float* ws, size_t ws_floats, int M, int N, int K, float rms_eps,
-                int32_t* idx, float* val, hipStream_t s, float* rms_ws = nullptr, size_t rms_ws_floats = 0);
+                int32_t* idx, float* val, hipStream_t s, float* rms_ws = nullptr, size_t rms_ws_floats = 0,
+                int rms_ready = 0);
 size_t gemm_argmax_workspace_floats(int M, int N);
 int argmax_partials(const float* part, int P, int M, int32_t* idx, float* val, hipStream_t s);
 int gemm_logprob(const bf16_t* x, const void* W, float* ws, size_t ws_floats, int M, int N, int K, float rms_eps,
                  const int32_t* targets, int col_offset, float* tgt, float* mx, float* se, hipStream_t s,
-                 float* rms_ws = nullptr, size_t rms_ws_floats = 0);
+                 float* rms_ws = nullptr, size_t rms_ws_floats = 0, int rms_ready = 0);
 size_t gemm_logprob_workspace_floats(int M, int N);
 
 int rope_kv_write(const bf16_t* qkv, const float* table, int table_len, const int32_t* positions, bf16_t* kc,
diff --git a/jax_llama_amd/models/llama.py b/jax_llama_amd/models/llama.py
--- a/jax_llama_amd/models/llama.py
+++ b/jax_llama_amd/models/llama.py
@@ -337,9 +337,11 @@
                        self.head_dim, self.device, kv_format=fmt)
 
     def _row_parallel(self, x: torch.Tensor, w: PackedLinear, h: torch.Tensor, hb: torch.Tensor,
-                      x_packed: Optional[torch.Tensor] = None, mirror_packed: Optional[torch.Tensor] = None) -> None:
+                      x_packed: Optional[torch.Tensor] = None, mirror_packed: Optional[torch.Tensor] = None,
+                      stat_eps: Optional[float] = None) -> None:
         if self.comm.size == 1:
-            ops.linear_residual(x, w, h, mirror=hb, x_packed=x_packed, mirror_packed=mirror_packed)
+            ops.linear_residual(x, w, h, mirror=hb, x_packed=x_packed, mirror_packed=mirror_packed,
+                                mirror_stat_eps=stat_eps)
         elif self.comm.linear_residual_(x, w, h, hb, x_packed=x_packed, hb_pack=mirror_packed):
             pass
         else:
@@ -350,21 +352,27 @@
     def forward_tokens(self, ids: torch.Tensor, positions: torch.Tensor, cache: KVCache, slot0,
                        kv_start: torch.Tensor, key_mask: Optional[torch.Tensor] = None,
                        logits_mode: str = "last", collect_hidden: bool = False,
-                       collect_attn: bool = False, targets: Optional[torch.Tensor] = None):
+                       collect_attn: bool = False, targets: Optional[torch.Tensor] = None,
+                       last_rows_only: bool = False):
         if (logits_mode == "logprob") != (targets is not None):
             raise ValueError("logits_mode='logprob' takes `targets` (and no other mode does)")
         with ops.autotune.tp_scope(self.comm):
             return self._forward_tokens(ids, positions, cache, slot0, kv_start, key_mask, logits_mode,
-                                        collect_hidden, collect_attn, targets)
+                                        collect_hidden, collect_attn, targets, last_rows_only)
 
     def _forward_tokens(self, ids, positions, cache, slot0, kv_start, key_mask, logits_mode, collect_hidden,
-                        collect_attn, targets=None):
+                        collect_attn, targets=None, last_rows_only=False):
         b, s = ids.shape
         d = self.config.hidden_size
         hb = torch.empty(b * s, d, dtype=BF16, device=self.device)
         h = ops.embedding(ids.reshape(-1), self.wte, mirror=hb)
-        hidden, attns = self.blocks(h, hb, positions, cache, slot0, kv_start, key_mask, s,
-                                    output_hidden_states=collect_hidden, output_attentions=collect_attn)
+        hidden, attns, last = self.blocks(h, hb, positions, cache, slot0, kv_start, key_mask, s,
+                                          output_hidden_states=collect_hidden, output_attentions=collect_attn,
+                                          last_rows=last_rows_only and logits_mode in ("last", "argmax"))
+        if last is not None:
+            h_last, hb_last = last
+        elif logits_mode in ("last", "argmax"):
+            h_last, hb_last = h.reshape(b, s, d)[:, -1], hb.reshape(b, s, d)[:, -1]
         if logits_mode == "none":
             logits = None
         elif logits_mode == "logprob":
@@ -374,14 +382,14 @@
             else:
                 logits = ops.linear_logprob(hb, self.lm_head, targets, rms_eps=self.eps, col_offset=off)
         elif self.precision == "highest":
-            hl = h if logits_mode == "all" else h.reshape(b, s, d)[:, -1].contiguous()
+            hl = h if logits_mode == "all" else h_last.contiguous()
             logits = ops.linear_f32(self.final_norm(hl), self.lm_head_f32)
             if logits_mode == "argmax":
                 logits = ops.argmax(logits.contiguous())
         elif logits_mode == "argmax":
-            logits = ops.linear_argmax(hb.reshape(b, s, d)[:, -1].contiguous(), self.lm_head, rms_eps=self.eps)
-        else:
-            hl = hb if logits_mode == "all" else hb.reshape(b, s, d)[:, -1].contiguous()
+            logits = ops.linear_argmax(hb_last.contiguous(), self.lm_head, rms_eps=self.eps)
+        else:
+            hl = hb if logits_mode == "all" else hb_last.contiguous()
             logits = ops.linear(hl, self.lm_head, rms_eps=self.eps, out_dtype=torch.float32)
         return logits, h, hidden, attns
 
diff --git a/jax_llama_amd/models/modules.py b/jax_llama_amd/models/modules.py
--- a/jax_llama_amd/models/modules.py
+++ b/jax_llama_amd/models/modules.py
@@ -8,6 +8,9 @@
 from ..ops import reference as ref
 
 
+LAST_LAYER_ON_FINAL_ROWS = True
+
+
 class LLaMAAttention:
     def __init__(self, model, layer_idx: int):
         self.model = model
@@ -16,6 +19,14 @@
     @property
     def weights(self):
         return self.model.layers[self.layer_idx]
+
+    def attend(self, hb, positions, cache, slot0, kv_start, key_mask, seq_len: int) -> torch.Tensor:
+        m, lw = self.model, self.weights
+        kc, vc = cache.layer(self.layer_idx)
+        q = ops.linear_qkv_rope(hb, lw.qkv, m.eps, m.rope, positions, kc, vc, slot0, seq_len,
+                                m.n_heads, m.n_kv_heads, m.head_dim)
+        q4 = q.reshape(hb.shape[0] // seq_len, seq_len, m.n_heads, m.head_dim)
+        return ops.attention(q4, kc, vc, slot0, kv_start, key_mask)
 
     def __call__(self, h, hb, positions, cache, slot0, kv_start, key_mask, seq_len: int,
                  output_attentions: bool = False, pk: Optional["PackedActs"] = None) -> Optional[torch.Tensor]:
@@ -73,7 +84,8 @@
         g = ops.linear_swiglu(hb, lw.gu, rms_eps=m.eps, x_packed=pk.hb_in() if pk else None,
                               out_packed=pk.act if pk else None)
 
-        m._row_parallel(g, lw.down, h, hb, x_packed=pk.act if pk else None, mirror_packed=pk.hb if pk else None)
+        m._row_parallel(g, lw.down, h, hb, x_packed=pk.act if pk else None, mirror_packed=pk.hb if pk else None,
+                        stat_eps=m.eps)
 
 
 class LLaMABlock:
@@ -87,6 +99,30 @@
         w = self.attention(h, hb, positions, cache, slot0, kv_start, key_mask, seq_len, output_attentions, pk)
         self.feed_forward(h, hb, pk)
         return w
+
+    def last_rows_exact(self, rows: int) -> bool:
+        m, lw = self.attention.model, self.attention.weights
+        dev = m.device
+        return (ops.unsplit_gemm4(rows, lw.o, ops.MODE_RESIDUAL, None, dev)
+                and ops.unsplit_gemm4(rows, lw.gu, ops.MODE_SWIGLU, m.eps, dev)
+                and ops.unsplit_gemm4(rows, lw.down, ops.MODE_RESIDUAL, None, dev))
+
+    def last_rows(self, h, hb, positions, cache, slot0, kv_start, key_mask, seq_len: int):
+        m = self.attention.model
+        b = hb.shape[0] // seq_len
+        a = self.attention.attend(hb, positions, cache, slot0, kv_start, key_mask, seq_len)
+        dev, d = hb.device, hb.shape[1]
+        ws = ops.workspace
+        a_c = ws.get("last_rows_att", b * a.shape[1], a.dtype, dev).view(b, a.shape[1])
+        h_c = ws.get("last_rows_h", b * d, h.dtype, dev).view(b, d)
+        hb_c = ws.get("last_rows_hb", b * d, hb.dtype, dev).view(b, d)
+        a_c.copy_(a.view(b, seq_len, -1)[:, -1])
+        h_c.copy_(h.view(b, seq_len, d)[:, -1])
+        hb_c.copy_(hb.view(b, seq_len, d)[:, -1])
+        with ops.pinned_plan():
+            m._row_parallel(a_c, self.attention.weights.o, h_c, hb_c)
+            self.feed_forward(h_c, hb_c)
+        return h_c, hb_c
 
 
 class PackedActs:
@@ -111,7 +147,7 @@
         return len(self.blocks)
 
     def __call__(self, h, hb, positions, cache, slot0, kv_start, key_mask, seq_len: int,
-                 output_hidden_states: bool = False, output_attentions: bool = False):
+                 output_hidden_states: bool = False, output_attentions: bool = False, last_rows: bool = False):
         hidden, attns = [], []
         b = hb.shape[0] // seq_len
         rows = hb.shape[0]
@@ -119,10 +155,17 @@
         if (ops.PACKED_X and hb.is_cuda and ops.PACKED_X_MIN_M <= rows <= min(ops.PACKED_ATT_MAX_M, ops.SKINNY_M)
                 and self.model.comm.packs_residual(rows * self.model.config.hidden_size * 4)):
             pk = PackedActs(rows, self.model, hb.device, full=rows <= ops.PACKED_X_MAX_M)
+        last_rows = (last_rows and LAST_LAYER_ON_FINAL_ROWS and seq_len > 1 and pk is None and bool(self.blocks)
+                     and not output_hidden_states and not output_attentions and self.model.comm.size == 1
+                     and self.blocks[-1].last_rows_exact(rows))
+        last = None
         for blk in self.blocks:
             if output_hidden_states:
                 hidden.append(h.reshape(b, seq_len, -1).clone())
+            if last_rows and blk is self.blocks[-1]:
+                last = blk.last_rows(h, hb, positions, cache, slot0, kv_start, key_mask, seq_len)
+                break
             w = blk(h, hb, positions, cache, slot0, kv_start, key_mask, seq_len, output_attentions, pk)
             if output_attentions:
                 attns.append(w)
-        return hidden, attns
+        return hidden, attns, last
diff --git a/jax_llama_amd/ops/__init__.py b/jax_llama_amd/ops/__init__.py
--- a/jax_llama_amd/ops/__init__.py
+++ b/jax_llama_amd/ops/__init__.py
@@ -64,12 +64,14 @@
     def clear(self):
         self._bufs.clear()
         self.generation += 1
+        _ROWSTAT.clear()
 
 
 workspace = _Workspace()
 
 
 def embedding(ids: torch.Tensor, table: torch.Tensor, mirror: Optional[torch.Tensor] = None) -> torch.Tensor:
+    rowstat_reset(table.device)
     if not _is_gpu(table):
         out = ref.embedding(ids, table)
         if mirror is not None:
@@ -89,6 +91,7 @@
 
 
 def residual_add_(h: torch.Tensor, p: torch.Tensor, mirror: Optional[torch.Tensor] = None) -> torch.Tensor:
+    rowstat_reset(h.device)
     if not _is_gpu(h):
         h.add_(p.float().view_as(h))
         if mirror is not None:
@@ -169,13 +172,14 @@
 
 def linear_residual(x: torch.Tensor, w, residual: torch.Tensor, rms_eps: Optional[float] = None,
                     accumulate: bool = True, mirror: Optional[torch.Tensor] = None,
-                    x_packed: Optional[torch.Tensor] = None, mirror_packed: Optional[torch.Tensor] = None) -> torch.Tensor:
+                    x_packed: Optional[torch.Tensor] = None, mirror_packed: Optional[torch.Tensor] = None,
+                    mirror_stat_eps: Optional[float] = None) -> torch.Tensor:
     if not _is_gpu(x):
         ref.linear_residual(x, w.dense(), residual, rms_eps, accumulate)
         if mirror is not None:
             mirror.copy_(residual.to(BF16))
         return residual
-    _gpu_linear(x, w, residual, MODE_RESIDUAL, rms_eps, accumulate, mirror, x_packed, mirror_packed)
+    _gpu_linear(x, w, residual, MODE_RESIDUAL, rms_eps, accumulate, mirror, x_packed, mirror_packed, mirror_stat_eps)
     return residual
 
 
@@ -242,19 +246,27 @@
     return x.shape[0] > 0 and e.gemv_w4_plan_check(x.shape[0], w.n, w.k, mode, x.dtype != BF16)[0] == 0
 
 
-def _gpu_linear(x, w, out, mode, rms_eps, accumulate, mirror=None, x_packed=None, pack_out=None):
+def _gpu_linear(x, w, out, mode, rms_eps, accumulate, mirror=None, x_packed=None, pack_out=None, stat_eps=None):
+    global pinned_calls
     assert x.is_contiguous() and out.is_contiguous()
     assert x.shape[1] == w.k, (x.shape, w.k)
     m = x.shape[0]
     e = ext()
+    if _PIN_TILE is not None and m > 0:
+        w = bf16_weight(w)
+        pinned_calls += 1
+        _tiled(e, x, w.weight, w.n, w.k, out, mode, rms_eps, accumulate, mirror, None, stat_eps, plan=(1, _PIN_TILE))
+        return
     if is_mxfp4(w):
         if _w4_fast(e, x, w, mode):
+            rowstat_reset(x.device)
             e.linear_skinny_w4(x, w.qweight, w.scale, w.n, w.k, out, mode, -1.0 if rms_eps is None else float(rms_eps),
                                bool(accumulate), mirror, pack_out if mode != MODE_STORE else None)
             return
         w = bf16_weight(w)
     if is_fp8(w):
         if _w8_fast(e, x, w, mode):
+            rowstat_reset(x.device)
             e.linear_skinny_w8(x, w.qweight, w.scale, w.n, w.k, out, mode, -1.0 if rms_eps is None else float(rms_eps),
                                bool(accumulate), mirror, pack_out if mode != MODE_STORE else None)
             return
@@ -265,8 +277,9 @@
     if v == TILED and pack_out is not None and not _tiled_packs(e, m, w.n, w.k, x.device, mode, rms_eps):
         v = 1
     if v == TILED:
-        _tiled(e, x, w.weight, w.n, w.k, out, mode, rms_eps, accumulate, mirror, pack_out)
+        _tiled(e, x, w.weight, w.n, w.k, out, mode, rms_eps, accumulate, mirror, pack_out, stat_eps)
     else:
+        rowstat_reset(x.device)
         ws, tk = _skinny_ws(e, m, w.n, w.k, mode, x.device)
         e.linear_skinny(x, w.weight, w.n, w.k, out, mode, -1.0 if rms_eps is None else float(rms_eps),
                         bool(accumulate), v, ws, tk, mirror, x_packed if v in XP_VARIANTS else None, pack_out)
@@ -276,6 +289,7 @@
                        x_packed: Optional[torch.Tensor] = None, hb_pack: Optional[torch.Tensor] = None) -> torch.Tensor:
     e = ext()
     m = x.shape[0]
+    rowstat_reset(x.device)
     assert x.dtype == BF16 and x.is_contiguous() and m <= e.SKINNY_MAX_M, (x.dtype, x.shape)
     v = _variant(e, x, w, MODE_RESIDUAL, x_packed, pack_out=True)
     if v not in autotune.GEMV_VARIANTS:
@@ -291,6 +305,7 @@
 def tiled_tp_residual(x: torch.Tensor, w, h: torch.Tensor, hb: torch.Tensor, state: int) -> bool:
     e = ext()
     m = x.shape[0]
+    rowstat_reset(x.device)
     assert x.dtype == BF16 and x.is_contiguous(), (x.dtype, x.shape)
     ks, tm = autotune.choose_gemm_plan(e, m, w.n, w.k, x.device, MODE_STORE, False)
     if tm not in autotune.G5_TILES and ks <= 1:
@@ -329,12 +344,76 @@
     return workspace.get("gemm_rms", x.shape[0], torch.float32, x.device)
 
 
-def _tiled(e, x, weight, n, k, out, mode, rms_eps, accumulate, mirror=None, pack_out=None):
+FUSED_ROWSTAT = True
+_ROWSTAT = {}
+
+
+def _rowstat_key(device):
+    return (workspace._scope, device)
+
+
+def rowstat_reset(device=None) -> None:
+    if device is None:
+        _ROWSTAT.clear()
+    else:
+        _ROWSTAT.pop(_rowstat_key(device), None)
+
+
+def _rowstat_note(mirror: torch.Tensor, eps: float, scratch: torch.Tensor) -> None:
+    cols = mirror.shape[-1]
+    _ROWSTAT[_rowstat_key(mirror.device)] = (mirror.data_ptr(), mirror.numel() // cols, cols, float(eps),
+                                             mirror._version, scratch.data_ptr())
+
+
+def _rowstat_take(x: torch.Tensor, eps, scratch: Optional[torch.Tensor]) -> bool:
+    held = _ROWSTAT.pop(_rowstat_key(x.device), None)
+    if held is None or scratch is None or eps is None or not FUSED_ROWSTAT or x.dim() != 2:
+        return False
+    return held == (x.data_ptr(), x.shape[0], x.shape[1], float(eps), x._version, scratch.data_ptr())
+
+
+_PIN_TILE = None
+pinned_calls = 0
+
+
+@contextlib.contextmanager
+def pinned_plan(tile: int = 7):
+    global _PIN_TILE
+    prev, _PIN_TILE = _PIN_TILE, int(tile)
+    try:
+        yield
+    finally:
+        _PIN_TILE = prev
+
+
+def unsplit_gemm4(rows: int, w, mode: int, rms_eps: Optional[float], device) -> bool:
+    if device.type != "cuda":
+        return True
+    e = ext()
+    if rows <= e.SKINNY_MAX_M:
+        return False
+    fused = _fused_rms(e, mode, rms_eps)
+    ks, tm = autotune.choose_gemm_plan(e, rows, w.n, w.k, device, mode, fused)
+    return bool(e.gemm_plan_g4_unsplit(rows, w.n, w.k, mode, fused, ks, tm, fused and ks <= 1))
+
+
+def _tiled(e, x, weight, n, k, out, mode, rms_eps, accumulate, mirror=None, pack_out=None, stat_eps=None, plan=None):
     fused = _fused_rms(e, mode, rms_eps)
     xb = _tiled_input(x, rms_eps, fused)
-    ks, tm, ws = _gemm_ws(e, x.shape[0], n, k, x.device, mode, fused)
-    e.gemm(xb, weight, n, k, out, mode, bool(accumulate), mirror, ks, ws, float(rms_eps) if fused else -1.0, tm,
-           pack_out, _rms_ws(x, fused, ks))
+    if plan is None:
+        ks, tm, ws = _gemm_ws(e, x.shape[0], n, k, x.device, mode, fused)
+    else:
+        assert plan[0] == 1, plan
+        ks, tm, ws = 1, plan[1], None
+    rws = _rms_ws(x, fused, ks)
+    ready = _rowstat_take(x, rms_eps, rws)
+    stat = None
+    if FUSED_ROWSTAT and stat_eps is not None and mode == MODE_RESIDUAL and mirror is not None:
+        stat = workspace.get("gemm_rms", x.shape[0], torch.float32, x.device)
+    wrote = e.gemm(xb, weight, n, k, out, mode, bool(accumulate), mirror, ks, ws, float(rms_eps) if fused else -1.0,
+                   tm, pack_out, rws, 0, ready, stat, 0.0 if stat_eps is None else float(stat_eps))
+    if wrote:
+        _rowstat_note(mirror, stat_eps, stat)
 
 
 def _tiled_packs(e, m, n, k, device, mode, rms_eps) -> bool:
@@ -429,6 +508,7 @@
         return rope_kv_write(qkv, table, positions, k_cache, v_cache, slot0, seq_len, n_heads, n_kv_heads, head_dim)
     if is_mxfp4(w):
         if _w4_fast(e, x, w, MODE_QKV):
+            rowstat_reset(x.device)
             q = torch.empty(m, n_heads, head_dim, dtype=BF16, device=x.device)
             e.linear_qkv_w4(x, w.qweight, w.scale, w.n, w.k, -1.0 if rms_eps is None else float(rms_eps), table,
                             positions.reshape(-1).to(torch.int32), k_cache, v_cache, _slot_tensor(slot0, x.device),
@@ -437,6 +517,7 @@
         w = bf16_weight(w)
     if is_fp8(w):
         if _w8_fast(e, x, w, MODE_QKV):
+            rowstat_reset(x.device)
             q = torch.empty(m, n_heads, head_dim, dtype=BF16, device=x.device)
             e.linear_qkv_w8(x, w.qweight, w.scale, w.n, w.k, -1.0 if rms_eps is None else float(rms_eps), table,
                             positions.reshape(-1).to(torch.int32), k_cache, v_cache, _slot_tensor(slot0, x.device),
@@ -451,20 +532,23 @@
         fused = _fused_rms(e, MODE_QKV, rms_eps)
         if ks == 1 and fused and QKV_DIRECT and e.gemm_qkv_direct_ok(m, tm, w.k):
             q = torch.empty(m, n_heads, head_dim, dtype=BF16, device=x.device)
+            rws = _rms_ws(x, fused, 1)
             e.gemm_qkv(_tiled_input(x, rms_eps, fused), w.weight, w.n, w.k, table, positions.reshape(-1).to(torch.int32),
                        k_cache, v_cache, _slot_tensor(slot0, x.device), int(seq_len), int(n_heads), int(n_kv_heads),
-                       int(head_dim), q, 1, None, float(rms_eps), tm, _rms_ws(x, fused, 1))
+                       int(head_dim), q, 1, None, float(rms_eps), tm, rws, _rowstat_take(x, rms_eps, rws))
             return q
         if ks == 1:
             qkv = linear(x, w, rms_eps=rms_eps)
             return rope_kv_write(qkv, table, positions, k_cache, v_cache, slot0, seq_len, n_heads, n_kv_heads,
                                  head_dim)
         q = torch.empty(m, n_heads, head_dim, dtype=BF16, device=x.device)
+        rowstat_reset(x.device)
         e.gemm_qkv(_tiled_input(x, rms_eps, fused), w.weight, w.n, w.k, table, positions.reshape(-1).to(torch.int32),
                    k_cache, v_cache, _slot_tensor(slot0, x.device), int(seq_len), int(n_heads), int(n_kv_heads),
                    int(head_dim), q, ks, ws, float(rms_eps) if fused else -1.0, tm)
         return q
     q = torch.empty(m, n_heads, head_dim, dtype=BF16, device=x.device)
+    rowstat_reset(x.device)
     ws, tk = _skinny_ws(e, m, w.n, w.k, MODE_QKV, x.device)
     e.linear_qkv(x, w.weight, w.n, w.k, -1.0 if rms_eps is None else float(rms_eps), table,
                  positions.reshape(-1).to(torch.int32), k_cache, v_cache, _slot_tensor(slot0, x.device),
@@ -536,6 +620,7 @@
     e = ext()
     m = x.shape[0]
     dev = x.device
+    rowstat_reset(dev)
     rep = n_heads // n_kv_heads
     q = workspace.get("qa_q", m * n_heads * head_dim, BF16, dev).view(m, n_heads, head_dim)
     out = torch.empty(m, n_heads * head_dim, dtype=BF16, device=dev)
@@ -677,8 +762,9 @@
     ws = workspace.get("gemm_argmax", e.gemm_argmax_workspace(m, w.n), torch.float32, x.device)
     idx = torch.empty(m, dtype=torch.int32, device=x.device)
     val = torch.empty(m, dtype=torch.float32, device=x.device)
-    e.gemm_argmax(xb, w.weight, w.n, w.k, ws, -1.0 if rms_eps is None else float(rms_eps), idx, val,
-                  _rms_ws(x, rms_eps is not None, 1))
+    rws = _rms_ws(x, rms_eps is not None, 1)
+    e.gemm_argmax(xb, w.weight, w.n, w.k, ws, -1.0 if rms_eps is None else float(rms_eps), idx, val, rws,
+                  _rowstat_take(x, rms_eps, rws))
     return idx, val
 
 
@@ -721,8 +807,9 @@
         e = ext()
         xb = x if x.dtype == BF16 else x.to(BF16)
         ws = workspace.get("gemm_logprob", e.gemm_logprob_workspace(m, w.n), torch.float32, x.device)
+        rws = _rms_ws(x, rms_eps is not None, 1)
         e.gemm_logprob(xb, w.weight, w.n, w.k, ws, -1.0 if rms_eps is None else float(rms_eps), tg, int(col_offset),
-                       out[0], out[1], out[2], _rms_ws(x, rms_eps is not None, 1))
+                       out[0], out[1], out[2], rws, _rowstat_take(x, rms_eps, rws))
     else:
         for r0, r1 in _logprob_chunks(m, w.n):
             logits = linear(x[r0:r1], w, rms_eps, out_dtype=torch.float32)
diff --git a/jax_llama_amd/runtime/engine.py b/jax_llama_amd/runtime/engine.py
--- a/jax_llama_amd/runtime/engine.py
+++ b/jax_llama_amd/runtime/engine.py
@@ -188,14 +188,14 @@
         mode = self._logits_mode()
         if b <= rows:
             logits, *_ = self.model.forward_tokens(ids, pos_dev, self.cache, 0, self.kv_start, self.key_mask,
-                                                   logits_mode=mode)
+                                                   logits_mode=mode, last_rows_only=True)
             return logits
         parts = []
         for b0 in range(0, b, rows):
             b1 = min(b, b0 + rows)
             km = self.key_mask[b0:b1] if self.key_mask is not None else None
             lg, *_ = self.model.forward_tokens(ids[b0:b1], pos_dev[b0:b1], self.cache.rows(b0, b1), 0,
-                                               self.kv_start[b0:b1], km, logits_mode=mode)
+                                               self.kv_start[b0:b1], km, logits_mode=mode, last_rows_only=True)
             parts.append(lg)
         if isinstance(parts[0], tuple):
             return tuple(torch.cat([p[i] for p in parts]) for i in range(len(parts[0])))
@@ -209,7 +209,7 @@
         gc = self.gc
         sampler = (gc.top_k, gc.temperature, gc.top_p, int(gc.seed)) if gc.do_sample else None
         return (gc.do_sample, self.key_mask is not None, ops.workspace.generation, _fused_greedy(),
-                ops.ARGMAX_FUSED_MIN_M, ops.SKINNY_ARGMAX, ops.QKV_ATTN, self.model.comm.reduce_dtype,
+                ops.ARGMAX_FUSED_MIN_M, ops.SKINNY_ARGMAX, ops.QKV_ATTN, ops.FUSED_ROWSTAT, self.model.comm.reduce_dtype,
                 int(gc.pad_token_id), int(gc.eos_token_id), sampler)
 
     def _ensure_graph(self):
```

Result: no change. 41720 tokens/s (median of 6 runs) (+0.8%).
